# hy-vision-learning/jck-generation

Measured on AMD Instinct MI355X. Metric: images/sec (G+D step) DCGAN 64x64 bs256, higher is better.
Workload: dtype bf16; 1 GPU; DCGAN 64x64x3 synthetic, batch 256 per GPU, full G+D step incl. GP pass, RNG and Adam (BASELINE.json configs[1]); per_gpu_batch=256, global_batch=256, parallelism=dp1, dead_D_wgrad_in_G_phase=skipped (never observable: zeroed at train/dcgan_trainer.py:155)

## Files before the change

### include/jckgan.h

```cpp
#ifndef JCKGAN_H
#define JCKGAN_H
#include <stddef.h>
#include <stdint.h>
#ifdef __cplusplus
extern "C" {
#endif

#define JCK_PREC_BF16 0
#define JCK_PREC_F32 1
#define JCK_PREC_BF16X3 2

#define JCK_OK 0
#define JCK_E_ARG (-1)
#define JCK_E_HIP (-2)
#define JCK_E_WS (-3)

const char* jck_last_error(void);
const char* jck_last_launch(void);
const char* jck_launch_name(int i);
int jck_version(void);
int jck_pad_rows(int c);
int jck_pad_chan(int c);

size_t jck_packed_bytes(int prec, long long elems);
// ... 1 lines not shown
int jck_pack_up(int prec, const float* w, int Cs, int Cb, void* wp, void* stream);
int jck_pack_g1(int prec, const float* w, int Ci, int Co, int CiPad, void* wp, void* stream);
int jck_pack_head(const float* w, int C, float* wp, void* stream);

size_t jck_stats_floats(long long pixels, int C, int nyrep);
int jck_conv_down(int prec, const void* big, const void* w, void* small_out, float* stats, int* stats_slots,
                  int N, int Hb, int Wb, int Cb, int Cs, void* stream);
int jck_conv_up(int prec, const void* small_in, const void* w, void* big_out, float* stats, int* stats_slots,
                int epi_tanh, int N, int Hs, int Ws, int Cs, int Cb, void* stream);
size_t jck_conv_wgrad_ws_bytes(int N, int Hb, int Wb, int Cb, int Cs);
int jck_conv_wgrad(int prec, const void* small_side, const void* big_side, float* ws, size_t ws_bytes, float* grad,
                   int accumulate, int N, int Hb, int Wb, int Cb, int Cs, void* stream);
int jck_g1_fwd(int prec, const void* z, const void* w, void* out, float* stats, int* stats_slots, int B, int CiPad,
               int Co, void* stream);
int jck_conv_up_affine(int prec, const void* small_in, const void* w, const float* scale, const float* shift, void* big_out,
                       int N, int Hs, int Ws, int Cs, int Cb, void* stream);
int jck_g1_fwd_affine(int prec, const void* z, const void* w, const float* scale, const float* shift, void* out, int B,
                      int CiPad, int Co, void* stream);
int jck_conv_down_mask(int prec, const void* big, const void* w, const void* a_small, const float* scale, void* small_out,
                       int N, int Hb, int Wb, int Cb, int Cs, void* stream);
int jck_conv_down_affine(int prec, const void* big, const void* w, const float* scale, const float* shift, float slope,
                         void* small_out, int N, int Hb, int Wb, int Cb, int Cs, void* stream);
int jck_latent_loss(int prec, const void* x_nhwc4, const float* target_nchw_f32, void* g_raw_out, float* loss_out, int N, int HW,
                    void* stream);
int jck_latent_adam(int prec, const float* slab, int Z, int ld, float* z, float* m, float* v, float lr, float prior, int t,
                    void* z_operand, int CiPad, int N, void* stream);
int jck_conv_up_mask(int prec, const void* small_in, const void* w, const void* a_big, const float* scale, float slope, void* big_out,
                     int N, int Hs, int Ws, int Cs, int Cb, void* stream);
int jck_leaky_affine_bwd(int prec, const void* g, const void* a, const float* scale, float slope, void* g_y, long long rows, int C,
                         void* stream);
int jck_critic_ds(const float* logit, int mode, float weight, int B, float* ds, float* term, void* stream);
int jck_latent_loss_ex(int prec, const void* x_nhwc4, const float* target_nchw_f32, const float* weight, const void* g_x, void* g_raw_out,
                       float* loss_out, int N, int HW, void* stream);
int jck_feat_match(int prec, const void* a, const void* f, const float* scale, float slope, float weight, void* g_y, int accumulate,
                   float* fterm, int N, long long M, int C, void* stream);
size_t jck_g1_wgrad_ws_bytes(int B, int CiPad, int Co);
int jck_g1_wgrad(int prec, const void* z, const void* dy, float* ws, size_t ws_bytes, float* grad, int accumulate, int B,
                 int Ci, int CiPad, int Co, void* stream);

int jck_bn_finalize(const float* stats, int slots, float count, const float* gamma, const float* beta,
                    float* running_mean, float* running_var, int64_t* num_batches_tracked, float momentum, float eps,
                    float* aux, int C, void* stream);
int jck_bn_act_fwd(int prec, const void* y, const float* aux, float slope, void* a, long long rows, int C, void* stream);
int jck_bn_eval_aux(int nlayers, const float* const* gamma, const float* const* beta, const float* const* running_mean,
                    const float* const* running_var, float* const* aux, const int* C, float eps, void* stream);
size_t jck_bn_bwd_ws_floats(int C);
int jck_bn_act_bwd(int prec, const void* g_a, const void* y, const float* aux, float slope, float* sums, void* g_y,
                   float* dgamma, float* dbeta, long long rows, int C, void* stream);
int jck_bn_finalize_grouped(const float* stats, int slots_per_group, float count, const float* gamma, const float* beta, float eps,
                            float* aux, float* stat_out, int C, int groups, void* stream);
int jck_bn_fwd(int prec, const void* y, const float* stats, int slots_per_group, float count, const float* gamma, const float* beta,
               float eps, float slope, void* a, float* aux, float* stat_out, float* running_mean, float* running_var, int64_t* nbt,
               float momentum, long long rows_per_group, int C, int groups, void* stream);
int jck_bn_act_fwd_grouped(int prec, const void* y, const float* aux, float slope, void* a, long long rows_per_group, int C,
                           int groups, void* stream);
int jck_bn_act_bwd_grouped(int prec, const void* g_a, const void* y, const float* aux, float slope, float* sums, void* g_y,
                           float* dgamma, float* dbeta, long long rows_per_group, int C, int groups, int grad_groups, void* stream);
size_t jck_grid_sync_bytes(void);
int jck_grid_sync_error(const void* sync_ws);
int jck_bn_act_bwd_res(int prec, const void* g_a, const void* y, const float* aux, float slope, float* sums, void* g_y,
                       float* dgamma, float* dbeta, long long rows_per_group, int C, int groups, int grad_groups, void* sync_ws,
                       void* stream);
int jck_conv_down_grouped(int prec, const void* big, const void* w, void* small_out, float* stats, int* stats_slots, int N, int Hb,
                          int Wb, int Cb, int Cs, int group_images, void* stream);
int jck_conv_up_grouped(int prec, const void* small_in, const void* w, void* big_out, float* stats, int* stats_slots, int N, int Hs,
                        int Ws, int Cs, int Cb, int group_images, void* stream);
int jck_img_prep(int prec, const float* img_nchw, const float* noise_nchw, float keep, float mix, void* out, int N, int HW,
                 void* stream);
int jck_img_prep_u8(int prec, const unsigned char* data, const int64_t* idx, const float* noise, float keep, float mix,
                    void* out_nhwc4, float* out_nchw, int B, int Hs, int Ws, void* stream);
#define JCK_RESIZE_MAX_SRC 1024
#define JCK_RESIZE_TAPS_MAGIC 0x7a736572
long long jck_resize_taps_bytes(int Hs, int Ws, int S);
int jck_resize_taps_build(int Hs, int Ws, int S, void* host_buf);
int jck_img_prep_u8_any(int prec, const unsigned char* data, const int64_t* idx, const unsigned char* flip, const float* noise,
                        const unsigned* rng, int tensor_id, float keep, float mix, void* out_nhwc4, float* out_nchw, int B, int Hs,
                        int Ws, int S, const void* taps_dev, void* stream);
long long jck_resize_lds_bytes(int Hs, int S, int* band, int* rows);
int jck_img_prep_u8_box(int prec, const unsigned char* data, const int64_t* idx, const unsigned char* flip,
                        const int* origin , const float* noise,
                        const unsigned* rng, int tensor_id, float keep, float mix, void* out_nhwc4, float* out_nchw,
                        int B, int Hs, int Ws, int Hc, int Wc, int y0, int x0 , int S,
                        const void* taps_dev , void* stream);
int jck_resize_norm(const float* in, float* out, int N, int C, int H, int W, int OH, int OW, float pre_scale, float pre_shift,
                    const float* mean, const float* stdv, void* stream);
int jck_nhwc4_to_nchw(int prec, const void* in, float* out_nchw, int N, int HW, void* stream);
int jck_img_to_u8(int prec, const void* in, unsigned char* out_u8_nhwc, int N, int HW, void* stream);
int jck_axpy_noise(int prec, const void* x, const float* noise_nchw, float keep, float mix, void* out, int N, int HW,
                   void* stream);
int jck_interp(int prec, const void* a, const void* b, const float* alpha, void* out, int N, int HW, void* stream);
int jck_mix_interp(int prec, const void* x, const float* noise_nchw, const unsigned* rng, int tensor_id, float keep, float mix, void* out,
                   const void* real, const float* alpha, void* xhat, int N, int HW, void* stream);
int jck_gp_norm(int prec, const void* g, int N, int HW, float* scal, int slot, int scal_ld, float* norms, void* stream);
int jck_tanh_bwd(int prec, const void* g, const void* y, float scale, void* out, long long numel, void* stream);
int jck_head_fwd(int prec, const void* a4, const float* wp, const float* bias , int B, int K,
                 float target, int mode, float* prob, float* ds, float* scal, int slot_loss, int slot_p, int scal_ld, void* stream);
int jck_score_head(int prec, const void* x, const float* w, const float* bias , int B, int K,
                   float* logit, float* prob , void* stream);
int jck_grid_pool(int prec, const void* a, int N, int H, int C, int grid, int mode, float* out, long long ld, long long col0,
                  void* stream);
int jck_head_fwd_grouped(int prec, const void* a4, const float* wp, const float* bias, int B, int K, int G, const float* targets,
                         const int* modes, float* prob, float* ds, float* scal, const int* slot_loss, const int* slot_p,
                         int scal_ld, void* stream);
size_t jck_head_bwd_ws_floats(int K);
int jck_head_bwd(int prec, const float* ds, const float* wp, const void* a4, int B, int K, void* g_a4, float* dwp,
                 int accumulate, float* ws, void* stream);
int jck_head_unpack_grad(const float* dwp, int C, float* grad, int accumulate, void* stream);
int jck_head_bwd_conv(int prec, const float* ds, const float* wp, const void* a4, int B, int C, void* g_a4, float* grad,
                      float* ws, void* stream);
int jck_head_bwd_conv2(int prec, const float* ds, const float* wp, const void* a4, int B, int B_more, int C, void* g_a4, float* grad,
                       float* ws, void* stream);

int jck_pack_linear(int prec, const float* w, int N, int K, int rows, int cols, int transpose, int permC, int permHW, void* wp,
                    void* stream);
int jck_linear_fwd(int prec, const void* x, const void* wp, const float* bias, void* out, int B, int Kpad, int N, int NStore,
                   int ksplit, void* stream);
int jck_linear_finish(int prec, const float* slab, int Z, const float* bias, const float* mask, float scale, void* h, void* hd,
                      int B, int N, void* stream);
size_t jck_linear_wgrad_ws_bytes(int B, int Kpad, int N);
int jck_linear_wgrad(int prec, const void* gy, int ldgy, const void* x, int Kpad, float* ws, size_t ws_bytes, float* gradp,
                     int accumulate, int B, int N, void* stream);
int jck_unperm_linear_grad(const float* gp, int N, int K, int ldp, int permC, int permHW, float* grad, int accumulate, void* stream);
int jck_label_embed_fwd(int prec, const int64_t* labels, const float* W, const float* b, float slope, int B, int NI, int NO,
                        void* cbuf, int ld, int col0, float* pre, void* stream);
int jck_label_embed_bwd(int prec, const void* gc, int ld, int col0, const float* pre, const int64_t* labels, float slope, int B,
                        int NI, int NO, float* dW, float* db, void* stream);
int jck_label_embed_fwd_tiled(int prec, const int64_t* labels, const float* W, const float* b, float slope, int B, int NI, int NO,
                              void* cbuf, int ld, int col0, float* pre, int label_period, void* stream);
int jck_label_embed_bwd_tiled(int prec, const void* gc, int ld, int col0, const float* pre, const int64_t* labels, float slope,
                              int B, int NI, int NO, float* dW, float* db, int label_period, void* stream);
int jck_concat_rows(int prec, const void* a4, int K0, void* cbuf, int ld, int B, void* stream);
int jck_split_rows(int prec, const void* gc, int ld, int K0, void* ga4, int B, void* stream);
int jck_dropout(int prec, const void* x, const float* mask, float scale, void* y, long long n, void* stream);
int jck_colsum(int prec, const void* g, int B, int N, int ld, float* db, void* stream);
int jck_sum_vec(const float* x, int n, float* out, void* stream);
int jck_cgan_z(int prec, const float* z, const int64_t* labels, int B, int NZ, int NL, int CiPad, void* out, void* stream);
int jck_gp_grad(int prec, const void* g, const float* norms, float coef, int N, int HW, void* u, void* stream);
int jck_gp_head2(int prec, const void* ughd, const float* w2, const float* prob, int B, int K, float* rs, float* dw2, float* ws,
                 void* stream);
size_t jck_gp_head2_conv_ws_floats(int B);
int jck_gp_head2_conv(int prec, const void* v4, const void* a4, const float* wp, const float* prob, int B, int C, float* rs,
                      void* g_a4, float* grad, float* ws, void* stream);
size_t jck_bn2_ws_floats(int C);
int jck_bn2_vchain(int prec, const void* v, const void* y, const void* gy, const float* aux, const float* s1, const float* gamma,
                   float slope, float* ws, void* u, void* xdir, float* dgamma, long long rows, int C, void* stream);
int jck_bn2_reverse(int prec, const void* ua, const void* y, const void* xdir, const float* aux, const float* gamma,
                    const float* vsums, float slope, float* ws, void* uy, float* dgamma, float* dbeta, long long rows, int C,
                    void* stream);

int jck_adam(float* p, const float* g, float* m, float* v, long long n, double lr, double beta1, double beta2, double eps,
             int step, float grad_scale, void* stream);
int jck_adam_ema(float* p, const float* g, float* m, float* v, float* ema, long long n, double lr, double beta1, double beta2,
                 double eps, int step, float grad_scale, float ema_weight, const unsigned* skip_if, void* stream);

typedef struct jck_engine jck_engine;
int jck_engine_create(jck_engine** out, int family, int prec, int batch);
int jck_engine_create_sized(jck_engine** out, int family, int prec, int batch, int image_size);
#define JCK_ENGINE_GP_BACKWARD 1u
int jck_engine_create_ex(jck_engine** out, int family, int prec, int batch, int image_size, unsigned flags);
int jck_engine_image_size(const jck_engine*);
int jck_engine_num_tensors_of(const jck_engine*, int net);
int jck_engine_tensor_info_of(const jck_engine*, int net, int idx, char* name, int name_cap, int* kind, long long* offset,
                              long long* numel, int* shape4);
long long jck_engine_arena_numel_of(const jck_engine*, int net, int which);
void jck_engine_destroy(jck_engine*);
int jck_engine_num_tensors(int family, int net );
int jck_engine_tensor_info(int family, int net, int idx, char* name, int name_cap, int* kind, long long* offset,
                           long long* numel, int* shape4);
size_t jck_engine_workspace_bytes(const jck_engine*);
long long jck_engine_arena_numel(int family, int net, int which );
int jck_engine_bind(jck_engine*, void* workspace, size_t ws_bytes, float* g_params, float* g_grads, float* g_m, float* g_v,
                    float* g_bn, int64_t* g_nbt, float* d_params, float* d_grads, float* d_m, float* d_v, float* d_bn,
                    int64_t* d_nbt);
int jck_engine_repack(jck_engine*, int net, void* stream);
#define JCK_PHASE_D_LOSS 0
#define JCK_PHASE_D_GP 1
#define JCK_PHASE_D_STEP 2
#define JCK_PHASE_G_LOSS 3
#define JCK_PHASE_G_STEP 4
#define JCK_PHASE_D_REAL 5
#define JCK_PHASE_D_FAKE 6
#define JCK_PHASE_D_REAL_FWD 7
#define JCK_PHASE_D_LOSS_A 8
#define JCK_PHASE_D_LOSS_B 9
#define JCK_PHASE_GP_ONLY 10
#define JCK_PHASE_LAZY_JOIN 0x100
#define JCK_PHASE_NO_RESIDENT 0x200
typedef struct jck_step_inputs {
  const float* real_nchw;
  const float* noise_real;
  const float* z;
  const float* noise_fake;
  const float* alpha;
  float lr;
  float grad_scale;
  int step;
  const int64_t* labels;
  const float* drop_mask[4];
  const unsigned char* real_u8;
  const int64_t* real_idx;
  int real_h, real_w;
  const unsigned char* real_flip;
  const void* real_taps;
  int real_box_h, real_box_w, real_y0, real_x0;
  const int* real_origin;
} jck_step_inputs;
int jck_engine_phase(jck_engine*, int phase, const jck_step_inputs* in, void* stream);
long long jck_engine_grad_tail(const jck_engine*, int net);
int jck_engine_order_after_tail(jck_engine*, void* stream);
int jck_engine_drop_prefetch(jck_engine*, void* stream);
int jck_engine_check(jck_engine*);
const float* jck_engine_scalars(const jck_engine*);
const float* jck_engine_scalars_at(const jck_engine*, int step);
int jck_engine_sample(jck_engine*, const float* z, const int64_t* labels , int n, float* out_nchw, void* stream);
#define JCK_SAMPLE_EVAL 1u
int jck_engine_sample_ex(jck_engine*, const float* z, const int64_t* labels, int n, unsigned flags, float* out_nchw ,
                         unsigned char* out_u8_nhwc , void* stream);
int jck_engine_latent_grad(jck_engine*, const float* z, const int64_t* labels, const float* target_nchw, int n,
                           float* loss , float* dz , void* stream);
int jck_engine_project(jck_engine*, float* z , const int64_t* labels, const float* target_nchw, int n,
                       int steps, float lr, float prior, float* m, float* v , int t0,
                       float* loss_hist , void* stream);
int jck_engine_latent_grad_ex(jck_engine*, const float* z, const int64_t* labels, const float* target_nchw ,
                              const float* weight , int critic_mode, float critic_weight, int n, float* loss ,
                              float* term , float* logit , float* dz , void* stream);
int jck_engine_project_ex(jck_engine*, float* z , const int64_t* labels, const float* target_nchw , int n,
                          int steps, float lr, float prior, const float* weight , int critic_mode, float critic_weight,
                          float* m, float* v, int t0, float* loss_hist , float* term_hist ,
                          void* stream);
int jck_engine_latent_grad_fm(jck_engine*, const float* z, const int64_t* labels, const float* target_nchw ,
                              const float* weight , int critic_mode, float critic_weight, int n, float* loss ,
                              float* term , float* logit , float* dz , void* stream,
                              const float* feat_target_nchw , int feat_stage, float feat_weight, float* fterm );
int jck_engine_project_fm(jck_engine*, float* z , const int64_t* labels, const float* target_nchw , int n,
                          int steps, float lr, float prior, const float* weight , int critic_mode, float critic_weight,
                          float* m, float* v, int t0, float* loss_hist , float* term_hist ,
                          void* stream, const float* feat_target_nchw , int feat_stage, float feat_weight,
                          float* fterm_hist );
int jck_engine_score(jck_engine*, const float* images_nchw , const float* noise_nchw ,
                     const int64_t* labels , int n, float* logit , float* prob , void* stream);
long long jck_engine_feature_dim(const jck_engine*, int grid);
int jck_engine_features(jck_engine*, const float* images_nchw ,
                        int n, int grid, int mode, float* out , long long ld, void* stream);
const void* jck_engine_tensor(const jck_engine*, const char* name, long long* numel);

int jck_conv2d_nhwc_f32(const float* x, const float* w_kc, const float* scale, const float* shift, float* out, int N, int H, int W,
                        int Cin, int KH, int KW, int SH, int SW, int PH, int PW, int Cout, int out_cstride, int out_coff, int relu,
                        void* stream);
int jck_pool2d_nhwc_f32(const float* x, float* out, int N, int H, int W, int C, int k, int stride, int pad, int mode, int out_cstride,
                        int out_coff, void* stream);
int jck_global_avgpool_nhwc_f32(const float* x, float* out, int N, int HW, int C, void* stream);
int jck_nchw_to_nhwc_f32(const float* x, float* out, int N, int C, int H, int W, void* stream);
int jck_mean_cov_f64(const float* x, double* mean, double* cov, int N, int D, void* stream);

size_t jck_pairstat_ws_bytes(int M, int N);
int jck_poly3_sum_f64(const float* x, int M, const float* y, int N, int D, double gamma, double coef0, int skip_diag, double* out,
                      double* ws, void* stream);
int jck_knn_radius2_f32(const float* x, int N, int D, int k, float* r2, void* stream);
int jck_manifold_hit_u8(const float* q, int M, const float* ref, const float* r2, int N, int D, unsigned char* hit, void* stream);

size_t jck_knn_index_ws_bytes(int M, int N);
int jck_knn_index_f32(const float* q, int M, const float* ref, int N, int D, int k, long long q_base, long long ref_base,
                      int exclude_self, int merge, long long* idx, float* d2, void* ws, void* stream);

int jck_engine_set_step(jck_engine*, int step, float lr, void* stream);
int jck_engine_bind_ema(jck_engine*, float* g_ema);
int jck_engine_set_ema(jck_engine*, double decay, int start_step);
int jck_engine_set_noise_seed(jck_engine*, unsigned long long seed);
int jck_step_rng(float* hp, int step, unsigned long long seed, float* z, long long nz, float* alpha, long long nalpha,
                 float* masks, long long nmask, float keep_p, void* stream);
int jck_img_prep_rng(int prec, const float* img_nchw, const unsigned* rng, int tensor_id, float keep, float mix, void* out, int N, int HW,
                     void* stream);
int jck_img_prep_u8_rng(int prec, const unsigned char* data, const int64_t* idx, const unsigned* rng, int tensor_id, float keep,
                        float mix, void* out_nhwc4, int B, int Hs, int Ws, void* stream);
int jck_axpy_noise_rng(int prec, const void* x, const unsigned* rng, int tensor_id, float keep, float mix, void* out, int N, int HW,
                       void* stream);
int jck_engine_capture_begin(jck_engine*, void* stream);
int jck_engine_capture_end(jck_engine*, void* stream, void** graph_exec);
int jck_engine_capture_abort(jck_engine*, void* stream);
int jck_engine_graph_nodes(const jck_engine*);
int jck_graph_launch(void* graph_exec, void* stream);
void jck_graph_destroy(void* graph_exec);

int jck_tune(const char* key, int value);
int jck_prof_enable(int on);
int jck_prof_collect(int cap, const char** name_out, int* count_out, double* ms_out, double* flops_out, double* bytes_out,
                     void** stream_out);

int jck_debug_tr_read(const void* in, int ld, void* out, void* stream);

typedef struct jck_comm jck_comm;
#define JCK_COMM_ID_BYTES 128
int jck_comm_unique_id(unsigned char* id128);
int jck_comm_create(jck_comm** out, const unsigned char* id128, int world, int rank);
int jck_comm_world(const jck_comm*);
int jck_comm_allreduce_enqueue(jck_comm*, float* buf, size_t count, void* producer_stream, int* ticket);
int jck_comm_wait(jck_comm*, int ticket, void* consumer_stream);
int jck_comm_destroy(jck_comm*);

#ifdef __cplusplus
}
#endif
#endif
```

### jck-generation_amd/csrc/engine.hip

```cpp
#include <cstdlib>

#include "engine_internal.hpp"
#define JCK_BATCHED_DEFAULT 3

namespace {

constexpr long long ALIGN_F = 64;

void add_param(NetLayout& L, const char* name, int a, int b, int c, int d) {
  TensorInfo ti{name, 0, L.n_params, (long long)a * b * c * d, {a, b, c, d}};
  L.t.push_back(ti);
  L.n_params = (L.n_params + ti.numel + ALIGN_F - 1) / ALIGN_F * ALIGN_F;
}
void add_bn(NetLayout& L, const char* wn, const char* bn, const char* rm, const char* rv, int c) {
  add_param(L, wn, c, 1, 1, 1);
  add_param(L, bn, c, 1, 1, 1);
  TensorInfo m{rm, 1, L.n_bn, c, {c, 1, 1, 1}};
  L.t.push_back(m);
  L.n_bn += (c + ALIGN_F - 1) / ALIGN_F * ALIGN_F;
  TensorInfo v{rv, 2, L.n_bn, c, {c, 1, 1, 1}};
  L.t.push_back(v);
  L.n_bn += (c + ALIGN_F - 1) / ALIGN_F * ALIGN_F;
}

Topo make_topo(int S) {
  Topo T = {};
  T.S = S; T.NS = S == 128 ? 5 : 4; T.HW = S * S;
  T.G_C1 = 64 << (T.NS - 1);
  T.FEAT = 16 * T.G_C1;
  for (int i = 0; i < T.NS; ++i) {
    T.D_CS[i] = 64 << i; T.D_CB[i] = i == 0 ? 3 : 32 << i; T.D_HB[i] = S >> i;
    T.G_CS[i] = T.G_C1 >> i; T.G_CB[i] = i == T.NS - 1 ? 3 : T.G_C1 >> (i + 1); T.G_HS[i] = 4 << i;
  }
  return T;
}
NetLayout make_layout(int family, int net, int S = 64) {
  NetLayout L;
  const Topo T = make_topo(S);
  const char* const* CW = CWN; const char* const* NW = NWN; const char* const* NB = NBN; const char* const* RM = RMN; const char* const* RV = RVN;
  if (net == 0) {
    add_param(L, CW[0], z_dim(family), T.G_C1, 4, 4);
    add_bn(L, NW[0], NB[0], RM[0], RV[0], T.G_C1);
    for (int i = 0; i < T.NS; ++i) {
      add_param(L, CW[i + 1], T.G_CS[i], T.G_CB[i], 4, 4);
      if (i < T.NS - 1) add_bn(L, NW[i + 1], NB[i + 1], RM[i + 1], RV[i + 1], T.G_CB[i]);
    }
  } else {
    if (family == 1) {
      add_param(L, "label_embedding.weight", EMB, N_CLASS, 1, 1);
      add_param(L, "label_embedding.bias", EMB, 1, 1, 1);
    }
    for (int i = 0; i < T.NS; ++i) {
      add_param(L, CW[i], T.D_CS[i], T.D_CB[i], 4, 4);
      add_bn(L, NW[i], NB[i], RM[i], RV[i], T.D_CS[i]);
    }
    if (family == 0) {
      add_param(L, CW[T.NS], 1, T.G_C1, 4, 4);
    } else {
      add_param(L, "linear1.weight", L1_OUT, L1_K, 1, 1);
      add_param(L, "linear1.bias", L1_OUT, 1, 1, 1);
      add_param(L, "linear2.weight", 1, L1_OUT, 1, 1);
      add_param(L, "linear2.bias", 1, 1, 1, 1);
    }
  }
  return L;
}

}

static unsigned jck_event_flags() { return hipEventDisableTiming | hipEventDisableSystemFence; }

DActs DActs::group(const jck_engine* e, int first, int n) const {
  DActs v = *this;
  v.g0 = g0 + first; v.groups = n;
  const size_t B = (size_t)e->B;
  auto at = [&](void* p, size_t elems) { return (void*)((unsigned char*)p + elems * e->esz); };
  for (int i = 0; i < TT.NS; ++i) {
    const int cs = TT.D_CS[i];
    const size_t px = (size_t)(TT.D_HB[i] / 2) * (TT.D_HB[i] / 2), off = first * B * px * cs;
    v.y[i] = at(y[i], off); v.a[i] = at(a[i], off); v.g[i] = at(g[i], off);
    v.aux[i] = aux[i] + (size_t)first * 4 * cs;
    v.sums[i] = sums[i] + (size_t)first * jck_bn_bwd_ws_floats(cs);
    v.stats[i] = stats[i] + (size_t)first * (jck_stats_floats((long long)(cap * B * px), cs, 1) / cap / (2 * cs)) * (2 * cs);
  }
  v.prob = prob + first * B; v.ds = ds + first * B;
  return v;
}

static bool env_on(const char* name) {
  const char* v = getenv(name);
  return !(v && atoi(v) == 0);
}
static int create_side_streams(jck_engine* e) {
  hipError_t rc = hipSuccess;
  e->for_each_side_stream([&](hipStream_t& s) { if (rc == hipSuccess) rc = hipStreamCreateWithFlags(&s, hipStreamNonBlocking); });
  e->for_each_event([&](hipEvent_t& ev) { if (rc == hipSuccess) rc = hipEventCreateWithFlags(&ev, jck_event_flags()); });
  HIPCHK(rc);
  return JCK_OK;
}
static void destroy_side_streams(jck_engine* e, bool sync) {
  e->for_each_side_stream([&](hipStream_t& s) {
    if (s) { if (sync) (void)hipStreamSynchronize(s); (void)hipStreamDestroy(s); }
    s = nullptr;
  });
  e->for_each_event([](hipEvent_t& ev) { if (ev) (void)hipEventDestroy(ev); ev = nullptr; });
}

extern "C" int jck_engine_create(jck_engine** out, int family, int prec, int batch) {
  return jck_engine_create_sized(out, family, prec, batch, 64);
}
extern "C" int jck_engine_create_sized(jck_engine** out, int family, int prec, int batch, int image_size) {
  return jck_engine_create_ex(out, family, prec, batch, image_size, 0);
}
extern "C" int jck_engine_create_ex(jck_engine** out, int family, int prec, int batch, int image_size, unsigned flags) {
  if (!out) JCK_FAIL(JCK_E_ARG, "null out");
  if (flags & ~JCK_ENGINE_GP_BACKWARD) JCK_FAIL(JCK_E_ARG, "unknown engine flags");
  if (image_size != 64 && image_size != 128) JCK_FAIL(JCK_E_ARG, "image_size must be 64 or 128");
  if (image_size != 64 && family != 0) JCK_FAIL(JCK_E_ARG, "the 128x128 topology exists for DCGAN only (CGAN's Linear(8392,256) fixes 64x64)");
  if (family != 0 && family != 1) JCK_FAIL(JCK_E_ARG, "family must be 0 (DCGAN) or 1 (CGAN)");
  if (prec != JCK_PREC_BF16 && !prec_f32_storage(prec)) JCK_FAIL(JCK_E_ARG, "bad prec");
  if (batch < 1 || batch > 8192) JCK_FAIL(JCK_E_ARG, "batch must be in [1, 8192]");
  jck_engine* e = new jck_engine();
  e->family = family; e->prec = prec; e->B = batch; e->esz = prec_f32_storage(prec) ? 4 : 2;
  e->T = make_topo(image_size);
  e->LG = make_layout(family, 0, image_size); e->LD = make_layout(family, 1, image_size);
  e->overlap = env_on("JCK_OVERLAP");
  e->batched = getenv("JCK_BATCHED") ? atoi(getenv("JCK_BATCHED")) : JCK_BATCHED_DEFAULT;
  if (!e->overlap || batch % 8 != 0 || e->batched != 3) e->batched = 0;
  e->gp_bwd = family == 0 && (flags & JCK_ENGINE_GP_BACKWARD);
  e->carve(nullptr);
  e->wgrad_side = env_on("JCK_WGRAD_SIDE");
  e->head_side = env_on("JCK_HEAD_SIDE");
  e->ext_events = env_on("JCK_EXT_EVENTS");
  e->bn_res = env_on("JCK_BN_RES");
  e->cbuf_direct = family == 1 && env_on("JCK_CBUF_DIRECT");
  e->head_fuse = env_on("JCK_HEAD_FUSE");
  e->real_side = env_on("JCK_REAL_SIDE");
  e->fold_zero = env_on("JCK_FOLD_ZERO");
  e->fuse_tanh = env_on("JCK_FUSE_TANH");
  if (e->overlap) JCK_TRY(create_side_streams(e));
  *out = e;
  return JCK_OK;
}
extern "C" void jck_engine_destroy(jck_engine* e) {
  if (!e) return;
  if (e->overlap) destroy_side_streams(e, true);
  infer_free(e);
  delete e;
}
extern "C" int jck_engine_num_tensors(int family, int net) { return (int)make_layout(family, net).t.size(); }
static int tensor_info(const NetLayout& L, int idx, char* name, int name_cap, int* kind, long long* offset, long long* numel, int* shape4) {
  if (idx < 0 || idx >= (int)L.t.size()) JCK_FAIL(JCK_E_ARG, "index out of range");
  const TensorInfo& t = L.t[idx];
  if (name && name_cap > 0) { strncpy(name, t.name, name_cap - 1); name[name_cap - 1] = 0; }
  if (kind) *kind = t.kind;
  if (offset) *offset = t.offset;
  if (numel) *numel = t.numel;
  if (shape4) for (int q_ = 0; q_ < 4; ++q_) shape4[q_] = t.shape[q_];
  return JCK_OK;
}
static long long arena_numel(const NetLayout& L, int which) { return which == 0 ? L.n_params : L.n_bn; }
extern "C" int jck_engine_tensor_info(int family, int net, int idx, char* name, int name_cap, int* kind, long long* offset,
                                      long long* numel, int* shape4) {
  return tensor_info(make_layout(family, net), idx, name, name_cap, kind, offset, numel, shape4);
}
extern "C" long long jck_engine_arena_numel(int family, int net, int which) { return arena_numel(make_layout(family, net), which); }
extern "C" int jck_engine_num_tensors_of(const jck_engine* e, int net) { return e ? (int)(net == 0 ? e->LG : e->LD).t.size() : 0; }
extern "C" int jck_engine_tensor_info_of(const jck_engine* e, int net, int idx, char* name, int name_cap, int* kind, long long* offset,
                                         long long* numel, int* shape4) {
  if (!e) JCK_FAIL(JCK_E_ARG, "null engine");
  return tensor_info(net == 0 ? e->LG : e->LD, idx, name, name_cap, kind, offset, numel, shape4);
}
extern "C" long long jck_engine_arena_numel_of(const jck_engine* e, int net, int which) {
  return e ? arena_numel(net == 0 ? e->LG : e->LD, which) : 0;
}
extern "C" int jck_engine_image_size(const jck_engine* e) { return e ? e->T.S : 0; }
extern "C" size_t jck_engine_workspace_bytes(const jck_engine* e) { return e ? e->ws_bytes : 0; }

extern "C" int jck_engine_bind(jck_engine* e, void* workspace, size_t ws_bytes, float* g_params, float* g_grads, float* g_m,
                               float* g_v, float* g_bn, int64_t* g_nbt, float* d_params, float* d_grads, float* d_m,
                               float* d_v, float* d_bn, int64_t* d_nbt) {
  if (!e || !workspace) JCK_FAIL(JCK_E_ARG, "null engine / workspace");
  if (ws_bytes < e->ws_bytes) JCK_FAIL(JCK_E_WS, "workspace too small: need " + std::to_string(e->ws_bytes));
  if (((uintptr_t)workspace) % 256) JCK_FAIL(JCK_E_ARG, "workspace must be 256-byte aligned");
  e->carve(reinterpret_cast<unsigned char*>(workspace));
  {
    unsigned char* p0 = reinterpret_cast<unsigned char*>(e->d_down[0]);
    unsigned char* p1 = reinterpret_cast<unsigned char*>(e->dset[0].y[0]);
    HIPCHK(hipMemset(p0, 0, (size_t)(p1 - p0)));
  }
  HIPCHK(hipMemset(e->gsync, 0, jck_grid_sync_bytes()));
  e->gp = g_params; e->gg = g_grads; e->gm = g_m; e->gv = g_v; e->gbn = g_bn; e->gnbt = g_nbt;
  e->dp = d_params; e->dg = d_grads; e->dm = d_m; e->dv = d_v; e->dbn = d_bn; e->dnbt = d_nbt;
  e->bound = true;
  return JCK_OK;
}

static int repack_convs(jck_engine* e, int net, void* stream, const TailJobs* tail = nullptr, int tail_x = 0) {
  PackJobs jobs = {};
  int n = 0, chunk = 0;
  auto add = [&](int kind, const float* w, void* wp, long long total, int a, int b, int c) {
    PackJob& J = jobs.j[n];
    J.w = w; J.wp = wp; J.total = total; J.kind = kind; J.a = a; J.b = b; J.c = c;
    jobs.first_chunk[n] = chunk;
    chunk += (int)((total + PACK_CHUNK - 1) / PACK_CHUNK);
    ++n;
  };
  auto add_down = [&](const float* w, int Cs, int Cb, void* wp) { add(0, w, wp, (long long)Cs * Cb, Cs, Cb, ilog2(jck_pad_chan(Cb))); };
  auto add_up = [&](const float* w, int Cs, int Cb, void* wp) {
    if (Cb <= 4) add(2, w, wp, (long long)Cs * Cb, Cs, Cb, 0);
    else add(1, w, wp, (long long)Cs * Cb, Cs, Cb, jck_pad_rows(Cb));
  };
  if (net == 1) {
    for (int i = 0; i < TT.NS; ++i) {
      const float* w = e->P(e->LD, e->dp, CWN[i]);
      add_down(w, TT.D_CS[i], TT.D_CB[i], e->d_down[i]);
      add_up(w, TT.D_CS[i], TT.D_CB[i], e->d_up[i]);
    }
    if (e->family == 0) add(4, e->P(e->LD, e->dp, CWN[TT.NS]), e->d_head_wp, TT.G_C1, TT.G_C1, 0, 0);
  } else {
    add(3, e->P(e->LG, e->gp, CWN[0]), e->g1_w, (long long)z_dim(e->family) * TT.G_C1, z_dim(e->family), TT.G_C1, z_pad(e->family));
    for (int i = 0; i < TT.NS; ++i) {
      const float* w = e->P(e->LG, e->gp, CWN[i + 1]);
      add_up(w, TT.G_CS[i], TT.G_CB[i], e->g_up[i]);
      add_down(w, TT.G_CS[i], TT.G_CB[i], e->g_down[i]);
    }
  }
  jobs.first_chunk[n] = chunk;
  jobs.n = n;
  if (net == 1) e->d_packed = true;
  if (tail) {
    const int nblk = chunk + tail_x * (tail->nl + 1);
    if (e->prec == JCK_PREC_BF16) hipLaunchKernelGGL(pack_tail_kernel<bf16_t>, dim3(nblk), dim3(256), 0, (hipStream_t)stream, jobs, chunk, *tail, tail_x);
    else hipLaunchKernelGGL(pack_tail_kernel<float>, dim3(nblk), dim3(256), 0, (hipStream_t)stream, jobs, chunk, *tail, tail_x);
  } else if (e->prec == JCK_PREC_BF16) hipLaunchKernelGGL(pack_multi_kernel<bf16_t>, dim3(chunk), dim3(256), 0, (hipStream_t)stream, jobs);
  else hipLaunchKernelGGL(pack_multi_kernel<float>, dim3(chunk), dim3(256), 0, (hipStream_t)stream, jobs);
  HIPCHK(hipGetLastError());
  return JCK_OK;
}
static int repack_linear(jck_engine* e, void* stream) {
  const float* w1 = e->P(e->LD, e->dp, "linear1.weight");
  return pack_linear_pair(e->prec, w1, L1_OUT, L1_K, L1_OUT, L1_KPAD, e->l1_w, L1_KPAD, L1_OUT, e->l1_wT, 512, 16, (hipStream_t)stream);
}
extern "C" int jck_engine_repack(jck_engine* e, int net, void* stream) {
  if (!e || !e->bound) JCK_FAIL(JCK_E_ARG, "engine not bound");
  JCK_TRY(repack_convs(e, net, stream));
  if (net == 1 && e->family == 1) JCK_TRY(repack_linear(e, stream));
  return JCK_OK;
}

static const double ADAM_B1 = 0.5, ADAM_B2 = 0.999, ADAM_EPS = 1e-8;


static int fork_side(jck_engine* e, int k, hipStream_t st, hipStream_t side, hipStream_t* ws, bool record = true) {
  *ws = st;
  if (!side) return JCK_OK;
  if (record) HIPCHK(hipEventRecord(e->evW[k], st));
  HIPCHK(hipStreamWaitEvent(side, e->evW[k], 0));
  *ws = side;
  return JCK_OK;
}

static int d_convs_forward(jck_engine* e, const DActs& S, const void* x_in, int B, int pass0, hipStream_t st, bool to_cbuf = false) {
  const int n = S.groups;
  const void* in = x_in;
  for (int i = 0; i < TT.NS; ++i) {
    const int hb = TT.D_HB[i], cs = TT.D_CS[i];
    const long long rows = (long long)B * (hb / 2) * (hb / 2);
    float* rec = e->d_rs[i] + ((size_t)e->parity * 4 + pass0 + S.g0) * 2 * cs;
    int slots = 0;
    JCK_TRY(jck_conv_down_grouped(e->prec, in, e->d_down[i], S.y[i], S.stats[i], &slots, n * B, hb, hb, TT.D_CB[i], cs, B, st));
    if (slots % n) JCK_FAIL(JCK_E_ARG, "batched D pass: statistic slots do not split by group");
    const bool cb = to_cbuf && i == TT.NS - 1;
    void* out = cb ? (unsigned char*)e->cbuf + (size_t)S.g0 * B * L1_KPAD * e->esz : S.a[i];
    bool fused = false;
    JCK_TRY(bn_fwd_fused(e->prec, S.y[i], S.stats[i], slots / n, (float)rows, e->P(e->LD, e->dp, NWN[i]), e->P(e->LD, e->dp, NBN[i]), BN_EPS, LRELU, out,
                         S.aux[i], rec, nullptr, nullptr, nullptr, BN_MOM, rows, cs, n, cb ? TT.FEAT : 0, cb ? L1_KPAD : 0, st, &fused));
    if (!fused) {
      JCK_TRY(jck_bn_finalize_grouped(S.stats[i], slots / n, (float)rows, e->P(e->LD, e->dp, NWN[i]), e->P(e->LD, e->dp, NBN[i]), BN_EPS, S.aux[i], rec,
                                      cs, n, st));
      JCK_TRY(bn_act_fwd_pitched(e->prec, S.y[i], S.aux[i], LRELU, out, rows, cs, n, cb ? TT.FEAT : 0, cb ? L1_KPAD : 0, st));
    }
    in = S.a[i];
  }
  return JCK_OK;
}

static int cg_head_forward(jck_engine* e, const void* a4, int rows, const float* drop_mask, hipStream_t st, int label_period = 0, bool finish = true) {
  if (!e->cur_labels || !drop_mask) JCK_FAIL(JCK_E_ARG, "CGAN pass needs labels and a dropout mask");
  if (a4) JCK_TRY(jck_concat_rows(e->prec, a4, TT.FEAT, e->cbuf, L1_KPAD, rows, st));
  JCK_TRY(jck_label_embed_fwd_tiled(e->prec, e->cur_labels, e->P(e->LD, e->dp, "label_embedding.weight"),
                                    e->P(e->LD, e->dp, "label_embedding.bias"), LRELU, rows, N_CLASS, EMB, e->cbuf, L1_KPAD, TT.FEAT,
                                    e->pre_e, label_period, st));
  JCK_TRY(jck_linear_fwd(e->prec, e->cbuf, e->l1_w, nullptr, e->l1_slab, rows, L1_KPAD, L1_OUT, L1_OUT, L1_KSPLIT, st));
  if (!finish) return JCK_OK;
  return jck_linear_finish(e->prec, e->l1_slab, L1_KSPLIT, e->P(e->LD, e->dp, "linear1.bias"), drop_mask, 1.0f / 0.75f, e->h_pre,
                           e->h_drop, rows, L1_OUT, st);
}
static int cg_head_middle(jck_engine* e, int B, int G, const float* targets, const int* modes, const int* slot_loss, const int* slot_p,
                          float* prob, float* ds, const float* drop_mask, hipStream_t st) {
  return cg_head_mid(e->prec, e->l1_slab, L1_KSPLIT, e->P(e->LD, e->dp, "linear1.bias"), drop_mask, 1.0f / 0.75f, e->h_pre, e->h_drop,
                     e->P(e->LD, e->dp, "linear2.weight"), e->P(e->LD, e->dp, "linear2.bias"), B, G, targets, modes, prob, ds, e->acc, slot_loss,
                     slot_p, e->acc_ld, e->g_hd, e->g_h, st);
}

static int d_forward(jck_engine* e, DActs& D, const void* x_in, int B, int pass, const float* drop_mask, hipStream_t st, bool head_finish = true) {
  const bool direct = e->family == 1 && e->cbuf_direct;
  JCK_TRY(d_convs_forward(e, D, x_in, B, pass, st, direct));
  if (e->family == 1) return cg_head_forward(e, direct ? nullptr : D.a[TT.NS - 1], B, drop_mask, st, 0, head_finish);
  return JCK_OK;
}

static int d_head(jck_engine* e, DActs& D, int B, float target, int mode, int slot_loss, int slot_p, hipStream_t st, void* g_out = nullptr) {
  if (e->family == 0)
    return head_fwd_grouped_ev(e->prec, D.a[TT.NS - 1], e->d_head_wp, nullptr, B, TT.FEAT, 1, &target, &mode, D.prob, D.ds, e->acc, &slot_loss,
                               &slot_p, e->acc_ld, g_out, st, nullptr);
  return jck_head_fwd(e->prec, e->h_drop, e->P(e->LD, e->dp, "linear2.weight"), e->P(e->LD, e->dp, "linear2.bias"), B, L1_OUT, target,
                      mode, D.prob, D.ds, e->acc, slot_loss, slot_p, e->acc_ld, st);
}

static int d_head_backward(jck_engine* e, DActs& D, const float* ds, int B, bool want_wgrad, const float* drop_mask, void* ga4_out, hipStream_t st,
                           hipStream_t side = nullptr, bool mid_done = false) {
  if (e->family == 0)
    return jck_head_bwd_conv(e->prec, ds, e->d_head_wp, D.a[TT.NS - 1], B, TT.G_C1, mid_done ? nullptr : ga4_out,
                             want_wgrad ? e->P(e->LD, e->dg, CWN[TT.NS]) : nullptr, e->head_ws, st);
  const size_t r0 = (size_t)e->ss.head_row0, w0 = (size_t)e->ss.head_wrow0;
  auto hb = [&](void* p, size_t row, size_t per_row) { return (void*)((unsigned char*)p + row * per_row * e->esz); };
  void *h_drop = hb(e->h_drop, r0, L1_OUT), *cbuf = hb(e->cbuf, r0, L1_KPAD);
  void *g_hd = hb(e->g_hd, w0, L1_OUT), *g_h = hb(e->g_h, w0, L1_OUT), *gc = hb(e->gc, w0, L1_KPAD);
  const float* pre_e = e->pre_e + r0 * EMB;
  hipStream_t ws = st;
  auto fork = [&](int k) { return fork_side(e, k, st, side, &ws); };
  const float* w2 = e->P(e->LD, e->dp, "linear2.weight");
  if (!mid_done) JCK_TRY(jck_head_bwd(e->prec, ds, w2, h_drop, B, L1_OUT, g_hd, nullptr, 1, e->head_ws, st));
  if (want_wgrad) {
    JCK_TRY(fork(0));
    JCK_TRY(jck_head_bwd(e->prec, ds, w2, h_drop, B, L1_OUT, nullptr, e->P(e->LD, e->dg, "linear2.weight"), 1, e->head_ws, ws));
    JCK_TRY(jck_sum_vec(ds, B, e->P(e->LD, e->dg, "linear2.bias"), ws));
  }
  if (!mid_done) JCK_TRY(jck_dropout(e->prec, g_hd, drop_mask, 1.0f / 0.75f, g_h, (long long)B * L1_OUT, st));
  if (want_wgrad) {
    JCK_TRY(fork(1));
    JCK_TRY(jck_linear_wgrad(e->prec, g_h, L1_OUT, cbuf, L1_KPAD, e->wg_ws, e->wg_ws_bytes, e->gw1p, 1, B, L1_OUT, ws));
    JCK_TRY(jck_colsum(e->prec, g_h, B, L1_OUT, L1_OUT, e->P(e->LD, e->dg, "linear1.bias"), ws));
  }
  JCK_TRY(jck_linear_fwd(e->prec, g_h, e->l1_wT, nullptr, gc, B, L1_OUT, L1_KPAD, L1_KPAD, 1, st));
  if (want_wgrad) {
    JCK_TRY(fork(2));
    JCK_TRY(jck_label_embed_bwd(e->prec, gc, L1_KPAD, TT.FEAT, pre_e, e->cur_labels, LRELU, B, N_CLASS, EMB,
                                e->P(e->LD, e->dg, "label_embedding.weight"), e->P(e->LD, e->dg, "label_embedding.bias"), ws));
  }
  return jck_split_rows(e->prec, gc, L1_KPAD, TT.FEAT, ga4_out, B, st);
}

static int cg_head_backward_batched(jck_engine* e, const float* ds, int B, const float* drop_mask, void* ga4_out, hipStream_t st,
                                    hipStream_t side = nullptr, bool mid_done = false) {
  const int R3 = 3 * B, R2 = 2 * B;
  const float* w2 = e->P(e->LD, e->dp, "linear2.weight");
  hipStream_t ws = st;
  auto fork = [&](int k) { return fork_side(e, k, st, side, &ws); };
  if (!mid_done) JCK_TRY(jck_head_bwd(e->prec, ds, w2, e->h_drop, R3, L1_OUT, e->g_hd, nullptr, 1, e->head_ws, st));
  if (!mid_done) {
    JCK_TRY(fork(0));
    JCK_TRY(jck_head_bwd(e->prec, ds, w2, e->h_drop, R2, L1_OUT, nullptr, e->P(e->LD, e->dg, "linear2.weight"), 1, e->head_ws, ws));
    JCK_TRY(jck_sum_vec(ds, R2, e->P(e->LD, e->dg, "linear2.bias"), ws));
    JCK_TRY(jck_dropout(e->prec, e->g_hd, drop_mask, 1.0f / 0.75f, e->g_h, (long long)R3 * L1_OUT, st));
  }
  JCK_TRY(fork(1));
  if (mid_done) {
    JCK_TRY(jck_head_bwd(e->prec, ds, w2, e->h_drop, R2, L1_OUT, nullptr, e->P(e->LD, e->dg, "linear2.weight"), 1, e->head_ws, ws));
    JCK_TRY(jck_sum_vec(ds, R2, e->P(e->LD, e->dg, "linear2.bias"), ws));
  }
  JCK_TRY(jck_linear_wgrad(e->prec, e->g_h, L1_OUT, e->cbuf, L1_KPAD, e->wg_ws, e->wg_ws_bytes, e->gw1p, 1, R2, L1_OUT, ws));
  JCK_TRY(jck_colsum(e->prec, e->g_h, R2, L1_OUT, L1_OUT, e->P(e->LD, e->dg, "linear1.bias"), ws));
  JCK_TRY(jck_linear_fwd(e->prec, e->g_h, e->l1_wT, nullptr, e->gc, R3, L1_OUT, L1_KPAD, L1_KPAD, 1, st));
  JCK_TRY(fork(2));
  JCK_TRY(jck_label_embed_bwd_tiled(e->prec, e->gc, L1_KPAD, TT.FEAT, e->pre_e, e->cur_labels, LRELU, R2, N_CLASS, EMB,
                                    e->P(e->LD, e->dg, "label_embedding.weight"), e->P(e->LD, e->dg, "label_embedding.bias"), B, ws));
  if (side) HIPCHK(hipEventRecord(e->evHead, side));
  return jck_split_rows(e->prec, e->gc, L1_KPAD, TT.FEAT, ga4_out, R3, st);
}

// ... 133 lines not shown
    JCK_TRY(jck_linear_wgrad(e->prec, gh1, L1_OUT, e->cbuf2, L1_KPAD, e->wg_ws, e->wg_ws_bytes, e->gw1p, 1, B, L1_OUT, ws));
    if (side) (void)hipEventRecord(e->evGP, side);
    JCK_TRY(jck_linear_fwd(e->prec, e->cbuf2, e->l1_w, nullptr, e->l1_slab, B, L1_KPAD, L1_OUT, L1_OUT, L1_KSPLIT, st));
    const bool fuse = e->head_fuse && L1_OUT == 256;
    if (!fuse) JCK_TRY(jck_linear_finish(e->prec, e->l1_slab, L1_KSPLIT, nullptr, drop_mask, 1.0f / 0.75f, nullptr, e->ughd, B, L1_OUT, st));
    hipStream_t hs = e->head_side && e->ext_events ? side : nullptr;
    if (fuse) {
      const size_t w0 = (size_t)e->ss.head_wrow0 * L1_OUT * esz;
      JCK_TRY(gp_head_mid_ev(e->prec, e->l1_slab, L1_KSPLIT, drop_mask, 1.0f / 0.75f, e->ughd, e->P(e->LD, e->dp, "linear2.weight"), prob1, B, e->rs,
                             e->P(e->LD, e->dg, "linear2.weight"), e->gp2_ws, (unsigned char*)e->g_hd + w0, (unsigned char*)e->g_h + w0, st, hs,
                             hs ? e->evHead : nullptr));
    } else
      JCK_TRY(gp_head2_ev(e->prec, e->ughd, e->P(e->LD, e->dp, "linear2.weight"), prob1, B, L1_OUT, e->rs,
                          e->P(e->LD, e->dg, "linear2.weight"), e->gp2_ws, st, hs, hs ? e->evHead : nullptr));
    if (side) (void)hipStreamWaitEvent(st, e->evGP, 0); else join();
    JCK_TRY(d_head_backward(e, e->dset[0], e->rs, B, true, drop_mask, e->d_v[TT.NS - 1], st, hs, fuse));
    JCK_TRY(jck_unperm_linear_grad(e->gw1p, L1_OUT, L1_K, L1_KPAD, 512, 16, e->P(e->LD, e->dg, "linear1.weight"), 1, hs ? hs : st));
  }
  for (int i = TT.NS - 1; i >= 0; --i) {
    const int hb = TT.D_HB[i], cs = TT.D_CS[i], cb = TT.D_CB[i];
    const long long rows = (long long)B * (hb / 2) * (hb / 2);
    JCK_TRY(jck_bn2_reverse(e->prec, e->d_v[i], P.y[i], e->d_xdir[i], P.aux[i], e->P(e->LD, e->dp, NWN[i]), e->bn2_ws[i],
                            LRELU, e->bn2_ws_rev, e->d_v[i], e->P(e->LD, e->dg, NWN[i]), e->P(e->LD, e->dg, NBN[i]), rows, cs, st));
    const void* big = i == 0 ? xhat : P.a[i - 1];
    JCK_TRY(fork(i));
    JCK_TRY(jck_conv_wgrad(e->prec, e->d_v[i], big, e->wg_ws, e->wg_ws_bytes, e->P(e->LD, e->dg, CWN[i]), 1, B, hb, hb, cb, cs, ws));
    if (side && lazy_join && i == 1) { (void)hipEventRecord(e->evWmid, side); e->ss.mid_recorded = true; }
    if (i > 0)
      JCK_TRY(jck_conv_up(e->prec, e->d_v[i], e->d_up[i], e->d_v[i - 1], nullptr, nullptr, 0, B, hb / 2, hb / 2, cs, cb, st));
  }
  if (side && lazy_join) { (void)hipEventRecord(e->evWdone, side); e->ss.join_pending = true; }
  else join();
  return JCK_OK;
}

int g_eval_fold(jck_engine* e, hipStream_t st) {
  const float *gamma[JCK_MAX_STAGES], *beta[JCK_MAX_STAGES], *rm[JCK_MAX_STAGES], *rv[JCK_MAX_STAGES];
  float* aux[JCK_MAX_STAGES];
  int Cs[JCK_MAX_STAGES];
  for (int i = 0; i < TT.NS; ++i) {
    gamma[i] = e->P(e->LG, e->gp, NWN[i]); beta[i] = e->P(e->LG, e->gp, NBN[i]);
    rm[i] = e->gbn + find(e->LG, RMN[i])->offset; rv[i] = e->gbn + find(e->LG, RVN[i])->offset;
    aux[i] = e->g_bn[i].aux; Cs[i] = TT.G_C1 >> i;
  }
  return jck_bn_eval_aux(TT.NS, gamma, beta, rm, rv, aux, Cs, BN_EPS, st);
}
int g_eval_products(jck_engine* e, int B, hipStream_t st) {
  const int zp = z_pad(e->family);
  auto scale = [&](int i) { return e->g_bn[i].aux; };
  auto shift = [&](int i) { return e->g_bn[i].aux + (TT.G_C1 >> i); };
  JCK_TRY(jck_g1_fwd_affine(e->prec, e->g_z, e->g1_w, scale(0), shift(0), e->g_a[0], B, zp, TT.G_C1, st));
  for (int i = 0; i < TT.NS; ++i) {
    const int h = 4 << i;
    if (i < TT.NS - 1)
      JCK_TRY(jck_conv_up_affine(e->prec, e->g_a[i], e->g_up[i], scale(i + 1), shift(i + 1), e->g_a[i + 1], B, h, h, TT.G_CS[i], TT.G_CB[i], st));
    else
      JCK_TRY(jck_conv_up(e->prec, e->g_a[i], e->g_up[i], e->fake_raw, nullptr, nullptr, 1, B, h, h, TT.G_CS[i], TT.G_CB[i], st));
  }
  return JCK_OK;
}

int g_forward(jck_engine* e, const float* z, const int64_t* labels, int B, hipStream_t st, bool z_in_place, bool eval) {
  const int zp = z_pad(e->family);
  if (e->family == 1) {
    if (!labels) JCK_FAIL(JCK_E_ARG, "CGAN generator needs labels");
    JCK_TRY(jck_cgan_z(e->prec, z, labels, B, 100, N_CLASS, zp, e->g_z, st));
  } else if (!z_in_place) {
    e->ss.gz_step = -1;
    if (e->prec == JCK_PREC_BF16) launch_pad_rows<bf16_t>(z, B, 100, zp, e->g_z, st); else launch_pad_rows<float>(z, B, 100, zp, e->g_z, st);
    HIPCHK(hipGetLastError());
  }
  if (eval) {
    JCK_TRY(g_eval_fold(e, st));
    return g_eval_products(e, B, st);
  }
  JCK_TRY(jck_g1_fwd(e->prec, e->g_z, e->g1_w, e->g_y[0], e->g_bn[0].stats, &e->g_bn[0].slots, B, zp, TT.G_C1, st));
  for (int i = 0; i < TT.NS; ++i) {
    const int h = 4 << i, C = TT.G_C1 >> i;
    const long long rows = (long long)B * h * h;
    bool fused = false;
    JCK_TRY(bn_fwd_fused(e->prec, e->g_y[i], e->g_bn[i].stats, e->g_bn[i].slots, (float)rows, e->P(e->LG, e->gp, NWN[i]), e->P(e->LG, e->gp, NBN[i]), BN_EPS,
                         0.f, e->g_a[i], e->g_bn[i].aux, nullptr, e->gbn + find(e->LG, RMN[i])->offset, e->gbn + find(e->LG, RVN[i])->offset,
                         (int64_t*)(e->gnbt + i), BN_MOM, rows, C, 1, 0, 0, st, &fused));
    if (!fused) {
    JCK_TRY(jck_bn_finalize(e->g_bn[i].stats, e->g_bn[i].slots, (float)rows, e->P(e->LG, e->gp, NWN[i]), e->P(e->LG, e->gp, NBN[i]),
                            e->gbn + find(e->LG, RMN[i])->offset, e->gbn + find(e->LG, RVN[i])->offset,
                            e->gnbt + i, BN_MOM, BN_EPS, e->g_bn[i].aux, C, st));
    JCK_TRY(jck_bn_act_fwd(e->prec, e->g_y[i], e->g_bn[i].aux, 0.f, e->g_a[i], rows, C, st));
    }
    if (i < TT.NS - 1)
      JCK_TRY(jck_conv_up_grouped(e->prec, e->g_a[i], e->g_up[i], e->g_y[i + 1], e->g_bn[i + 1].stats, &e->g_bn[i + 1].slots, B, h, h, TT.G_CS[i], TT.G_CB[i], B, st));
    else
      JCK_TRY(jck_conv_up(e->prec, e->g_a[i], e->g_up[i], e->fake_raw, nullptr, nullptr, 1, B, h, h, TT.G_CS[i], TT.G_CB[i], st));
  }
  return JCK_OK;
}

static int g_backward(jck_engine* e, const void* g_fake, int B, hipStream_t st, hipStream_t side, bool raw_ready = false) {
  const bool ext = side && e->ext_events;
  if (!raw_ready)
    JCK_TRY(tanh_bwd_ev(e->prec, g_fake, e->fake_raw, 0.9f, e->g_raw, (long long)B * TT.HW * 4, st, ext ? e->evW[TT.NS - 1] : nullptr));
  const void* gbig = e->g_raw;
  for (int i = TT.NS - 1; i >= 0; --i) {
    const int hs = TT.G_HS[i], cs = TT.G_CS[i], cb = TT.G_CB[i];
    hipStream_t ws = st;
    if (side) { if (!ext) HIPCHK(hipEventRecord(e->evW[i], st)); HIPCHK(hipStreamWaitEvent(side, e->evW[i], 0)); ws = side; }
    JCK_TRY(jck_conv_wgrad(e->prec, e->g_a[i], gbig, e->wg_ws, e->wg_ws_bytes, e->P(e->LG, e->gg, CWN[i + 1]), 1, B,
                           2 * hs, 2 * hs, cb, cs, ws));
    const long long rows = (long long)B * hs * hs;
    JCK_TRY(jck_conv_down(e->prec, gbig, e->g_down[i], e->g_gr[i], nullptr, nullptr, B, 2 * hs, 2 * hs, cb, cs, st));
    JCK_TRY(bn_act_bwd_res_ev(e->prec, e->g_gr[i], e->g_y[i], e->g_bn[i].aux, 0.f, e->g_bn[i].sums, e->g_gr[i],
                              e->P(e->LG, e->gg, NWN[i]), e->P(e->LG, e->gg, NBN[i]), rows, cs, 1, 1, e->bn_res ? e->gsync : nullptr, st,
                              ext && i > 0 ? e->evW[i - 1] : nullptr));
    gbig = e->g_gr[i];
  }
  JCK_TRY(jck_g1_wgrad(e->prec, e->g_z, e->g_gr[0], e->g1_ws, e->g1_ws_bytes, e->P(e->LG, e->gg, CWN[0]), 1, B, z_dim(e->family),
                       z_pad(e->family), TT.G_C1, st));
  if (side) { HIPCHK(hipEventRecord(e->evWdone, side)); HIPCHK(hipStreamWaitEvent(st, e->evWdone, 0)); }
  return JCK_OK;
}

static int prep_real(jck_engine* e, const jck_step_inputs* in, int B, hipStream_t st) {
  if (in->real_u8 && in->real_box_h)
    return jck_img_prep_u8_box(e->prec, in->real_u8, in->real_idx, in->real_flip, in->real_origin, in->noise_real, in->noise_real ? nullptr : e->rng(),
                               0, 0.9f, 0.1f, e->real_noisy, nullptr, B, in->real_h, in->real_w, in->real_box_h, in->real_box_w, in->real_y0,
                               in->real_x0, TT.S, in->real_taps, st);
  if (in->real_u8 && in->real_taps)
    return jck_img_prep_u8_any(e->prec, in->real_u8, in->real_idx, in->real_flip, in->noise_real, in->noise_real ? nullptr : e->rng(), 0,
                               0.9f, 0.1f, e->real_noisy, nullptr, B, in->real_h, in->real_w, TT.S, in->real_taps, st);
  if (in->real_u8) {
    if (TT.S != 64) JCK_FAIL(JCK_E_ARG, "the device-resident uint8 pipeline is the reference's Resize(64) of 32x32 images: 64x64 engines only");
    if (!in->noise_real)
      return jck_img_prep_u8_rng(e->prec, in->real_u8, in->real_idx, e->rng(), 0, 0.9f, 0.1f, e->real_noisy, B, 32, 32, st);
    return jck_img_prep_u8(e->prec, in->real_u8, in->real_idx, in->noise_real, 0.9f, 0.1f, e->real_noisy, nullptr, B, 32, 32, st);
  }
  if (!in->noise_real) return jck_img_prep_rng(e->prec, in->real_nchw, e->rng(), 0, 0.9f, 0.1f, e->real_noisy, B, TT.HW, st);
  return jck_img_prep(e->prec, in->real_nchw, in->noise_real, 0.9f, 0.1f, e->real_noisy, B, TT.HW, st);
}

static int refresh_adam_scalars(jck_engine* e, int step, float lr, hipStream_t st) {
  const int q = step & 1;
  JCK_TRY(jck_adam_set_step(e->hp2 + 8 * q, (double)lr, ADAM_B1, ADAM_B2, step, e->noise_seed, e->ema_w(step), st));
  e->hp_step[q] = step;
  e->hp_lr[q] = lr;
  return JCK_OK;
}
static int set_step_impl(jck_engine* e, int step, float lr, void* stream, bool zero_d);
static int adam_net(jck_engine* e, int net, long long first, long long count, float grad_scale, const float* hp, hipStream_t st,
                    float* zero_other = nullptr, float* ema = nullptr) {
  float *p = net ? e->dp : e->gp, *g = net ? e->dg : e->gg, *m = net ? e->dm : e->gm, *v = net ? e->dv : e->gv;
  return jck_adam_hp(p + first, g + first, m + first, v + first, count, ADAM_B1, ADAM_B2, ADAM_EPS, grad_scale, hp, st, zero_other,
                     zero_other ? (net ? e->LG : e->LD).n_params : 0, jck_grid_sync_error_word(e->gsync), ema);
}
static int clear_or_memset(jck_engine* e, int& clean_step, int step, hipStream_t st, void* p, size_t bytes, void* p2 = nullptr, size_t bytes2 = 0) {
  const bool clean = clean_step == step && !e->capturing;
  clean_step = -1;
  if (!clean) HIPCHK(hipMemsetAsync(p, 0, bytes, st));
  if (!clean && p2) HIPCHK(hipMemsetAsync(p2, 0, bytes2, st));
  return JCK_OK;
}
static int zero_d_grads(jck_engine* e, int step, hipStream_t st) {
  return clear_or_memset(e, e->ss.dg_clean_step, step, st, e->dg, e->LD.n_params * sizeof(float), e->family == 1 ? e->gw1p : nullptr,
                         (size_t)L1_OUT * L1_KPAD * sizeof(float));
}
static int clear_acc(jck_engine* e, int step, hipStream_t st) {
  return clear_or_memset(e, e->ss.acc_clean_step, step, st, e->acc, (size_t)8 * e->acc_ld * sizeof(float));
}

struct PhaseCtx {
  hipStream_t st, sA;
  const jck_step_inputs* in;
  const jck_step_inputs* given;
  int B, HW;
  bool cg, lazy, lazy_tail;
  bool par, ov_g, ov_gp;
  DActs &DR, &D0, &D1;
};

static int penalty_pass(jck_engine* e, const PhaseCtx& c, DActs& D, hipStream_t s) {
  JCK_TRY(jck_interp(e->prec, e->real_noisy, e->fake, c.in->alpha, e->xhat, c.B, c.HW, s));
  JCK_TRY(d_forward(e, D, e->xhat, c.B, 2, c.in->drop_mask[2], s));
  JCK_TRY(d_head(e, D, c.B, 0.f, 1, -1, -1, s));
  DBackward bw;
  bw.gw = 0; bw.resident = c.cg; bw.xgrad = bw.gp_norm = true;
  return d_backward(e, D, e->xhat, c.B, c.in->drop_mask[2], s, bw);
}
static int g_forward_step(jck_engine* e, const PhaseCtx& c, hipStream_t s) {
  return g_forward(e, c.in->z, c.in->labels, c.B, s, c.in->z == e->rz[c.in->step & 1] && e->ss.gz_step == (long long)c.in->step);
}

static int d_batched_forward(jck_engine* e, const PhaseCtx& c, bool pre, bool split, bool direct) {
  const DActs& S = e->bset;
  const bool beside = !pre && e->real_side && c.sA;
  const bool pre_side = pre && e->ss.pre_on_side;
  e->ss.pre_on_side = false;
  hipStream_t sr = beside ? c.sA : c.st;
  if (beside) { HIPCHK(hipEventRecord(e->ev0, c.st)); HIPCHK(hipStreamWaitEvent(c.sA, e->ev0, 0)); }
  if (!pre) JCK_TRY(prep_real(e, c.in, c.B, sr));
  if (!pre && split) JCK_TRY(d_convs_forward(e, S.group(e, 0, 1), e->real_noisy, c.B, 0, sr, direct));
  if (beside) HIPCHK(hipEventRecord(e->evReal, c.sA));
  JCK_TRY(g_forward_step(e, c, c.st));
  if (beside || pre_side) HIPCHK(hipStreamWaitEvent(c.st, e->evReal, 0));
  JCK_TRY(e->mix_fake_noise_interp(c.in, c.B, c.st));
  if (split) return d_convs_forward(e, S.group(e, 1, 2), e->fake, c.B, 0, c.st, direct);
  return d_convs_forward(e, S, e->real_noisy, c.B, 0, c.st, direct);
}

static int cg_batched_heads_backward(jck_engine* e, const PhaseCtx& c, bool head3, bool direct) {
  const DActs& S = e->bset;
  const float tg[2] = {0.9f, 0.1f};
  const float *w2 = e->P(e->LD, e->dp, "linear2.weight"), *b2 = e->P(e->LD, e->dp, "linear2.bias");
  e->ss.head_row0 = 0;
  if (head3) {
    const bool fuse = e->head_fuse;
    const float tg3[3] = {tg[0], tg[1], 0.f};
    const int md3[3] = {0, 0, 1}, sl3[3] = {0, 1, -1}, sp3[3] = {3, 4, -1};
    JCK_TRY(cg_head_forward(e, direct ? nullptr : S.a[TT.NS - 1], 3 * c.B, c.in->drop_mask[0], c.st, c.B, !fuse));
    if (fuse) JCK_TRY(cg_head_middle(e, c.B, 3, tg3, md3, sl3, sp3, S.prob, S.ds, c.in->drop_mask[0], c.st));
    else JCK_TRY(jck_head_fwd_grouped(e->prec, e->h_drop, w2, b2, c.B, L1_OUT, 3, tg3, md3, S.prob, S.ds, e->acc, sl3, sp3, e->acc_ld, c.st));
    JCK_TRY(cg_head_backward_batched(e, S.ds, c.B, c.in->drop_mask[0], S.g[TT.NS - 1], c.st, e->head_side ? c.sA : nullptr, fuse));
    e->ss.head_row0 = 2 * c.B;
    e->ss.head_wrow0 = 0;
  } else
    for (int g = 0; g < 3; ++g) {
      const bool pen = g == 2;
      const DActs Sg = S.group(e, g, 1);
      JCK_TRY(cg_head_forward(e, Sg.a[TT.NS - 1], c.B, c.in->drop_mask[g], c.st));
      JCK_TRY(jck_head_fwd(e->prec, e->h_drop, w2, b2, c.B, L1_OUT, pen ? 0.f : tg[g], pen ? 1 : 0, Sg.prob, Sg.ds, e->acc, pen ? -1 : g,
                           pen ? -1 : 3 + g, e->acc_ld, c.st));
      JCK_TRY(d_head_backward(e, e->dset[0], Sg.ds, c.B, !pen, c.in->drop_mask[g], Sg.g[TT.NS - 1], c.st));
    }
  DBackward bw;
  bw.gw = 2; bw.side = c.sA; bw.xgrad = bw.gp_norm = true; bw.lazy_join = c.lazy;
  JCK_TRY(d_convs_backward(e, S, e->real_noisy, c.B, c.st, bw));
  e->ss.gp_done = true;
  return JCK_OK;
}

static int phase_d_loss_batched(jck_engine* e, const PhaseCtx& c, int phase) {
  if (phase != JCK_PHASE_D_LOSS && (c.cg || e->batched != 3 || e->capturing || e->gp_bwd))
    JCK_FAIL(JCK_E_ARG, "PHASE_D_LOSS_A / _B: only with the batched DCGAN schedule, outside a capture, without JCK_ENGINE_GP_BACKWARD "
                        "(D's gradients are final only after PHASE_D_GP then)");
  const float tg[2] = {0.9f, 0.1f};
  const int sl[2] = {0, 1}, sp[2] = {3, 4};
  if (phase == JCK_PHASE_D_LOSS_B) {
    JCK_TRY(d_batched_pass(e, e->real_noisy, c.B, 3, tg, sl, sp, c.st, c.sA, 2));
    e->ss.gp_done = true;
    return JCK_OK;
  }
  if ((!c.in->real_nchw && !c.in->real_u8) || !c.in->z || !c.in->alpha) JCK_FAIL(JCK_E_ARG, "PHASE_D_LOSS needs real_nchw (or real_u8), z and alpha");
  const bool pre = !c.cg && e->ss.real_fwd_step == (long long)c.in->step;
  if (!c.cg) e->ss.real_fwd_step = -1;
  JCK_TRY(clear_acc(e, c.in->step, c.st));
  JCK_TRY(zero_d_grads(e, c.in->step, c.st));
  const bool head3 = c.cg && c.in->drop_mask[0] && c.in->drop_mask[1] == c.in->drop_mask[0] + (size_t)c.B * L1_OUT &&
                     c.in->drop_mask[2] == c.in->drop_mask[0] + (size_t)2 * c.B * L1_OUT;
  const bool direct = head3 && e->cbuf_direct;
  JCK_TRY(d_batched_forward(e, c, pre, pre || e->real_side, direct));
  if (c.cg) return cg_batched_heads_backward(e, c, head3, direct);
  const int part = phase == JCK_PHASE_D_LOSS_A ? 1 : 0;
  JCK_TRY(d_batched_pass(e, e->real_noisy, c.B, 3, tg, sl, sp, c.st, c.sA, part, c.lazy_tail));
  if (part == 0) e->ss.gp_done = true;
  return JCK_OK;
}

static int phase_d_per_pass(jck_engine* e, const PhaseCtx& c, int phase) {
  if (phase != JCK_PHASE_D_FAKE) {
    if (!c.in->real_nchw && !c.in->real_u8) JCK_FAIL(JCK_E_ARG, "PHASE_D_REAL needs real_nchw (or real_u8)");
    JCK_TRY(clear_acc(e, c.in->step, c.st));
    JCK_TRY(zero_d_grads(e, c.in->step, c.st));
  }
  hipStream_t sG = c.st;
  if (phase == JCK_PHASE_D_LOSS || phase == JCK_PHASE_D_FAKE) {
    if (!c.in->z) JCK_FAIL(JCK_E_ARG, "G forward needs z");
    if (c.ov_gp && !c.in->alpha) JCK_FAIL(JCK_E_ARG, "alpha is needed here (the penalty pass starts inside this phase)");
    if (c.ov_g) { HIPCHK(hipEventRecord(e->ev0, c.st)); HIPCHK(hipStreamWaitEvent(e->sB, e->ev0, 0)); sG = e->sB; }
    JCK_TRY(g_forward_step(e, c, sG));
    JCK_TRY(e->mix_fake_noise(c.in, c.B, sG));
    if (c.ov_g) HIPCHK(hipEventRecord(e->evF, sG));
  }
  if (phase != JCK_PHASE_D_FAKE) {
    JCK_TRY(prep_real(e, c.in, c.B, c.st));
    if (c.ov_gp && phase == JCK_PHASE_D_LOSS) HIPCHK(hipEventRecord(e->evReal, c.st));
    JCK_TRY(d_forward(e, c.DR, e->real_noisy, c.B, 0, c.in->drop_mask[0], c.st));
    JCK_TRY(d_head(e, c.DR, c.B, 0.9f, 0, 0, 3, c.st));
    DBackward bw;
    bw.side = c.sA; bw.join = phase == JCK_PHASE_D_REAL || c.cg || !e->defer_join;
    JCK_TRY(d_backward(e, c.DR, e->real_noisy, c.B, c.in->drop_mask[0], c.st, bw));
    if (phase == JCK_PHASE_D_REAL) return JCK_OK;
  }
  if (c.ov_g) HIPCHK(hipStreamWaitEvent(c.st, e->evF, 0));
  if (c.ov_gp) {
    if (phase == JCK_PHASE_D_FAKE) HIPCHK(hipEventRecord(e->evReal, c.st));
    HIPCHK(hipStreamWaitEvent(e->sC, e->evF, 0));
    HIPCHK(hipStreamWaitEvent(e->sC, e->evReal, 0));
    JCK_TRY(penalty_pass(e, c, c.D1, e->sC));
    HIPCHK(hipEventRecord(e->evGP, e->sC));
    e->ss.gp_inflight = true;
  }
  JCK_TRY(d_forward(e, c.D0, e->fake, c.B, 1, c.in->drop_mask[1], c.st));
  JCK_TRY(d_head(e, c.D0, c.B, 0.1f, 0, 1, 4, c.st));
  DBackward bw;
  bw.side = c.sA;
  return d_backward(e, c.D0, e->fake, c.B, c.in->drop_mask[1], c.st, bw);
}

static int phase_d_real_fwd(jck_engine* e, const PhaseCtx& c) {
  if (c.cg || e->batched != 3 || e->capturing) JCK_FAIL(JCK_E_ARG, "PHASE_D_REAL_FWD: only with the batched DCGAN schedule, outside a capture");
  if (!c.in->real_nchw && !c.in->real_u8) JCK_FAIL(JCK_E_ARG, "PHASE_D_REAL_FWD needs real_nchw (or real_u8)");
  hipStream_t sr = (e->real_side && c.sA) ? c.sA : c.st;
  if (sr != c.st) { HIPCHK(hipEventRecord(e->ev0, c.st)); HIPCHK(hipStreamWaitEvent(sr, e->ev0, 0)); }
  JCK_TRY(prep_real(e, c.in, c.B, sr));
  JCK_TRY(d_convs_forward(e, e->bset.group(e, 0, 1), e->real_noisy, c.B, 0, sr));
  if (sr != c.st) HIPCHK(hipEventRecord(e->evReal, sr));
  e->ss.pre_on_side = sr != c.st;
  e->ss.real_fwd_step = c.in->step;
  return JCK_OK;
}

static int phase_gp_only(jck_engine* e, const PhaseCtx& c) {
  if (!c.in->real_nchw || !c.in->noise_real || !c.given->alpha) JCK_FAIL(JCK_E_ARG, "PHASE_GP_ONLY needs real_nchw (real), noise_real (fake) and alpha");
  if (e->capturing) JCK_FAIL(JCK_E_ARG, "PHASE_GP_ONLY: not inside a capture");
  if (c.cg && !c.given->drop_mask[2]) JCK_FAIL(JCK_E_ARG, "PHASE_GP_ONLY (CGAN) needs drop_mask[2]");
  HIPCHK(hipMemsetAsync(e->acc, 0, (size_t)8 * e->acc_ld * sizeof(float), c.st));
  HIPCHK(hipMemsetAsync(e->dg, 0, e->LD.n_params * sizeof(float), c.st));
  if (c.cg) HIPCHK(hipMemsetAsync(e->gw1p, 0, (size_t)L1_OUT * L1_KPAD * sizeof(float), c.st));
  e->ss.begin_gp_only();
  JCK_TRY(jck_img_prep(e->prec, c.in->real_nchw, nullptr, 1.0f, 0.0f, e->real_noisy, c.B, c.HW, c.st));
  JCK_TRY(jck_img_prep(e->prec, c.in->noise_real, nullptr, 1.0f, 0.0f, e->fake, c.B, c.HW, c.st));
  JCK_TRY(penalty_pass(e, c, c.D0, c.st));
  if (c.cg || e->gp_bwd) JCK_TRY(gp_double_backward(e, c.D0, e->xhat, c.B, 1.0f, c.in->drop_mask[2], c.st, nullptr));
  return JCK_OK;
}

static int phase_d_gp(jck_engine* e, const PhaseCtx& c) {
  if (!c.in->alpha) JCK_FAIL(JCK_E_ARG, "PHASE_D_GP needs alpha");
  if (e->ss.gp_done && (c.cg || e->gp_bwd)) {
    e->ss.gp_done = false;
    JCK_TRY(gp_double_backward(e, e->bset.group(e, 2, 1), e->xhat, c.B, 10.0f, c.in->drop_mask[2], c.st, c.sA, c.lazy));
    if (!(c.lazy && c.sA)) e->ss.join_pending = e->ss.mid_recorded = false;
    e->ss.head_row0 = 0;
    return JCK_OK;
  }
  if (e->ss.gp_done) { e->ss.gp_done = false; return JCK_OK; }
  if (e->ss.gp_inflight) {
    HIPCHK(hipStreamWaitEvent(c.st, e->evGP, 0));
    e->ss.gp_inflight = false;
    if (e->gp_bwd) JCK_TRY(gp_double_backward(e, c.D1, e->xhat, c.B, 10.0f, nullptr, c.st, c.sA));
    return JCK_OK;
  }
  JCK_TRY(penalty_pass(e, c, c.D0, c.st));
  if (c.cg || e->gp_bwd) JCK_TRY(gp_double_backward(e, c.D0, e->xhat, c.B, 10.0f, c.in->drop_mask[2], c.st, c.sA));
  return JCK_OK;
}

static int phase_d_step(jck_engine* e, const PhaseCtx& c) {
  if (e->ss.gp_inflight || (e->gp_bwd && e->ss.gp_done)) JCK_FAIL(JCK_E_ARG, "PHASE_D_GP must be called before PHASE_D_STEP");
  if (!e->hp_holds(c.in->step, c.in->lr) && !e->capturing) JCK_TRY(refresh_adam_scalars(e, c.in->step, c.in->lr, c.st));
  const float* hp = e->hp2 + 8 * e->parity;
  float* zg = (e->fold_zero && !e->capturing && e->LG.n_params % 4 == 0) ? e->gg : nullptr;
  if (zg) e->ss.gg_clean_step = c.in->step;
  if (e->ss.join_pending) {
    const TensorInfo* c1 = find(e->LD, CWN[0]);
    const long long cut = c1->offset + c1->numel;
    HIPCHK(hipStreamWaitEvent(c.st, e->ss.mid_recorded ? e->evWmid : e->evWdone, 0));
    JCK_TRY(adam_net(e, 1, cut, e->LD.n_params - cut, c.in->grad_scale, hp, c.st, zg));
    JCK_TRY(repack_linear(e, c.st));
    if (e->ss.mid_recorded) HIPCHK(hipStreamWaitEvent(c.st, e->evWdone, 0));
    e->ss.join_pending = e->ss.mid_recorded = false;
    JCK_TRY(adam_net(e, 1, 0, cut, c.in->grad_scale, hp, c.st));
    return repack_convs(e, 1, c.st);
  }
  JCK_TRY(adam_net(e, 1, 0, e->LD.n_params, c.in->grad_scale, hp, c.st, zg));
  return jck_engine_repack(e, 1, c.st);
}

static int phase_g_loss(jck_engine* e, const PhaseCtx& c) {
  JCK_TRY(clear_or_memset(e, e->ss.gg_clean_step, c.in->step, c.st, e->gg, e->LG.n_params * sizeof(float)));
  const bool fuse = e->head_fuse;
  JCK_TRY(d_forward(e, c.D0, e->fake, c.B, 3, c.in->drop_mask[3], c.st, !fuse));
  if (fuse && !c.cg) JCK_TRY(d_head(e, c.D0, c.B, 0.9f, 0, 2, 5, c.st, c.D0.g[TT.NS - 1]));
  else if (fuse) {
    const float tg1 = 0.9f;
    const int md1 = 0, sl1 = 2, sp1 = 5;
    JCK_TRY(cg_head_middle(e, c.B, 1, &tg1, &md1, &sl1, &sp1, c.D0.prob, c.D0.ds, c.in->drop_mask[3], c.st));
  } else JCK_TRY(d_head(e, c.D0, c.B, 0.9f, 0, 2, 5, c.st));
  XgradEpi xe = {e->fake_raw, 0.9f, e->g_raw, (c.sA && e->ext_events) ? e->evW[TT.NS - 1] : nullptr, false};
  DBackward bw;
  bw.gw = 0; bw.xgrad = true; bw.xe = e->fuse_tanh ? &xe : nullptr;
  JCK_TRY(d_backward(e, c.D0, e->fake, c.B, c.in->drop_mask[3], c.st, bw, fuse));
  return g_backward(e, c.D0.gx, c.B, c.st, c.sA, xe.fused);
}

static int phase_g_step(jck_engine* e, const PhaseCtx& c) {
  if (!e->hp_holds(c.in->step, c.in->lr) && !e->capturing) JCK_TRY(refresh_adam_scalars(e, c.in->step, c.in->lr, c.st));
  JCK_TRY(adam_net(e, 0, 0, e->LG.n_params, c.in->grad_scale, e->hp2 + 8 * e->parity, c.st, nullptr, e->gema));
  TailJobs t = {};
  for (int i = 0; i < TT.NS; ++i) {
    const int cs = TT.D_CS[i];
    t.l[i].rec = e->d_rs[i] + (size_t)e->parity * 4 * 2 * cs;
    t.l[i].rm = e->dbn + find(e->LD, RMN[i])->offset;
    t.l[i].rv = e->dbn + find(e->LD, RVN[i])->offset;
    t.l[i].nbt = (long long*)(e->dnbt + i);
    t.l[i].C = cs;
  }
  t.nl = TT.NS; t.npass = 4; t.momentum = BN_MOM; t.acc = e->acc; t.acc_ld = e->acc_ld; t.B = c.B; t.invB = 1.0f / (float)c.B; t.lambda_gp = 10.0f; t.out = e->scal_out;
  return repack_convs(e, 0, c.st, &t, cdiv(TT.G_C1, 256));
}

static int phase_begin(jck_engine* e, int phase, jck_step_inputs& loc, hipStream_t st) {
  const bool cg = e->family == 1;
  const int q = loc.step & 1;
  if (!loc.z) loc.z = e->rz[q];
  if (!loc.alpha) loc.alpha = e->ralpha[q];
  if (cg && !loc.drop_mask[0] && !loc.drop_mask[1] && !loc.drop_mask[2] && !loc.drop_mask[3])
    for (int i = 0; i < 4; ++i) loc.drop_mask[i] = e->rmask[q] + (size_t)i * e->B * L1_OUT;
  if (e->ss.join_pending && !(phase == JCK_PHASE_D_STEP || (phase == JCK_PHASE_D_GP && cg && e->ss.gp_done))) {
    HIPCHK(hipStreamWaitEvent(st, e->evWdone, 0));
    e->ss.join_pending = e->ss.mid_recorded = false;
  }
  if (cg) {
    if (!loc.labels) JCK_FAIL(JCK_E_ARG, "CGAN phases need labels");
    e->cur_labels = loc.labels;
  }
  e->parity = q;
  if (!e->capturing) {
    const int ph = phase & 0xff;
    const bool zero_d = ph == JCK_PHASE_D_LOSS || ph == JCK_PHASE_D_LOSS_A || ph == JCK_PHASE_D_REAL || ph == JCK_PHASE_D_REAL_FWD;
    if (e->hp_step[q] != loc.step) JCK_TRY(set_step_impl(e, loc.step, loc.lr, st, zero_d));
    else if (e->hp_lr[q] != loc.lr) JCK_TRY(refresh_adam_scalars(e, loc.step, loc.lr, st));
  }
  e->acc = e->acc2 + (size_t)8 * e->acc_ld * e->parity;
  e->scal_out = e->scal2 + 8 * e->parity;
  return JCK_OK;
}
static int phase_impl(jck_engine* e, int phase, const jck_step_inputs* in_, void* stream) {
  if (!e || !e->bound || !in_) JCK_FAIL(JCK_E_ARG, "engine not bound / null inputs");
  hipStream_t st = (hipStream_t)stream;
  const bool cg = e->family == 1;
  const bool lazy = (phase & JCK_PHASE_LAZY_JOIN) && cg && !e->capturing;
  const bool lazy_tail = (phase & JCK_PHASE_LAZY_JOIN) && !cg && (phase & 0xff) == JCK_PHASE_D_LOSS_A;
  phase &= ~JCK_PHASE_LAZY_JOIN;
  jck_step_inputs loc = *in_;
  JCK_TRY(phase_begin(e, phase, loc, st));
  const bool par = e->overlap && !e->capturing;
  const PhaseCtx c = {st, (par && e->wgrad_side) ? e->sA : nullptr, &loc, in_, e->B, TT.HW, cg, lazy, lazy_tail, par, par, par && !cg,
                      cg ? e->dset[0] : e->dset[2], e->dset[0], e->dset[1]};
  switch (phase) {
    case JCK_PHASE_D_LOSS_A: case JCK_PHASE_D_LOSS_B: return phase_d_loss_batched(e, c, phase);
    case JCK_PHASE_D_LOSS: return e->batched ? phase_d_loss_batched(e, c, phase) : phase_d_per_pass(e, c, phase);
    case JCK_PHASE_D_REAL: case JCK_PHASE_D_FAKE: return phase_d_per_pass(e, c, phase);
    case JCK_PHASE_D_REAL_FWD: return phase_d_real_fwd(e, c);
    case JCK_PHASE_GP_ONLY: return phase_gp_only(e, c);
    case JCK_PHASE_D_GP: return phase_d_gp(e, c);
    case JCK_PHASE_D_STEP: return phase_d_step(e, c);
    case JCK_PHASE_G_LOSS: return phase_g_loss(e, c);
    case JCK_PHASE_G_STEP: return phase_g_step(e, c);
  }
  JCK_FAIL(JCK_E_ARG, "unknown phase");
}
extern "C" int jck_engine_phase(jck_engine* e, int phase, const jck_step_inputs* in_, void* stream) {
  const bool keep_res = e ? e->bn_res : false;
  if (e && (phase & JCK_PHASE_NO_RESIDENT)) e->bn_res = false;
  const int rc = phase_impl(e, phase & ~JCK_PHASE_NO_RESIDENT, in_, stream);
  if (e) e->bn_res = keep_res;
  if (rc != JCK_OK && e) {
    if (e->ss.join_pending && e->sA && stream && !e->capturing) (void)hipStreamWaitEvent((hipStream_t)stream, e->evWdone, 0);
    e->ss.drop_promises();
  }
  return rc;
}

static int set_step_impl(jck_engine* e, int step, float lr, void* stream, bool zero_d) {
  if (!e || !e->bound) JCK_FAIL(JCK_E_ARG, "engine not bound");
  if (e->capturing) JCK_FAIL(JCK_E_ARG, "set_step inside a graph capture would bake one step's scalars into the graph");
  const int q = step & 1;
  zero_d = zero_d && e->fold_zero && e->LD.n_params % 4 == 0;
  JCK_TRY(jck_adam_set_step(e->hp2 + 8 * q, (double)lr, ADAM_B1, ADAM_B2, step, e->noise_seed, e->ema_w(step), (hipStream_t)stream, e->rz[q], (long long)e->B * 100,
                            e->ralpha[q], e->B, e->rmask[q], e->rmask[q] ? (long long)4 * e->B * L1_OUT : 0, 0.75f,
                            e->acc2 + (size_t)8 * e->acc_ld * q, (long long)8 * e->acc_ld,
                            zero_d ? e->dg : nullptr, e->LD.n_params, zero_d && e->family == 1 ? e->gw1p : nullptr, (long long)L1_OUT * L1_KPAD,
                            e->family == 0 && e->fold_zero ? e->g_z : nullptr, 100, z_pad(e->family), prec_f32_storage(e->prec) ? 1 : 0));
  e->ss.gz_step = (e->family == 0 && e->fold_zero) ? step : -1;
  if (zero_d) e->ss.dg_clean_step = step;
  e->ss.acc_clean_step = step;
  e->hp_step[step & 1] = step;
  e->hp_lr[step & 1] = lr;
  return JCK_OK;
}
extern "C" int jck_engine_set_step(jck_engine* e, int step, float lr, void* stream) { return set_step_impl(e, step, lr, stream, false); }
extern "C" int jck_engine_bind_ema(jck_engine* e, float* g_ema) {
  if (!e || !e->bound) JCK_FAIL(JCK_E_ARG, "engine not bound");
  if (e->capturing) JCK_FAIL(JCK_E_ARG, "bind_ema inside a graph capture");
  if ((uintptr_t)g_ema & 15) JCK_FAIL(JCK_E_ARG, "bind_ema: the EMA arena must be 16-byte aligned");
  e->gema = g_ema;
  e->hp_step[0] = e->hp_step[1] = 0;
  e->hp_lr[0] = e->hp_lr[1] = -1.f;
  return JCK_OK;
}
extern "C" int jck_engine_set_ema(jck_engine* e, double decay, int start_step) {
  if (!e) JCK_FAIL(JCK_E_ARG, "null engine");
  if (!(decay >= 0.0 && decay <= 1.0)) JCK_FAIL(JCK_E_ARG, "set_ema: decay must lie in [0, 1]");
  e->ema_decay = decay; e->ema_start = start_step;
  e->hp_step[0] = e->hp_step[1] = 0;
  e->hp_lr[0] = e->hp_lr[1] = -1.f;
  return JCK_OK;
}
extern "C" int jck_engine_set_noise_seed(jck_engine* e, unsigned long long seed) {
  if (!e) JCK_FAIL(JCK_E_ARG, "null engine");
  e->noise_seed = seed;
  e->hp_step[0] = e->hp_step[1] = 0;
  e->hp_lr[0] = e->hp_lr[1] = -1.f;
  return JCK_OK;
}

extern "C" int jck_engine_capture_begin(jck_engine* e, void* stream) {
  if (!e || !e->bound) JCK_FAIL(JCK_E_ARG, "engine not bound");
  if (!stream) JCK_FAIL(JCK_E_ARG, "cannot capture on the default stream");
  if (jck_prof_is_on()) JCK_FAIL(JCK_E_ARG, "per-launch profiling (jck_prof_enable) records timing events: not capturable");
  HIPCHK(hipStreamBeginCapture((hipStream_t)stream, hipStreamCaptureModeRelaxed));
  e->capturing = true;
  return JCK_OK;
}
extern "C" int jck_engine_capture_end(jck_engine* e, void* stream, void** graph_exec) {
  if (!e || !graph_exec) JCK_FAIL(JCK_E_ARG, "null argument");
  e->capturing = false;
  hipGraph_t g = nullptr;
  HIPCHK(hipStreamEndCapture((hipStream_t)stream, &g));
  {
    size_t nn = 0, ne = 0;
    hipError_t q = hipGraphGetNodes(g, nullptr, &nn);
    if (q == hipSuccess) q = hipGraphGetEdges(g, nullptr, nullptr, &ne);
    bool linear = q == hipSuccess && nn > 0 && ne == nn - 1;
    e->graph_nodes = (int)nn;
    if (linear && ne > 0) {
      std::vector<hipGraphNode_t> from(ne), to(ne);
      q = hipGraphGetEdges(g, from.data(), to.data(), &ne);
      linear = q == hipSuccess;
      for (size_t i = 0; linear && i < ne; ++i)
        for (size_t k = i + 1; k < ne; ++k)
          if (from[i] == from[k] || to[i] == to[k]) { linear = false; break; }
    }
    if (!linear) {
      (void)hipGraphDestroy(g);
      JCK_FAIL(JCK_E_ARG, "captured graph has parallel branches (" + std::to_string(nn) + " nodes, " + std::to_string(ne) +
                              " edges): not instantiated on this runtime - see DESIGN.md section 5.6");
    }
  }
  hipGraphExec_t ge = nullptr;
  hipError_t rc = hipGraphInstantiate(&ge, g, nullptr, nullptr, 0);
  (void)hipGraphDestroy(g);
  if (rc != hipSuccess) JCK_FAIL(JCK_E_HIP, std::string("hipGraphInstantiate: ") + hipGetErrorString(rc));
  *graph_exec = ge;
  return JCK_OK;
}
extern "C" int jck_engine_capture_abort(jck_engine* e, void* stream) {
  if (e) e->capturing = false;
  hipGraph_t g = nullptr;
  (void)hipStreamEndCapture((hipStream_t)stream, &g);
  if (g) (void)hipGraphDestroy(g);
// ... 78 lines not shown
```

### jck-generation_amd/csrc/engine_internal.hpp

```cpp
#pragma once
#include <cstring>
#include <vector>

#include "ops_internal.hpp"
#include "ew_optim.hpp"
#define JCK_INTERNAL __attribute__((visibility("hidden")))
struct jck_engine;
#define TT (e->T)

namespace jck_eng JCK_INTERNAL {

struct TensorInfo { const char* name; int kind; long long offset, numel; int shape[4]; };

struct NetLayout {
  std::vector<TensorInfo> t;
  long long n_params = 0, n_bn = 0;
};

#define JCK_MAX_STAGES 5
struct Topo {
  int S, NS, HW;
  int D_CS[JCK_MAX_STAGES], D_CB[JCK_MAX_STAGES], D_HB[JCK_MAX_STAGES];
  int G_CS[JCK_MAX_STAGES], G_CB[JCK_MAX_STAGES], G_HS[JCK_MAX_STAGES];
  int G_C1, FEAT;
};
const int N_CLASS = 100, EMB = 200, L1_OUT = 256, L1_FEAT = 8192, L1_K = L1_FEAT + EMB, L1_KPAD = 8448;
constexpr int L1_KSPLIT = 12;
inline int z_dim(int family) { return family == 1 ? 200 : 100; }
inline int z_pad(int family) { return family == 1 ? 256 : 128; }

static const char* const CWN[6] = {"conv1.weight", "conv2.weight", "conv3.weight", "conv4.weight", "conv5.weight", "conv6.weight"};
static const char* const NWN[5] = {"norm1.weight", "norm2.weight", "norm3.weight", "norm4.weight", "norm5.weight"};
static const char* const NBN[5] = {"norm1.bias", "norm2.bias", "norm3.bias", "norm4.bias", "norm5.bias"};
static const char* const RMN[5] = {"norm1.running_mean", "norm2.running_mean", "norm3.running_mean", "norm4.running_mean", "norm5.running_mean"};
static const char* const RVN[5] = {"norm1.running_var", "norm2.running_var", "norm3.running_var", "norm4.running_var", "norm5.running_var"};

inline const TensorInfo* find(const NetLayout& L, const char* name) {
  for (auto& t : L.t) if (!strcmp(t.name, name)) return &t;
  return nullptr;
}

struct Carver {
  size_t off = 0;
  unsigned char* base = nullptr;
  template <typename T> T* take(size_t count) {
    T* p = base ? reinterpret_cast<T*>(base + off) : nullptr;
    off = (off + count * sizeof(T) + 255) / 256 * 256;
    return p;
  }
};

struct BnBuf { float *stats, *sums, *aux; int slots; };

struct DActs {
  void *y[JCK_MAX_STAGES], *a[JCK_MAX_STAGES], *g[JCK_MAX_STAGES], *gx;
  float *stats[JCK_MAX_STAGES], *aux[JCK_MAX_STAGES], *sums[JCK_MAX_STAGES], *prob, *ds, *norms;
  int cap, g0, groups;
  DActs group(const jck_engine* e, int first, int n) const;
};

}
using namespace jck_eng;

static const float BN_MOM = 0.1f, BN_EPS = 1e-5f, LRELU = 0.2f;

struct StepState {
  bool gp_done = false;
  bool gp_inflight = false;
  bool join_pending = false, mid_recorded = false;
  long long real_fwd_step = -1;
  bool tail_on_side = false, pre_on_side = false;
  int head_row0 = 0;
  int head_wrow0 = 0;
  int acc_clean_step = -1;
  int dg_clean_step = -1, gg_clean_step = -1;
  long long gz_step = -1;
  void drop_promises() { acc_clean_step = dg_clean_step = gg_clean_step = -1; join_pending = mid_recorded = false; }
  void begin_gp_only() { acc_clean_step = dg_clean_step = -1; gp_done = gp_inflight = false; head_row0 = head_wrow0 = 0; }
};
struct jck_engine {
  int family, prec, B;
  Topo T;
  size_t esz;
  NetLayout LG, LD;
  size_t ws_bytes = 0;
  bool bound = false;
  float *gp = nullptr, *gg = nullptr, *gm = nullptr, *gv = nullptr, *gbn = nullptr;
  float *dp = nullptr, *dg = nullptr, *dm = nullptr, *dv = nullptr, *dbn = nullptr;
  int64_t *gnbt = nullptr, *dnbt = nullptr;
  float* gema = nullptr;
  double ema_decay = 0.0; int ema_start = 0;
  float ema_w(int step) const { return !gema ? 0.f : (step < ema_start ? 1.f : (float)(1.0 - ema_decay)); }
  int graph_nodes = 0;
  void *d_down[JCK_MAX_STAGES], *d_up[JCK_MAX_STAGES];
  float *d_head_wp, *d_head_dwp;
  void *g1_w, *g_up[JCK_MAX_STAGES], *g_down[JCK_MAX_STAGES];
  DActs dset[3] = {};
  DActs bset = {};
  int batched = 0;
  StepState ss;
  float* d_rs[JCK_MAX_STAGES];
  int parity = 0;
  hipStream_t sA = nullptr, sB = nullptr, sC = nullptr;
  hipEvent_t evW[JCK_MAX_STAGES] = {}, evWdone = nullptr, evWmid = nullptr, evHead = nullptr, evTail = nullptr, ev0 = nullptr, evF = nullptr, evReal = nullptr, evGP = nullptr;
  template <typename F> void for_each_side_stream(F f) { for (hipStream_t* p : {&sA, &sB, &sC}) f(*p); }
  template <typename F> void for_each_event(F f) {
    for (hipEvent_t* p : {&evWdone, &evWmid, &evHead, &evTail, &ev0, &evF, &evReal, &evGP}) f(*p);
    for (hipEvent_t& p : evW) f(p);
  }
  bool overlap = true, defer_join = true;
  bool wgrad_side = true;
  bool head_side = true;
  bool ext_events = true;
  unsigned* gsync = nullptr; bool bn_res = true;
  bool cbuf_direct = true;
  bool head_fuse = true;
  bool real_side = true;
  bool fold_zero = true;
  bool fuse_tanh = true;
  void *g_z, *g_y[JCK_MAX_STAGES], *g_a[JCK_MAX_STAGES], *g_gr[JCK_MAX_STAGES], *fake_raw, *fake, *g_raw;
  void *real_noisy, *xhat;
  BnBuf g_bn[JCK_MAX_STAGES];
  float *acc, *scal_out;
  float *acc2, *scal2;
  int acc_ld = 0;
  float *head_ws, *gp2_ws;
  float* hp2;
  unsigned long long noise_seed = 0x6a636b67616e0001ull;
  float *rz[2] = {nullptr, nullptr}, *ralpha[2] = {nullptr, nullptr}, *rmask[2] = {nullptr, nullptr};
  int hp_step[2] = {0, 0};
  float hp_lr[2] = {-1.f, -1.f};
  bool hp_holds(int step, float lr) const { return hp_step[step & 1] == step && hp_lr[step & 1] == lr; }
  bool capturing = false;
  bool gp_bwd = false;
  float* g1_ws = nullptr; size_t g1_ws_bytes = 0;
  float* wg_ws; size_t wg_ws_bytes;
  void *l1_w, *l1_wT;
  void *cbuf, *cbuf2;
  void *h_pre, *h_drop, *g_h, *g_hd, *gh_b1, *ughd, *gc;
  float *pre_e, *l1_slab, *gw1p, *rs, *prob_gp;
  void *d_v[JCK_MAX_STAGES], *d_xdir[JCK_MAX_STAGES], *d_u0;
  float* bn2_ws[JCK_MAX_STAGES]; float* bn2_ws_rev;
  const int64_t* cur_labels = nullptr;
  struct LatentBufs {
    void* base = nullptr;
    void* w = nullptr; float *slab = nullptr, *loss = nullptr;
  } lat;
  struct ScoreBufs {
    void* base = nullptr;
    void *x = nullptr, *y = nullptr, *a[JCK_MAX_STAGES] = {}, *cbuf = nullptr, *h = nullptr;
    float *aux[JCK_MAX_STAGES] = {}, *slab = nullptr;
  } sc;
  struct CriticBufs {
    void* base = nullptr;
    void *g[JCK_MAX_STAGES] = {}, *gx = nullptr, *g_h = nullptr, *gc = nullptr;
    float *ds = nullptr, *term = nullptr, *logit = nullptr;
  } cr;
  struct FeatBufs {
    void* base = nullptr;
    void* fa = nullptr; float* term = nullptr;
  } fm;
  bool d_packed = false;

  void carve(unsigned char* base) {
    jck_engine* e = this;
    Carver c; c.base = base;
    auto bytes = [&](size_t n) { return n * esz; };
    for (int i = 0; i < TT.NS; ++i) {
      d_down[i] = c.take<unsigned char>(bytes((size_t)jck_pad_rows(TT.D_CS[i]) * 16 * jck_pad_chan(TT.D_CB[i])));
      d_up[i] = c.take<unsigned char>(bytes((size_t)4 * jck_pad_rows(TT.D_CB[i]) * 4 * TT.D_CS[i]));
    }
    d_head_wp = c.take<float>(TT.FEAT); d_head_dwp = c.take<float>(TT.FEAT);
    g1_w = c.take<unsigned char>(bytes((size_t)16 * TT.G_C1 * z_pad(family)));
    for (int i = 0; i < TT.NS; ++i) {
      g_up[i] = c.take<unsigned char>(bytes((size_t)4 * jck_pad_rows(TT.G_CB[i]) * 4 * TT.G_CS[i]));
      g_down[i] = c.take<unsigned char>(bytes((size_t)jck_pad_rows(TT.G_CS[i]) * 16 * jck_pad_chan(TT.G_CB[i])));
    }
    const size_t img = (size_t)B * TT.HW * 4;
    auto take_set = [&](DActs& D, int cap, bool penalty_out) {
      D.cap = D.groups = cap; D.g0 = 0;
      for (int i = 0; i < TT.NS; ++i) {
        const size_t n = (size_t)cap * B * (TT.D_HB[i] / 2) * (TT.D_HB[i] / 2) * TT.D_CS[i];
        D.y[i] = c.take<unsigned char>(bytes(n)); D.a[i] = c.take<unsigned char>(bytes(n)); D.g[i] = c.take<unsigned char>(bytes(n));
        D.sums[i] = c.take<float>(cap * jck_bn_bwd_ws_floats(TT.D_CS[i]));
        D.aux[i] = c.take<float>(cap * 4 * TT.D_CS[i]);
        D.stats[i] = c.take<float>(jck_stats_floats((long long)cap * B * (TT.D_HB[i] / 2) * (TT.D_HB[i] / 2), TT.D_CS[i], 1));
      }
      if (penalty_out) D.gx = c.take<unsigned char>(bytes(img));
      D.prob = c.take<float>((size_t)cap * B); D.ds = c.take<float>((size_t)cap * B);
      if (penalty_out) D.norms = c.take<float>(B);
    };
    for (DActs& D : dset) take_set(D, 1, true);
    for (int i = 0; i < TT.NS; ++i) d_rs[i] = c.take<float>(2 * 4 * 2 * TT.D_CS[i]);
    g_z = c.take<unsigned char>(bytes((size_t)B * z_pad(family)));
    for (int i = 0; i < TT.NS; ++i) {
      const int h = 4 << i, C = TT.G_C1 >> i;
      const size_t n = (size_t)B * h * h * C;
      g_y[i] = c.take<unsigned char>(bytes(n)); g_a[i] = c.take<unsigned char>(bytes(n)); g_gr[i] = c.take<unsigned char>(bytes(n));
    }
    fake_raw = c.take<unsigned char>(bytes(img)); g_raw = c.take<unsigned char>(bytes(img));
    real_noisy = c.take<unsigned char>(bytes(img)); fake = c.take<unsigned char>(bytes(img)); xhat = c.take<unsigned char>(bytes(img));
    if (batched) {
      take_set(bset, 3, false);
      bset.gx = dset[0].gx; bset.norms = dset[0].norms;
    }
    for (int i = 0; i < TT.NS; ++i) g_bn[i].sums = c.take<float>(jck_bn_bwd_ws_floats(TT.G_C1 >> i));
    for (int i = 0; i < TT.NS; ++i) {
      const int C = TT.G_C1 >> i, h = 4 << i;
      g_bn[i].aux = c.take<float>(4 * C);
      g_bn[i].stats = c.take<float>(jck_stats_floats((long long)B * h * h, C, i == 0 ? 16 : 1));
    }
    acc_ld = (B + 63) / 64 * 64;
    acc2 = c.take<float>((size_t)2 * 8 * acc_ld); scal2 = c.take<float>(16);
    acc = acc2; scal_out = scal2;
    hp2 = c.take<float>(16);
    for (int q = 0; q < 2; ++q) {
      rz[q] = c.take<float>((size_t)B * 100); ralpha[q] = c.take<float>((size_t)(B + 3) / 4 * 4);
      rmask[q] = family == 1 ? c.take<float>((size_t)4 * B * L1_OUT) : nullptr;
    }
    head_ws = c.take<float>(jck_head_bwd_ws_floats(TT.FEAT));
    gp2_ws = c.take<float>((size_t)acc_ld + jck_head_bwd_ws_floats(L1_OUT));
    gsync = c.take<unsigned>(jck_grid_sync_bytes() / sizeof(unsigned));
    size_t w = 0;
    for (int i = 0; i < TT.NS; ++i) {
      w = std::max(w, jck_conv_wgrad_ws_bytes(B, TT.D_HB[i], TT.D_HB[i], TT.D_CB[i], TT.D_CS[i]));
      w = std::max(w, jck_conv_wgrad_ws_bytes(2 * B, TT.D_HB[i], TT.D_HB[i], TT.D_CB[i], TT.D_CS[i]));
      w = std::max(w, jck_conv_wgrad_ws_bytes(B, TT.G_HS[i] * 2, TT.G_HS[i] * 2, TT.G_CB[i], TT.G_CS[i]));
    }
    w = std::max(w, jck_g1_wgrad_ws_bytes(B, z_pad(family), TT.G_C1));
    if (family == 1) w = std::max(std::max(w, jck_linear_wgrad_ws_bytes(B, L1_KPAD, L1_OUT)), jck_linear_wgrad_ws_bytes(2 * B, L1_KPAD, L1_OUT));
    wg_ws_bytes = w;
    wg_ws = c.take<float>(w / 4);
    g1_ws_bytes = jck_g1_wgrad_ws_bytes(B, z_pad(family), TT.G_C1);
    g1_ws = c.take<float>(g1_ws_bytes / 4);
    if (family == 1) {
      l1_w = c.take<unsigned char>(bytes((size_t)L1_OUT * L1_KPAD)); l1_wT = c.take<unsigned char>(bytes((size_t)L1_KPAD * L1_OUT));
      const size_t HR = batched ? 3 : 1;
      cbuf = c.take<unsigned char>(bytes(HR * B * L1_KPAD)); cbuf2 = c.take<unsigned char>(bytes((size_t)B * L1_KPAD));
      h_pre = c.take<unsigned char>(bytes(HR * B * L1_OUT)); h_drop = c.take<unsigned char>(bytes(HR * B * L1_OUT));
      g_h = c.take<unsigned char>(bytes(HR * B * L1_OUT)); g_hd = c.take<unsigned char>(bytes(HR * B * L1_OUT));
      gh_b1 = c.take<unsigned char>(bytes((size_t)B * L1_OUT)); ughd = c.take<unsigned char>(bytes((size_t)B * L1_OUT));
      gc = c.take<unsigned char>(bytes(HR * B * L1_KPAD));
      pre_e = c.take<float>(HR * B * EMB); l1_slab = c.take<float>((size_t)L1_KSPLIT * HR * B * L1_OUT);
      gw1p = c.take<float>((size_t)L1_OUT * L1_KPAD);
    }
    if (family == 1 || gp_bwd) {
      rs = c.take<float>(B); prob_gp = c.take<float>(B);
      for (int i = 0; i < TT.NS; ++i) {
        const size_t n = (size_t)B * (TT.D_HB[i] / 2) * (TT.D_HB[i] / 2) * TT.D_CS[i];
        d_v[i] = c.take<unsigned char>(bytes(n)); d_xdir[i] = c.take<unsigned char>(bytes(n));
        bn2_ws[i] = c.take<float>(jck_bn2_ws_floats(TT.D_CS[i]));
      }
      bn2_ws_rev = c.take<float>(jck_bn2_ws_floats(TT.G_C1));
      d_u0 = c.take<unsigned char>(bytes(img));
    }
    ws_bytes = c.off;
  }

  float* P(const NetLayout& L, float* arena, const char* name) const { return arena + find(L, name)->offset; }
  const unsigned* rng() const { return reinterpret_cast<const unsigned*>(hp2 + 8 * parity + 4); }
  int mix_fake_noise(const jck_step_inputs* in, int B, hipStream_t st) {
    if (!in->noise_fake) return jck_axpy_noise_rng(prec, fake_raw, rng(), 1, 0.9f, 0.1f, fake, B, T.HW, st);
    return jck_axpy_noise(prec, fake_raw, in->noise_fake, 0.9f, 0.1f, fake, B, T.HW, st);
  }
  int mix_fake_noise_interp(const jck_step_inputs* in, int B, hipStream_t st) {
    return jck_mix_interp(prec, fake_raw, in->noise_fake, in->noise_fake ? nullptr : rng(), 1, 0.9f, 0.1f, fake, real_noisy, in->alpha, xhat,
                          B, T.HW, st);
  }
};

template <typename T>
static void launch_pad_rows(const float* z, int B, int zd, int zp, void* out, hipStream_t st) {
// ... 9 lines not shown
```

### jck-generation_amd/csrc/ew_optim.hpp

```cpp
#pragma once
#include "common.hpp"
#include "philox.hpp"

struct StepRng { float* z; long long nz; float* alpha; long long nalpha; float* masks; long long nmask; float keep_p; float* zero; long long nzero;
                 float* zbig[2]; long long nzbig[2];
                 void* zpad; int zd, zp, zpad_f32; };
__device__ __forceinline__ float u01(unsigned x) { return ((float)(x >> 8) + 0.5f) * (1.0f / 16777216.0f); }
static __global__ void adam_hp_kernel(float* __restrict__ hp, float step_size, float bc2_sqrt, unsigned seed_lo, unsigned seed_hi,
                                      unsigned step, const StepRng r, float ema_w) {
  if (threadIdx.x == 0 && blockIdx.x == 0) {
    hp[0] = step_size; hp[1] = bc2_sqrt; hp[2] = ema_w;
    unsigned* w = reinterpret_cast<unsigned*>(hp + 4);
    w[0] = seed_lo; w[1] = seed_hi; w[2] = step; w[3] = 0u;
  }
  const long long q0 = (r.nz + 3) / 4, q1 = (r.nalpha + 3) / 4, q2 = (r.nmask + 3) / 4;
  for (long long i = blockIdx.x * (long long)blockDim.x + threadIdx.x; i < r.nzero; i += (long long)gridDim.x * blockDim.x) r.zero[i] = 0.f;
#pragma unroll
  for (int b = 0; b < 2; ++b)
    for (long long i = blockIdx.x * (long long)blockDim.x + threadIdx.x; i < (r.nzbig[b] >> 2); i += (long long)gridDim.x * blockDim.x)
      reinterpret_cast<f32x4*>(r.zbig[b])[i] = f32x4{0.f, 0.f, 0.f, 0.f};
  for (long long i = blockIdx.x * (long long)blockDim.x + threadIdx.x; i < q0 + q1 + q2; i += (long long)gridDim.x * blockDim.x) {
    unsigned o[4];
    if (i < q0) {
      philox4x32_10((unsigned)i, (unsigned)(i >> 32), 8u, step, seed_lo, seed_hi, o);
      const float r0 = sqrtf(-2.0f * logf(u01(o[0]))), r1 = sqrtf(-2.0f * logf(u01(o[2])));
      float s0, c0, s1, c1;
      sincosf(6.283185307179586f * u01(o[1]), &s0, &c0);
      sincosf(6.283185307179586f * u01(o[3]), &s1, &c1);
      const float v[4] = {r0 * c0, r0 * s0, r1 * c1, r1 * s1};
      for (int k = 0; k < 4; ++k)
        if (i * 4 + k < r.nz) {
          r.z[i * 4 + k] = v[k];
          if (r.zpad) {
            const long long e = i * 4 + k, b = e / r.zd;
            const int c = (int)(e - b * r.zd);
            if (r.zpad_f32) reinterpret_cast<float*>(r.zpad)[b * r.zp + c] = v[k];
            else stf(reinterpret_cast<bf16_t*>(r.zpad) + b * r.zp + c, v[k]);
          }
        }
    } else if (i < q0 + q1) {
      const long long j = i - q0;
      philox4x32_10((unsigned)j, (unsigned)(j >> 32), 9u, step, seed_lo, seed_hi, o);
      for (int k = 0; k < 4; ++k)
        if (j * 4 + k < r.nalpha) r.alpha[j * 4 + k] = (float)(o[k] >> 8) * (1.0f / 16777216.0f);
    } else {
      const long long j = i - q0 - q1;
      philox4x32_10((unsigned)j, (unsigned)(j >> 32), 10u, step, seed_lo, seed_hi, o);
      for (int k = 0; k < 4; ++k)
        if (j * 4 + k < r.nmask) r.masks[j * 4 + k] = (float)(o[k] >> 8) * (1.0f / 16777216.0f) < r.keep_p ? 1.f : 0.f;
    }
  }
}
__device__ __forceinline__ void adam_one(float& pi, float gi_raw, float& mi_io, float& vi_io, float w1, float beta2, float omb2,
                                         float eps, float step_size, float bc2_sqrt, float grad_scale) {
  const float gi = gi_raw * grad_scale;
  const float mi = (w1 < 0.5f) ? mi_io + w1 * (gi - mi_io) : gi - (gi - mi_io) * (1.f - w1);
  const float vi = vi_io * beta2 + (omb2 * gi) * gi;
  mi_io = mi;
  vi_io = vi;
  const float denom = sqrtf(vi) / bc2_sqrt + eps;
  pi = pi - step_size * (mi / denom);
}
__device__ __forceinline__ float ema_one(float e, float pn, float w) { return (w < 0.5f) ? e + w * (pn - e) : pn - (pn - e) * (1.f - w); }
template <bool EMA>
static __global__ void adam_kernel(float* __restrict__ p, const float* __restrict__ g, float* __restrict__ m,
                            float* __restrict__ v, long long n, float w1 , float beta2, float omb2 ,
                            float eps, float step_size, float bc2_sqrt, float grad_scale, const float* __restrict__ hp = nullptr,
                            int vec = 1, float* __restrict__ zero = nullptr, long long nzero4 = 0,
                            const unsigned* __restrict__ skip_if = nullptr, float* __restrict__ ema = nullptr, float ema_w = 1.f) {
  if (hp) { step_size = hp[0]; bc2_sqrt = hp[1]; }
  if (EMA && hp) ema_w = hp[2];
  const bool skip = skip_if && *skip_if != 0u;
  for (long long i = blockIdx.x * (long long)blockDim.x + threadIdx.x; i < nzero4; i += (long long)gridDim.x * blockDim.x)
    reinterpret_cast<f32x4*>(zero)[i] = f32x4{0.f, 0.f, 0.f, 0.f};
  if (skip) return;
  const long long n4 = vec ? (n >> 2) : 0;
  for (long long i = blockIdx.x * (long long)blockDim.x + threadIdx.x; i < n4; i += (long long)gridDim.x * blockDim.x) {
    f32x4 pv = reinterpret_cast<f32x4*>(p)[i], mv = reinterpret_cast<f32x4*>(m)[i], vv = reinterpret_cast<f32x4*>(v)[i];
    const f32x4 gv = reinterpret_cast<const f32x4*>(g)[i];
    f32x4 ev;
    if (EMA) ev = reinterpret_cast<f32x4*>(ema)[i];
#pragma unroll
    for (int k = 0; k < 4; ++k) {
      float pk = pv[k], mk = mv[k], vk = vv[k];
      adam_one(pk, gv[k], mk, vk, w1, beta2, omb2, eps, step_size, bc2_sqrt, grad_scale);
      pv[k] = pk; mv[k] = mk; vv[k] = vk;
      if (EMA) ev[k] = ema_one(ev[k], pk, ema_w);
    }
    reinterpret_cast<f32x4*>(p)[i] = pv; reinterpret_cast<f32x4*>(m)[i] = mv; reinterpret_cast<f32x4*>(v)[i] = vv;
    if (EMA) reinterpret_cast<f32x4*>(ema)[i] = ev;
  }
  for (long long i = (n4 << 2) + blockIdx.x * (long long)blockDim.x + threadIdx.x; i < n; i += (long long)gridDim.x * blockDim.x) {
    adam_one(p[i], g[i], m[i], v[i], w1, beta2, omb2, eps, step_size, bc2_sqrt, grad_scale);
    if (EMA) ema[i] = ema_one(ema[i], p[i], ema_w);
  }
}

__device__ __forceinline__ float pack_down_val(const float* __restrict__ w, int Cs, int Cb, int logCbPad, long long i) {
  const long long K = 16ll << logCbPad;
  const int cs = (int)(i / K);
  const int k = (int)(i % K);
  const int t = k >> logCbPad, cb = k & ((1 << logCbPad) - 1);
  return (cs < Cs && cb < Cb) ? w[((long long)cs * Cb + cb) * 16 + t] : 0.f;
}
template <typename W>
__global__ void pack_down_kernel(const float* __restrict__ w, int Cs, int Cb, int CsPad, int logCbPad, W* __restrict__ wp) {
  const long long K = 16ll << logCbPad, total = (long long)CsPad * K;
  for (long long i = blockIdx.x * (long long)blockDim.x + threadIdx.x; i < total; i += (long long)gridDim.x * blockDim.x)
    stf(wp + i, pack_down_val(w, Cs, Cb, logCbPad, i));
}

static __device__ __constant__ int c_up_k[2][2] = {{1, 3}, {0, 2}};
__device__ __forceinline__ float pack_up_val(const float* __restrict__ w, int Cs, int Cb, int CbPad, long long i) {
  const long long K = 4ll * Cs, per = (long long)CbPad * K;
  const int phase = (int)(i / per);
  const long long r = i % per;
  const int cb = (int)(r / K);
  const int k = (int)(r % K);
  const int t = k / Cs, cs = k % Cs;
  const int kh = c_up_k[phase >> 1][t >> 1], kw = c_up_k[phase & 1][t & 1];
  return cb < Cb ? w[((long long)cs * Cb + cb) * 16 + kh * 4 + kw] : 0.f;
}
template <typename W>
__global__ void pack_up_kernel(const float* __restrict__ w, int Cs, int Cb, int CbPad, W* __restrict__ wp) {
  const long long total = 4ll * CbPad * 4 * Cs;
  for (long long i = blockIdx.x * (long long)blockDim.x + threadIdx.x; i < total; i += (long long)gridDim.x * blockDim.x)
    stf(wp + i, pack_up_val(w, Cs, Cb, CbPad, i));
}

__device__ __forceinline__ float pack_up16_val(const float* __restrict__ w, int Cs, int Cb, long long i) {
  const long long K = 9ll * Cs;
  const int r = (int)(i / K), k = (int)(i % K);
  const int phase = r >> 2, c = r & 3, t9 = k / Cs, cs = k % Cs;
  const int dy = t9 / 3 - 1, dx = t9 % 3 - 1, ph = phase >> 1, pw = phase & 1;
  const int kh = ph == 0 ? (dy == 0 ? 1 : (dy == -1 ? 3 : -1)) : (dy == 1 ? 0 : (dy == 0 ? 2 : -1));
  const int kw = pw == 0 ? (dx == 0 ? 1 : (dx == -1 ? 3 : -1)) : (dx == 1 ? 0 : (dx == 0 ? 2 : -1));
  return (c < Cb && kh >= 0 && kw >= 0) ? w[((long long)cs * Cb + c) * 16 + kh * 4 + kw] : 0.f;
}
template <typename W>
__global__ void pack_up16_kernel(const float* __restrict__ w, int Cs, int Cb, W* __restrict__ wp) {
  const long long total = 16 * 9ll * Cs;
  for (long long i = blockIdx.x * (long long)blockDim.x + threadIdx.x; i < total; i += (long long)gridDim.x * blockDim.x)
    stf(wp + i, pack_up16_val(w, Cs, Cb, i));
}

__device__ __forceinline__ float pack_g1_val(const float* __restrict__ w, int Ci, int Co, int CiPad, long long i) {
  const int ci = (int)(i % CiPad);
  const long long r = i / CiPad;
  const int co = (int)(r % Co), t = (int)(r / Co);
  return ci < Ci ? w[((long long)ci * Co + co) * 16 + t] : 0.f;
}
template <typename W>
__global__ void pack_g1_kernel(const float* __restrict__ w, int Ci, int Co, int CiPad, W* __restrict__ wp) {
  const long long total = 16ll * Co * CiPad;
  for (long long i = blockIdx.x * (long long)blockDim.x + threadIdx.x; i < total; i += (long long)gridDim.x * blockDim.x)
    stf(wp + i, pack_g1_val(w, Ci, Co, CiPad, i));
}

static __global__ void pack_head_kernel(const float* __restrict__ w, int C, float* __restrict__ wp) {
  const int i = blockIdx.x * blockDim.x + threadIdx.x;
  if (i >= 16 * C) return;
  const int t = i / C, c = i % C;
  wp[i] = w[c * 16 + t];
}

#define PACK_MAX_JOBS 12
#define PACK_CHUNK 256
struct PackJob { const float* w; void* wp; long long total; int kind, a, b, c; };
struct PackJobs { PackJob j[PACK_MAX_JOBS]; int first_chunk[PACK_MAX_JOBS + 1]; int n; };
template <typename W>
__device__ __forceinline__ void pack_multi_block(const PackJobs& jobs, int bx) {
  int ji = 0;
  while (ji + 1 < jobs.n && bx >= jobs.first_chunk[ji + 1]) ++ji;
  const PackJob& J = jobs.j[ji];
  const long long u = (long long)(bx - jobs.first_chunk[ji]) * PACK_CHUNK + threadIdx.x;
  if (u >= J.total) return;
  W* wp = reinterpret_cast<W*>(J.wp);
  float v[16];
  auto load16 = [&](const float* src) {
#pragma unroll
    for (int q = 0; q < 4; ++q) {
      const f32x4 t = *reinterpret_cast<const f32x4*>(src + 4 * q);
      v[4 * q] = t[0]; v[4 * q + 1] = t[1]; v[4 * q + 2] = t[2]; v[4 * q + 3] = t[3];
    }
  };
  switch (J.kind) {
    case 0: {
      const int Cb = J.b, cs = (int)(u / Cb), cb = (int)(u % Cb);
      load16(J.w + ((long long)cs * Cb + cb) * 16);
      W* d = wp + (((long long)cs * 16) << J.c) + cb;
#pragma unroll
      for (int t = 0; t < 16; ++t) stf(d + ((long long)t << J.c), v[t]);
    } break;
    case 1: {
      const int Cs = J.a, Cb = J.b, cb = (int)(u / Cs), cs = (int)(u % Cs);
      load16(J.w + ((long long)cs * Cb + cb) * 16);
      const long long K = 4ll * Cs, per = (long long)J.c * K;
#pragma unroll
      for (int phase = 0; phase < 4; ++phase)
#pragma unroll
        for (int t = 0; t < 4; ++t) {
          const int kh = c_up_k[phase >> 1][t >> 1], kw = c_up_k[phase & 1][t & 1];
          stf(wp + phase * per + (long long)cb * K + (long long)t * Cs + cs, v[kh * 4 + kw]);
        }
    } break;
    case 2: {
      const int Cs = J.a, Cb = J.b, c = (int)(u / Cs), cs = (int)(u % Cs);
      load16(J.w + ((long long)cs * Cb + c) * 16);
      const long long K = 9ll * Cs;
#pragma unroll
      for (int phase = 0; phase < 4; ++phase)
#pragma unroll
        for (int t9 = 0; t9 < 9; ++t9) {
          const int dy = t9 / 3 - 1, dx = t9 % 3 - 1, ph = phase >> 1, pw = phase & 1;
          const int kh = ph == 0 ? (dy == 0 ? 1 : (dy == -1 ? 3 : -1)) : (dy == 1 ? 0 : (dy == 0 ? 2 : -1));
          const int kw = pw == 0 ? (dx == 0 ? 1 : (dx == -1 ? 3 : -1)) : (dx == 1 ? 0 : (dx == 0 ? 2 : -1));
          if (kh >= 0 && kw >= 0) stf(wp + (long long)(phase * 4 + c) * K + (long long)t9 * Cs + cs, v[kh * 4 + kw]);
        }
    } break;
    case 3: {
      const int Ci = J.a, Co = J.b, co = (int)(u / Ci), ci = (int)(u % Ci);
      load16(J.w + ((long long)ci * Co + co) * 16);
#pragma unroll
      for (int t = 0; t < 16; ++t) stf(wp + ((long long)t * Co + co) * J.c + ci, v[t]);
    } break;
    default: {
      const int c = (int)u;
      load16(J.w + (long long)c * 16);
#pragma unroll
      for (int t = 0; t < 16; ++t) reinterpret_cast<float*>(J.wp)[(long long)t * J.a + c] = v[t];
    } break;
  }
}
template <typename W>
__global__ __launch_bounds__(256) void pack_multi_kernel(const PackJobs jobs) { pack_multi_block<W>(jobs, (int)blockIdx.x); }

template <typename T>
__global__ void cast_f32_kernel(const float* __restrict__ in, T* __restrict__ out, long long n) {
  for (long long i = blockIdx.x * (long long)blockDim.x + threadIdx.x; i < n; i += (long long)gridDim.x * blockDim.x)
    stf(out + i, in[i]);
}
template <typename T>
__global__ void cast_to_f32_kernel(const T* __restrict__ in, float* __restrict__ out, long long n) {
  for (long long i = blockIdx.x * (long long)blockDim.x + threadIdx.x; i < n; i += (long long)gridDim.x * blockDim.x)
    out[i] = ldf(in + i);
}

template <typename T>
__global__ void pad_rows_kernel(const float* __restrict__ in, int B, int Ci, int CiPad, T* __restrict__ out) {
  const long long total = (long long)B * CiPad;
  for (long long i = blockIdx.x * (long long)blockDim.x + threadIdx.x; i < total; i += (long long)gridDim.x * blockDim.x) {
    const int c = (int)(i % CiPad);
    const long long b = i / CiPad;
    stf(out + i, c < Ci ? in[b * Ci + c] : 0.f);
  }
}

struct TailLayer { const float* rec; float* rm; float* rv; long long* nbt; int C; };
struct TailJobs { TailLayer l[5]; int nl; int npass; float momentum; const float* acc; int acc_ld, B; float invB, lambda_gp; float* out; };
__device__ __forceinline__ void step_tail_block(const TailJobs& t, int bx, int by) {
  if (by == t.nl) {
    if (bx != 0) return;
    __shared__ float sm[4];
    float tot[7];
#pragma unroll
    for (int q = 0; q < 7; ++q) {
      float s = 0.f;
      for (int n = threadIdx.x; n < t.B; n += 256) s += t.acc[(long long)q * t.acc_ld + n];
      tot[q] = block_sum256(s, sm);
    }
    if (threadIdx.x == 0) {
      const float lr = tot[0] * t.invB, lf = tot[1] * t.invB, gp = tot[6] * t.invB;
      t.out[0] = (lr + lf) + t.lambda_gp * gp;
      t.out[1] = tot[2] * t.invB;
      t.out[2] = tot[3] * t.invB;
      t.out[3] = tot[4] * t.invB;
      t.out[4] = tot[5] * t.invB;
      t.out[5] = gp;
      t.out[6] = lr;
      t.out[7] = lf;
    }
    return;
  }
  const TailLayer& L = t.l[by];
  const int c = bx * blockDim.x + threadIdx.x;
  if (c == 0 && L.nbt) *L.nbt += t.npass;
  if (c >= L.C) return;
  float rm = L.rm[c], rv = L.rv[c];
  for (int p = 0; p < t.npass; ++p) {
    rm = (1.f - t.momentum) * rm + t.momentum * L.rec[(long long)p * 2 * L.C + c];
    rv = (1.f - t.momentum) * rv + t.momentum * L.rec[(long long)p * 2 * L.C + L.C + c];
  }
  L.rm[c] = rm;
  L.rv[c] = rv;
}
template <typename W>
__global__ __launch_bounds__(256) void pack_tail_kernel(const PackJobs jobs, int pack_chunks, const TailJobs t, int tail_x) {
  if ((int)blockIdx.x < pack_chunks) { pack_multi_block<W>(jobs, (int)blockIdx.x); return; }
  const int q = (int)blockIdx.x - pack_chunks;
  step_tail_block(t, q % tail_x, q / tail_x);
}
```

### jck-generation_amd/csrc/ops.hip

```cpp
#include "ops_internal.hpp"
#include "ew.hpp"
#include "ew_optim.hpp"
#include "latent.hpp"
#include "resize.hpp"

#include <cstdlib>
#include <cstring>
#include <string>

static thread_local std::string g_err;
void jck_set_error(const std::string& s) { g_err = s; }
extern "C" const char* jck_last_error(void) { return g_err.c_str(); }
#ifndef JCK_BUILD_ID
#define JCK_BUILD_ID 100
#endif
extern "C" int jck_version(void) { return JCK_BUILD_ID; }

struct KernelInfo { const char* launch; const char* label; };
#define SAME(s) {s, s}
static constexpr KernelInfo KERNELS[] = {
    SAME("igemm<bf16,128,128>"),   SAME("igemm<bf16,128,64>"),   SAME("igemm<bf16,64,128,img>"),   {nullptr, "igemm<bf16,64,128>"}, SAME("igemm<bf16,16,256>"),
    SAME("igemm<f32,128,128>"),    SAME("igemm<f32,128,64>"),    SAME("igemm<f32,64,128,img>"),    SAME("igemm<f32,64,128>"),       SAME("igemm<f32,16,256>"),
    SAME("igemm<bf16x3,128,128>"), SAME("igemm<bf16x3,128,64>"), SAME("igemm<bf16x3,64,128,img>"), SAME("igemm<bf16x3,64,128>"),    SAME("igemm<bf16x3,16,256>"),
    {"igemm_dma_persist<128,256,8>", "igemm<bf16,128,256>"}, {"igemm_dma_persist<128,128,4>", "igemm<bf16,128,128>"},
// ... 397 lines not shown
  if (B < 1 || K < 8 || K % 8) JCK_FAIL(JCK_E_ARG, "score_head: B >= 1 and K a multiple of 8");
  if ((uintptr_t)x % 16 || (uintptr_t)w % 16) JCK_FAIL(JCK_E_ARG, "score_head: x and w must be 16-byte aligned");
  DISPATCH_T(prec, hipLaunchKernelGGL(score_head_kernel<T>, dim3(B), dim3(256), 0, (hipStream_t)stream, (const T*)x, w, K, bias, logit, prob));
  HIPCHK(hipGetLastError());
  return JCK_OK;
}
extern "C" int jck_grid_pool(int prec, const void* a, int N, int H, int C, int grid, int mode, float* out, long long ld, long long col0, void* stream) {
  if (!a || !out) JCK_FAIL(JCK_E_ARG, "grid_pool: null a / out");
  if (N < 1 || H < 1 || C < 8 || C % 8) JCK_FAIL(JCK_E_ARG, "grid_pool: N >= 1, H >= 1 and C a multiple of 8");
  if (grid != 1 && grid != 2 && grid != 4) JCK_FAIL(JCK_E_ARG, "grid_pool: grid must be 1, 2 or 4");
  if (H % grid) JCK_FAIL(JCK_E_ARG, "grid_pool: H must be a multiple of grid");
  if (mode != 0 && mode != 1) JCK_FAIL(JCK_E_ARG, "grid_pool: mode must be 0 (max) or 1 (mean)");
  if (col0 < 0 || ld < col0 + (long long)grid * grid * C) JCK_FAIL(JCK_E_ARG, "grid_pool: the column block [col0, col0 + grid * grid * C) must lie inside a row of ld");
  if ((uintptr_t)a % 16 || ((uintptr_t)out + 4 * (uintptr_t)col0) % 16 || (N > 1 && ld % 4))
    JCK_FAIL(JCK_E_ARG, "grid_pool: a and every row's column block must be 16-byte aligned");
  DISPATCH_T(prec, {
    const long long total = (long long)N * grid * grid * (C / (16 / (int)sizeof(T)));
    hipLaunchKernelGGL(grid_pool_kernel<T>, dim3(ew_grid(total, 64)), dim3(64), 0, (hipStream_t)stream, (const T*)a, H, C, grid, mode, out, ld, col0, total);
  });
  HIPCHK(hipGetLastError());
  return JCK_OK;
}
int cg_head_mid(int prec, const float* slab, int ksplit, const float* bias1, const float* mask, float scale, void* h, void* hd, const float* w2,
                const float* bias2, int B, int G, const float* targets, const int* modes, float* prob, float* ds, float* scal,
                const int* slot_loss, const int* slot_p, int scal_ld, void* g_hd, void* g_h, hipStream_t stream) {
  if (G < 1 || G > 4 || B < 1 || !mask || !slab || ksplit < 1) JCK_FAIL(JCK_E_ARG, "cg_head_mid: 1..4 groups of >= 1 rows, a dropout mask, split-K slabs");
  HeadGroups hg;
  if (!head_groups(hg, B, G, targets, modes, slot_loss, slot_p, scal, scal_ld)) JCK_FAIL(JCK_E_ARG, "cg_head_mid: scalar slots need scal with scal_ld >= B");
  const long long rows = (long long)G * B;
  DISPATCH_T(prec, hipLaunchKernelGGL(cg_head_mid_kernel<T>, dim3((unsigned)rows), dim3(256), 0, stream, slab, ksplit, rows * 256, bias1, mask, scale,
                                      (T*)h, (T*)hd, w2, bias2, hg, 1.0f / (float)B, prob, ds, scal, scal_ld, (T*)g_hd, (T*)g_h));
  HIPCHK(hipGetLastError());
  return JCK_OK;
}
#define HEAD_NS 8
#define HEAD_CONV_NS 16
extern "C" size_t jck_head_bwd_ws_floats(int K) { return (size_t)HEAD_CONV_NS * K; }
extern "C" int jck_head_bwd(int prec, const float* ds, const float* wp, const void* a4, int B, int K, void* g_a4, float* dwp,
                            int accumulate, float* ws, void* stream) {
  if (K % 8) JCK_FAIL(JCK_E_ARG, "head_bwd: K % 8 != 0");
  if (dwp && !ws) JCK_FAIL(JCK_E_ARG, "head_bwd: the weight gradient needs a workspace of jck_head_bwd_ws_floats(K) floats");
  if (g_a4) {
    const long long total8 = (long long)B * K / 8;
    DISPATCH_T(prec, hipLaunchKernelGGL(head_dgrad_kernel<T>, dim3(ew_grid(total8)), dim3(256), 0, (hipStream_t)stream, ds, wp,
                                        K, (T*)g_a4, total8));
    HIPCHK(hipGetLastError());
  }
  if (dwp) {
    DISPATCH_T(prec, hipLaunchKernelGGL(head_wgrad_kernel<T>, dim3(cdiv(K / 8, 64), HEAD_NS), dim3(256), 0, (hipStream_t)stream, ds,
                                        (const T*)a4, B, K, ws));
    HIPCHK(hipGetLastError());
    hipLaunchKernelGGL(head_part_reduce_kernel, dim3(cdiv(K, 256)), dim3(256), 0, (hipStream_t)stream, ws, HEAD_NS, K, 0, dwp, accumulate);
    HIPCHK(hipGetLastError());
  }
  return JCK_OK;
}
extern "C" int jck_head_bwd_conv(int prec, const float* ds, const float* wp, const void* a4, int B, int C, void* g_a4,
                                 float* grad, float* ws, void* stream) {
  return jck_head_bwd_conv2(prec, ds, wp, a4, B, 0, C, g_a4, grad, ws, stream);
}
extern "C" int jck_head_bwd_conv2(int prec, const float* ds, const float* wp, const void* a4, int B, int B_more, int C, void* g_a4,
                                  float* grad, float* ws, void* stream) {
  return head_bwd_conv2_ev(prec, ds, wp, a4, B, B_more, C, g_a4, grad, ws, (hipStream_t)stream, nullptr, nullptr);
}
int head_bwd_conv2_ev(int prec, const float* ds, const float* wp, const void* a4, int B, int B_more, int C, void* g_a4, float* grad, float* ws,
                      hipStream_t stream, hipStream_t side, hipEvent_t handover) {
  if (C % 8) JCK_FAIL(JCK_E_ARG, "head_bwd_conv: C % 8 != 0");
  if ((side != nullptr) != (handover != nullptr)) JCK_FAIL(JCK_E_ARG, "head_bwd_conv: side stream and hand-over event go together");
  if (B_more < 0 || (B_more > 0 && !g_a4)) JCK_FAIL(JCK_E_ARG, "head_bwd_conv2: the extra rows produce an input gradient only");
  if (!g_a4 && !grad) return JCK_OK;
  if (grad && !ws) JCK_FAIL(JCK_E_ARG, "head_bwd_conv: the weight gradient needs a workspace of jck_head_bwd_ws_floats(16*C) floats");
  const int K = 16 * C;
  if (!g_a4 && grad && side) {
    HIPCHK(hipStreamWaitEvent(side, handover, 0));
    DISPATCH_T(prec, hipLaunchKernelGGL(head_bwd_fused_kernel<T>, dim3(cdiv(K / 8, 64), HEAD_CONV_NS), dim3(256), 0, side, ds, wp,
                                        (const T*)a4, B, K, C, (T*)nullptr, ws, 0));
    HIPCHK(hipGetLastError());
    hipLaunchKernelGGL(head_part_reduce_kernel, dim3(cdiv(K, 256)), dim3(256), 0, side, ws, HEAD_CONV_NS, K, C, grad, 1);
    HIPCHK(hipGetLastError());
    return JCK_OK;
  }
  hipEvent_t ev = grad ? handover : nullptr;
  DISPATCH_T(prec, LAUNCH_EV(head_bwd_fused_kernel<T>, dim3(cdiv(K / 8, 64), HEAD_CONV_NS), dim3(256), 0, stream, ev, ds, wp,
                             (const T*)a4, B, K, C, (T*)g_a4, grad ? ws : nullptr, B_more));
  HIPCHK(hipGetLastError());
  if (grad) {
    hipStream_t rs = stream;
    if (ev) { HIPCHK(hipStreamWaitEvent(side, ev, 0)); rs = side; }
    hipLaunchKernelGGL(head_part_reduce_kernel, dim3(cdiv(K, 256)), dim3(256), 0, rs, ws, HEAD_CONV_NS, K, C, grad, 1);
    HIPCHK(hipGetLastError());
  }
  return JCK_OK;
}

extern "C" int jck_adam(float* p, const float* g, float* m, float* v, long long n, double lr, double beta1, double beta2,
                        double eps, int step, float grad_scale, void* stream) {
  if (step < 1) JCK_FAIL(JCK_E_ARG, "adam: step is 1-based");
  const double bc1 = 1.0 - std::pow(beta1, step), bc2 = 1.0 - std::pow(beta2, step);
  const float step_size = (float)(lr / bc1), bc2s = (float)std::sqrt(bc2);
  const int vec = (((uintptr_t)p | (uintptr_t)g | (uintptr_t)m | (uintptr_t)v) & 15) == 0;
  hipLaunchKernelGGL(adam_kernel<false>, dim3(ew_grid(vec ? (n + 3) / 4 : n)), dim3(256), 0, (hipStream_t)stream, p, g, m, v, n, (float)(1.0 - beta1),
                     (float)beta2, (float)(1.0 - beta2), (float)eps, step_size, bc2s, grad_scale, (const float*)nullptr, vec);
  HIPCHK(hipGetLastError());
  return JCK_OK;
}
extern "C" int jck_adam_ema(float* p, const float* g, float* m, float* v, float* ema, long long n, double lr, double beta1, double beta2,
                            double eps, int step, float grad_scale, float ema_weight, const unsigned* skip_if, void* stream) {
  if (step < 1) JCK_FAIL(JCK_E_ARG, "adam: step is 1-based");
  if (!ema) JCK_FAIL(JCK_E_ARG, "adam_ema: null EMA arena (jck_adam is the form without one)");
  if (!(ema_weight >= 0.f && ema_weight <= 1.f)) JCK_FAIL(JCK_E_ARG, "adam_ema: ema_weight = 1 - decay must lie in [0, 1]");
  const double bc1 = 1.0 - std::pow(beta1, step), bc2 = 1.0 - std::pow(beta2, step);
  const float step_size = (float)(lr / bc1), bc2s = (float)std::sqrt(bc2);
  const int vec = (((uintptr_t)p | (uintptr_t)g | (uintptr_t)m | (uintptr_t)v | (uintptr_t)ema) & 15) == 0;
  hipLaunchKernelGGL(adam_kernel<true>, dim3(ew_grid(vec ? (n + 3) / 4 : n)), dim3(256), 0, (hipStream_t)stream, p, g, m, v, n, (float)(1.0 - beta1),
                     (float)beta2, (float)(1.0 - beta2), (float)eps, step_size, bc2s, grad_scale, (const float*)nullptr, vec, (float*)nullptr,
                     0ll, skip_if, ema, ema_weight);
  HIPCHK(hipGetLastError());
  return JCK_OK;
}
int jck_adam_set_step(float* hp, double lr, double beta1, double beta2, int step, unsigned long long seed, float ema_w, hipStream_t st, float* rz,
                      long long nz, float* ralpha, long long nalpha, float* rmasks, long long nmask, float keep_p, float* zero,
                      long long nzero, float* zbig0, long long nzbig0, float* zbig1, long long nzbig1, void* zpad, int zd, int zp, int zpad_f32) {
  if (step < 1) JCK_FAIL(JCK_E_ARG, "adam: step is 1-based");
  if (((uintptr_t)zbig0 | (uintptr_t)zbig1) & 15 || (nzbig0 | nzbig1) & 3) JCK_FAIL(JCK_E_ARG, "set_step: large zero ranges must be 16-byte aligned, counts % 4 == 0");
  const double bc1 = 1.0 - std::pow(beta1, step), bc2 = 1.0 - std::pow(beta2, step);
  StepRng r = {rz, rz ? nz : 0, ralpha, ralpha ? nalpha : 0, rmasks, rmasks ? nmask : 0, keep_p, zero, zero ? nzero : 0,
               {zbig0, zbig1}, {zbig0 ? nzbig0 : 0, zbig1 ? nzbig1 : 0}, (rz && zd > 0 && zp >= zd) ? zpad : nullptr, zd, zp, zpad_f32};
  const long long quads = std::max((r.nz + 3) / 4 + (r.nalpha + 3) / 4 + (r.nmask + 3) / 4, std::max(r.nzbig[0], r.nzbig[1]) / 16);
  const unsigned blocks = (unsigned)std::max<long long>(1, std::min<long long>((quads + 255) / 256, 1024));
  hipLaunchKernelGGL(adam_hp_kernel, dim3(blocks), dim3(256), 0, st, hp, (float)(lr / bc1), (float)std::sqrt(bc2), (unsigned)seed,
                     (unsigned)(seed >> 32), (unsigned)step, r, ema_w);
  HIPCHK(hipGetLastError());
  return JCK_OK;
}
extern "C" int jck_step_rng(float* hp, int step, unsigned long long seed, float* z, long long nz, float* alpha, long long nalpha,
                            float* masks, long long nmask, float keep_p, void* stream) {
  if (!hp) JCK_FAIL(JCK_E_ARG, "step_rng: hp scratch (8 floats) is required");
  return jck_adam_set_step(hp, 2e-4, 0.5, 0.999, step, seed, 0.f, (hipStream_t)stream, z, nz, alpha, nalpha, masks, nmask, keep_p);
}
int jck_adam_hp(float* p, const float* g, float* m, float* v, long long n, double beta1, double beta2, double eps,
                float grad_scale, const float* hp, hipStream_t st, float* zero, long long nzero, const unsigned* skip_if, float* ema) {
  const int vec = (((uintptr_t)p | (uintptr_t)g | (uintptr_t)m | (uintptr_t)v | (uintptr_t)ema) & 15) == 0;
  if (zero && (((uintptr_t)zero & 15) || (nzero & 3))) JCK_FAIL(JCK_E_ARG, "adam: the zero range must be 16-byte aligned, count % 4 == 0");
  if (ema)
    hipLaunchKernelGGL(adam_kernel<true>, dim3(ew_grid(vec ? (n + 3) / 4 : n)), dim3(256), 0, st, p, g, m, v, n, (float)(1.0 - beta1), (float)beta2,
                       (float)(1.0 - beta2), (float)eps, 0.f, 1.f, grad_scale, hp, vec, zero, zero ? nzero / 4 : 0, skip_if, ema, 1.f);
  else
    hipLaunchKernelGGL(adam_kernel<false>, dim3(ew_grid(vec ? (n + 3) / 4 : n)), dim3(256), 0, st, p, g, m, v, n, (float)(1.0 - beta1), (float)beta2,
                     (float)(1.0 - beta2), (float)eps, 0.f, 1.f, grad_scale, hp, vec, zero, zero ? nzero / 4 : 0, skip_if);
  HIPCHK(hipGetLastError());
  return JCK_OK;
}

static int launch_latent_loss(KernelId id, double bytes, int prec, const void* x, const float* target, const float* weight, const void* g_x,
                              void* g_raw, float* loss, int N, int HW, hipStream_t st) {
  ProfScope prof(id, 0.0, st, bytes);
  if (target && !weight && !g_x) {
    DISPATCH_T(prec, hipLaunchKernelGGL((latent_loss_kernel<T, true>), dim3(N), dim3(256), 0, st, (const T*)x, target, nullptr, nullptr, (T*)g_raw,
                                        loss, HW));
  } else {
    DISPATCH_T(prec, hipLaunchKernelGGL((latent_loss_kernel<T, false>), dim3(N), dim3(256), 0, st, (const T*)x, target, weight, (const T*)g_x,
                                        (T*)g_raw, loss, HW));
  }
  HIPCHK(hipGetLastError());
  return JCK_OK;
}
extern "C" int jck_latent_loss(int prec, const void* x_nhwc4, const float* target_nchw_f32, void* g_raw_out, float* loss_out, int N,
                               int HW, void* stream) {
  if (!x_nhwc4 || !target_nchw_f32 || !g_raw_out || !loss_out || N < 1 || HW < 1) JCK_FAIL(JCK_E_ARG, "latent_loss: bad arguments");
  if ((((uintptr_t)x_nhwc4 | (uintptr_t)g_raw_out) & 15) != 0) JCK_FAIL(JCK_E_ARG, "latent_loss: the image tensors must be 16-byte aligned");
  return launch_latent_loss(K_LATENT_LOSS, (double)N * HW * (12.0 + 8.0 * (prec_f32_storage(prec) ? 4 : 2)), prec, x_nhwc4, target_nchw_f32,
                            nullptr, nullptr, g_raw_out, loss_out, N, HW, (hipStream_t)stream);
}
extern "C" int jck_latent_adam(int prec, const float* slab, int Z, int ld, float* z, float* m, float* v, float lr, float prior, int t,
                               void* z_operand, int CiPad, int N, void* stream) {
  const int zd = 100;
  if (!slab || !z || Z < 1 || ld < zd || N < 1 || t < 0) JCK_FAIL(JCK_E_ARG, "latent_adam: bad arguments");
  if (t > 0 && (!m || !v || !z_operand || CiPad < zd)) JCK_FAIL(JCK_E_ARG, "latent_adam: an update needs m, v and the operand rows");
  const double bc1 = 1.0 - std::pow(0.9, (double)t), bc2 = 1.0 - std::pow(0.999, (double)t);
  const double step_size = t > 0 ? (double)lr / bc1 : 0.0, bc2_sqrt = t > 0 ? std::sqrt(bc2) : 1.0;
  ProfScope prof(K_LATENT_ADAM, 0.0, (hipStream_t)stream, (double)N * zd * 4.0 * (Z + 6));
  DISPATCH_T(prec, hipLaunchKernelGGL(latent_adam_kernel<T>, dim3((unsigned)((N * zd + 255) / 256)), dim3(256), 0, (hipStream_t)stream, slab, Z,
                                      (long long)N * ld, ld, z, m, v, step_size, bc2_sqrt, 2.0 * (double)prior / zd, (T*)z_operand, CiPad, zd,
                                      N, t == 0 ? 1 : 0));
  HIPCHK(hipGetLastError());
  return JCK_OK;
}
extern "C" int jck_latent_loss_ex(int prec, const void* x_nhwc4, const float* target_nchw_f32, const float* weight, const void* g_x,
                                  void* g_raw_out, float* loss_out, int N, int HW, void* stream) {
  if (!x_nhwc4 || !g_raw_out || !loss_out || N < 1 || HW < 1) JCK_FAIL(JCK_E_ARG, "latent_loss_ex: bad arguments");
  if (!target_nchw_f32 && !g_x) JCK_FAIL(JCK_E_ARG, "latent_loss_ex: without a target the image gradient g_x is required");
  if ((((uintptr_t)x_nhwc4 | (uintptr_t)g_raw_out | (uintptr_t)g_x) & 15) != 0) JCK_FAIL(JCK_E_ARG, "latent_loss_ex: the image tensors must be 16-byte aligned");
  return launch_latent_loss(K_LATENT_LOSS_EX, (double)N * HW * (16.0 + 12.0 * (prec_f32_storage(prec) ? 4 : 2)), prec, x_nhwc4, target_nchw_f32,
                            weight, g_x, g_raw_out, loss_out, N, HW, (hipStream_t)stream);
}
extern "C" int jck_leaky_affine_bwd(int prec, const void* g, const void* a, const float* scale, float slope, void* g_y, long long rows, int C,
                                    void* stream) {
  if (!g || !a || !scale || !g_y || rows < 1) JCK_FAIL(JCK_E_ARG, "leaky_affine_bwd: null tensor or no rows");
  if (!is_pow2(C) || C < 8) JCK_FAIL(JCK_E_ARG, "leaky_affine_bwd: C must be a power of two >= 8");
  if ((((uintptr_t)g | (uintptr_t)a | (uintptr_t)g_y | (uintptr_t)scale) & 15) != 0) JCK_FAIL(JCK_E_ARG, "leaky_affine_bwd: tensors and scale must be 16-byte aligned");
  const long long total8 = rows * C / 8;
  ProfScope prof(K_LEAKY_AFFINE_BWD, 0.0, (hipStream_t)stream, (double)rows * C * 3.0 * (prec_f32_storage(prec) ? 4 : 2));
  DISPATCH_T(prec, hipLaunchKernelGGL(leaky_affine_bwd_kernel<T>, dim3(ew_grid(total8)), dim3(256), 0, (hipStream_t)stream, (const T*)g, (const T*)a,
                                      scale, slope, (T*)g_y, total8, C));
  HIPCHK(hipGetLastError());
  return JCK_OK;
}
extern "C" int jck_feat_match(int prec, const void* a, const void* f, const float* scale, float slope, float weight, void* g_y, int accumulate,
                              float* fterm, int N, long long M, int C, void* stream) {
  if (prec != JCK_PREC_BF16 && !prec_f32_storage(prec)) JCK_FAIL(JCK_E_ARG, "feat_match: bad prec");
  if (!a || !f || !scale || !g_y || !fterm || N < 1) JCK_FAIL(JCK_E_ARG, "feat_match: null tensor or no images");
  if (!is_pow2(C) || C < 8) JCK_FAIL(JCK_E_ARG, "feat_match: C must be a power of two >= 8");
  if (M < C || M % C) JCK_FAIL(JCK_E_ARG, "feat_match: M must be a positive multiple of C");
  if (!(weight >= 0.f) || !(weight <= 3.402823466e38f)) JCK_FAIL(JCK_E_ARG, "feat_match: weight must be finite and >= 0");
  if (accumulate != 0 && accumulate != 1) JCK_FAIL(JCK_E_ARG, "feat_match: accumulate must be 0 or 1");
  if ((((uintptr_t)a | (uintptr_t)f | (uintptr_t)g_y | (uintptr_t)scale) & 15) != 0) JCK_FAIL(JCK_E_ARG, "feat_match: tensors and scale must be 16-byte aligned");
  const hipStream_t st = (hipStream_t)stream;
  ProfScope prof(K_FEAT_MATCH, 0.0, st, (double)N * M * (accumulate ? 4.0 : 3.0) * (prec_f32_storage(prec) ? 4 : 2));
  if (accumulate) {
    DISPATCH_T(prec, hipLaunchKernelGGL((feat_match_kernel<T, true>), dim3(N), dim3(256), 0, st, (const T*)a, (const T*)f, scale, slope, weight,
                                        (T*)g_y, fterm, M, C));
  } else {
    DISPATCH_T(prec, hipLaunchKernelGGL((feat_match_kernel<T, false>), dim3(N), dim3(256), 0, st, (const T*)a, (const T*)f, scale, slope, weight,
                                        (T*)g_y, fterm, M, C));
  }
  HIPCHK(hipGetLastError());
  return JCK_OK;
}
extern "C" int jck_critic_ds(const float* logit, int mode, float weight, int B, float* ds, float* term, void* stream) {
  if (!logit || !ds || !term || B < 1) JCK_FAIL(JCK_E_ARG, "critic_ds: null logit / ds / term or no rows");
  if (mode != 1 && mode != 2) JCK_FAIL(JCK_E_ARG, "critic_ds: mode must be 1 (nsgan) or 2 (logit)");
  ProfScope prof(K_CRITIC_DS, 0.0, (hipStream_t)stream, (double)B * 12.0);
  hipLaunchKernelGGL(critic_ds_kernel, dim3(cdiv(B, 256)), dim3(256), 0, (hipStream_t)stream, logit, mode, weight, B, ds, term);
  HIPCHK(hipGetLastError());
  return JCK_OK;
}

extern "C" int jck_pack_linear(int prec, const float* w, int N, int K, int rows, int cols, int transpose, int permC, int permHW,
                               void* wp, void* stream) {
  const long long total = (long long)rows * cols;
  DISPATCH_T(prec, hipLaunchKernelGGL(pack_linear_kernel<T>, dim3(ew_grid(total)), dim3(256), 0, (hipStream_t)stream, w, N, K, rows,
                                      cols, transpose, permC, permHW, (T*)wp));
  HIPCHK(hipGetLastError());
  return JCK_OK;
}

int pack_linear_pair(int prec, const float* w, int N, int K, int rows0, int cols0, void* wp0, int rows1, int cols1, void* wp1, int permC,
                     int permHW, hipStream_t stream) {
  const long long total = std::max((long long)rows0 * cols0, (long long)rows1 * cols1);
  DISPATCH_T(prec, hipLaunchKernelGGL(pack_linear_pair_kernel<T>, dim3(ew_grid(total), 2), dim3(256), 0, stream, w, N, K, rows0, cols0,
                                      (T*)wp0, rows1, cols1, (T*)wp1, permC, permHW));
  HIPCHK(hipGetLastError());
  return JCK_OK;
}

extern "C" int jck_unperm_linear_grad(const float* gp, int N, int K, int ldp, int permC, int permHW, float* grad, int accumulate,
                                      void* stream) {
  const long long total = (long long)N * K;
  hipLaunchKernelGGL(unperm_linear_grad_kernel, dim3(ew_grid(total)), dim3(256), 0, (hipStream_t)stream, gp, N, K, ldp, permC,
                     permHW, grad, accumulate);
  HIPCHK(hipGetLastError());
  return JCK_OK;
}
extern "C" int jck_linear_finish(int prec, const float* slab, int Z, const float* bias, const float* mask, float scale, void* h,
                                 void* hd, int B, int N, void* stream) {
  DISPATCH_T(prec, hipLaunchKernelGGL(linear_finish_kernel<T>, dim3(cdiv(B * N, 256)), dim3(256), 0, (hipStream_t)stream, slab, Z,
                                      (long long)B * N, bias, mask, scale, (T*)h, (T*)hd, B, N));
  HIPCHK(hipGetLastError());
  return JCK_OK;
}
extern "C" int jck_label_embed_fwd_tiled(int prec, const int64_t* labels, const float* W, const float* b, float slope, int B, int NI,
                                         int NO, void* cbuf, int ld, int col0, float* pre, int label_period, void* stream) {
  if (label_period < 0 || (label_period > 0 && B % label_period)) JCK_FAIL(JCK_E_ARG, "label_embed: rows are not a multiple of the label period");
  DISPATCH_T(prec, hipLaunchKernelGGL(label_embed_fwd_kernel<T>, dim3(B), dim3(256), (size_t)NI * sizeof(float), (hipStream_t)stream,
                                      (const long long*)labels, W, b, slope, B, NI, NO, (T*)cbuf, ld, col0, pre, label_period));
  HIPCHK(hipGetLastError());
  return JCK_OK;
}
extern "C" int jck_label_embed_fwd(int prec, const int64_t* labels, const float* W, const float* b, float slope, int B, int NI,
                                   int NO, void* cbuf, int ld, int col0, float* pre, void* stream) {
  return jck_label_embed_fwd_tiled(prec, labels, W, b, slope, B, NI, NO, cbuf, ld, col0, pre, 0, stream);
}
extern "C" int jck_label_embed_bwd_tiled(int prec, const void* gc, int ld, int col0, const float* pre, const int64_t* labels, float slope,
                                         int B, int NI, int NO, float* dW, float* db, int label_period, void* stream) {
  if (label_period < 0 || (label_period > 0 && B % label_period)) JCK_FAIL(JCK_E_ARG, "label_embed: rows are not a multiple of the label period");
  DISPATCH_T(prec, hipLaunchKernelGGL(label_embed_bwd_kernel<T>, dim3(NI + cdiv(NO, 16)), dim3(256), (size_t)B * (sizeof(float) + sizeof(int)), (hipStream_t)stream,
                                      (const T*)gc, ld, col0, pre, (const long long*)labels, slope, B, NI, NO, dW, db, label_period));
  HIPCHK(hipGetLastError());
  return JCK_OK;
}
extern "C" int jck_label_embed_bwd(int prec, const void* gc, int ld, int col0, const float* pre, const int64_t* labels, float slope,
                                   int B, int NI, int NO, float* dW, float* db, void* stream) {
  return jck_label_embed_bwd_tiled(prec, gc, ld, col0, pre, labels, slope, B, NI, NO, dW, db, 0, stream);
}
extern "C" int jck_concat_rows(int prec, const void* a4, int K0, void* cbuf, int ld, int B, void* stream) {
  if (K0 % 8 || ld % 8) JCK_FAIL(JCK_E_ARG, "concat_rows: K0 % 8 or ld % 8");
  const long long total8 = (long long)B * K0 / 8;
  DISPATCH_T(prec, hipLaunchKernelGGL(concat_rows_kernel<T>, dim3(ew_grid(total8)), dim3(256), 0, (hipStream_t)stream, (const T*)a4,
                                      K0, (T*)cbuf, ld, total8));
  HIPCHK(hipGetLastError());
  return JCK_OK;
}
extern "C" int jck_split_rows(int prec, const void* gc, int ld, int K0, void* ga4, int B, void* stream) {
  if (K0 % 8 || ld % 8) JCK_FAIL(JCK_E_ARG, "split_rows: K0 % 8 or ld % 8");
  const long long total8 = (long long)B * K0 / 8;
  DISPATCH_T(prec, hipLaunchKernelGGL(split_rows_kernel<T>, dim3(ew_grid(total8)), dim3(256), 0, (hipStream_t)stream, (const T*)gc, ld,
// ... 90 lines not shown
```

### jck-generation_amd/csrc/ops_internal.hpp

```cpp
#pragma once
#include <hip/hip_ext.h>

#include <algorithm>
#include <cmath>
#include <string>

#include "../../include/jckgan.h"
#include "common.hpp"

void jck_set_error(const std::string& s);

static inline bool prec_f32_storage(int prec) { return prec == JCK_PREC_F32 || prec == JCK_PREC_BF16X3; }
static inline bool is_pow2(int v) { return v > 0 && (v & (v - 1)) == 0; }
static inline unsigned ew_grid(long long n, int per_block = 256) { return (unsigned)std::max<long long>(1, std::min<long long>((n + per_block - 1) / per_block, 8192)); }

#define JCK_FAIL(code, msg)                                   \
  do {                                                        \
    jck_set_error(std::string(__func__) + ": " + (msg));     \
    return (code);                                            \
  } while (0)

#define HIPCHK(expr)                                                                                     \
  do {                                                                                                   \
    hipError_t e_ = (expr);                                                                              \
    if (e_ != hipSuccess) {                                                                              \
      jck_set_error(std::string(__func__) + ": HIP error " + hipGetErrorString(e_) + " at " #expr);     \
      return JCK_E_HIP;                                                                                  \
    }                                                                                                    \
  } while (0)

#define JCK_TRY(expr)           \
  do {                          \
    int rc_ = (expr);           \
    if (rc_ != JCK_OK) return rc_; \
  } while (0)

#define LAUNCH_EV(kernel, grid, block, shmem, stream, ev, ...)                                                      \
  do {                                                                                                              \
    if (ev) hipExtLaunchKernelGGL(kernel, grid, block, shmem, stream, (hipEvent_t) nullptr, (hipEvent_t)(ev), 0u, __VA_ARGS__); \
    else hipLaunchKernelGGL(kernel, grid, block, shmem, stream, __VA_ARGS__);                                       \
  } while (0)
#define DISPATCH_T(prec, CALL)                                  \
  do {                                                          \
    if ((prec) == JCK_PREC_BF16) { typedef bf16_t T; CALL; }    \
    else if (prec_f32_storage(prec)) { typedef float T; CALL; } \
    else JCK_FAIL(JCK_E_ARG, "bad prec");                       \
  } while (0)

enum KernelId : int {
  K_PRECS = 3,
  K_IGEMM_TILES = 5,
  K_DMA_TILES = 4,
  K_WGRAD_TILES = 4,
  K_IGEMM = 0,
  K_IGEMM_PERSIST = K_IGEMM + K_PRECS * K_IGEMM_TILES,
  K_IGEMM_DMA = K_IGEMM_PERSIST + K_DMA_TILES,
  K_IMG_DOWN = K_IGEMM_DMA + K_DMA_TILES, K_IMG_UP,
  K_WGRAD_DMA_WS, K_WGRAD_DMA,
  K_WGRAD,
  K_BN_ACT_FWD = K_WGRAD + K_PRECS * K_WGRAD_TILES, K_BN_BWD_RES, K_BN_BWD_3L,
  K_LATENT_LOSS, K_LATENT_ADAM,
  K_CONV_UP_MASK, K_LEAKY_AFFINE_BWD, K_CRITIC_DS, K_LATENT_LOSS_EX,
  K_FEAT_MATCH,
  K_IMG_PREP_ANY,
  K_IMG_PREP_BOX,
  K_COUNT
};
template <class P> constexpr int kid_prec() { return P::SPLIT ? 2 : P::IS_F32 ? 1 : 0; }
template <class P, int BCH, int BPIX, int NSUB> constexpr KernelId kid_igemm() {
  static_assert(P::IS_F32 || !(BCH == 64 && NSUB == 1), "bf16 has no register-staged 64 x 128 tile (and no name for one)");
  return KernelId(K_IGEMM + K_IGEMM_TILES * kid_prec<P>() + (BCH == 128 ? (BPIX == 128 ? 0 : 1) : BCH == 64 ? (NSUB == 2 ? 2 : 3) : 4));
}
constexpr KernelId kid_igemm_dma(KernelId family, int BCH, int BPIX) { return KernelId(family + (BPIX == 256 ? 0 : BCH == 64 ? 3 : BPIX == 128 ? 1 : 2)); }
template <class P, int BG, int BS, int NSUB> constexpr KernelId kid_wgrad() {
  return KernelId(K_WGRAD + K_WGRAD_TILES * kid_prec<P>() + (BG == 128 ? (BS == 128 ? 0 : 1) : NSUB == 2 ? 2 : 3));
}
void note_launch(KernelId k);

extern bool g_prof_on;
struct ProfRec { KernelId kernel; double flops, bytes; hipStream_t st; hipEvent_t e0, e1; };
struct ProfScope {
  ProfScope(KernelId k, double flops, hipStream_t st, double bytes = 0.0) : on(g_prof_on) { if (on) begin(k, flops, st, bytes); }
  ~ProfScope() { if (on) end(); }
 private:
  void begin(KernelId k, double flops, hipStream_t st, double bytes);
  void end();
  bool on; ProfRec r;
};
bool jck_prof_is_on();

extern int g_igemm_dma_ksplit, g_bn_bwd_fuse, g_bn_res, g_wgrad_wgs, g_wgrad_ws, g_wgrad_dma;

int jck_adam_set_step(float* hp, double lr, double beta1, double beta2, int step, unsigned long long seed, float ema_w, hipStream_t st,
                      float* rz = nullptr, long long nz = 0, float* ralpha = nullptr, long long nalpha = 0, float* rmasks = nullptr,
                      long long nmask = 0, float keep_p = 0.75f, float* zero = nullptr, long long nzero = 0, float* zbig0 = nullptr,
                      long long nzbig0 = 0, float* zbig1 = nullptr, long long nzbig1 = 0, void* zpad = nullptr, int zd = 0, int zp = 0,
                      int zpad_f32 = 0);
int jck_adam_hp(float* p, const float* g, float* m, float* v, long long n, double beta1, double beta2, double eps,
                float grad_scale, const float* hp, hipStream_t st, float* zero = nullptr, long long nzero = 0,
                const unsigned* skip_if = nullptr,
                float* ema = nullptr);
const unsigned* jck_grid_sync_error_word(const void* sync_ws);
int bn_fwd_fused(int prec, const void* y, const float* stats, int slots_per_group, float count, const float* gamma, const float* beta,
                 float eps, float slope, void* a, float* aux, float* stat_out, float* running_mean, float* running_var, int64_t* nbt,
                 float momentum, long long rows_per_group, int C, int groups, long long out_row, long long out_pitch, hipStream_t stream,
                 bool* fused);
int bn_act_bwd_res_ev(int prec, const void* g_a, const void* y, const float* aux, float slope, float* sums, void* g_y, float* dgamma,
                      float* dbeta, long long rows_per_group, int C, int groups, int grad_groups, void* sync_ws, hipStream_t stream,
                      hipEvent_t done);
int conv_up_tanh_bwd_ev(int prec, const void* small_in, const void* w, const void* tanh_y, float scale, void* out, int N, int Hs, int Ws,
                        int Cs, int Cb, hipStream_t stream, hipEvent_t done, bool* fused);
int head_bwd_conv2_ev(int prec, const float* ds, const float* wp, const void* a4, int B, int B_more, int C, void* g_a4, float* grad, float* ws,
                      hipStream_t stream, hipStream_t side, hipEvent_t handover);
int gp_head2_ev(int prec, const void* ughd, const float* w2, const float* prob, int B, int K, float* rs, float* dw2, float* ws,
                hipStream_t stream, hipStream_t side, hipEvent_t handover);
int pack_linear_pair(int prec, const float* w, int N, int K, int rows0, int cols0, void* wp0, int rows1, int cols1, void* wp1, int permC,
                     int permHW, hipStream_t stream);
int bn_act_fwd_pitched(int prec, const void* y, const float* aux, float slope, void* a, long long rows_per_group, int C, int groups,
                       long long out_row, long long out_pitch, hipStream_t stream);
int cg_head_mid(int prec, const float* slab, int ksplit, const float* bias1, const float* mask, float scale, void* h, void* hd, const float* w2,
                const float* bias2, int B, int G, const float* targets, const int* modes, float* prob, float* ds, float* scal,
                const int* slot_loss, const int* slot_p, int scal_ld, void* g_hd, void* g_h, hipStream_t stream);
int gp_head_mid_ev(int prec, const float* slab, int ksplit, const float* mask, float scale, void* ughd, const float* w2, const float* prob, int B,
                   float* rs, float* dw2, float* ws, void* g_hd, void* g_h, hipStream_t stream, hipStream_t side, hipEvent_t handover);
int head_fwd_grouped_ev(int prec, const void* a4, const float* wp, const float* bias, int B, int K, int G, const float* targets,
                        const int* modes, float* prob, float* ds, float* scal, const int* slot_loss, const int* slot_p, int scal_ld,
                        void* g_out, hipStream_t stream, hipEvent_t done);
int tanh_bwd_ev(int prec, const void* g, const void* y, float scale, void* out, long long numel, hipStream_t stream, hipEvent_t done);
```

### jck-generation_amd/hipgan/_lib.py

```python
import ctypes as C
import os

import torch

HERE = os.path.dirname(os.path.abspath(__file__))
LIB_PATH = os.path.join(os.path.dirname(HERE), "lib", "libjckgan_hip.so")
PREC_BF16, PREC_F32, PREC_BF16X3 = 0, 1, 2

vp, i32, i64, f32, f64, sz = C.c_void_p, C.c_int, C.c_longlong, C.c_float, C.c_double, C.c_size_t


class StepInputs(C.Structure):
    _fields_ = [("real_nchw", vp), ("noise_real", vp), ("z", vp), ("noise_fake", vp), ("alpha", vp),
                ("lr", f32), ("grad_scale", f32), ("step", i32), ("labels", vp), ("drop_mask", vp * 4),
                ("real_u8", vp), ("real_idx", vp),
                ("real_h", i32), ("real_w", i32), ("real_flip", vp), ("real_taps", vp),
                ("real_box_h", i32), ("real_box_w", i32), ("real_y0", i32), ("real_x0", i32), ("real_origin", vp)]


PROTOS = {
    "jck_last_error": (C.c_char_p, []),
    "jck_last_launch": (C.c_char_p, []),
    "jck_launch_name": (C.c_char_p, [i32]),
    "jck_version": (i32, []),
    "jck_pad_rows": (i32, [i32]),
    "jck_pad_chan": (i32, [i32]),
    "jck_packed_bytes": (sz, [i32, i64]),
    "jck_stats_floats": (sz, [i64, i32, i32]),
    "jck_pack_down": (i32, [i32, vp, i32, i32, vp, vp]),
    "jck_pack_up": (i32, [i32, vp, i32, i32, vp, vp]),
    "jck_pack_g1": (i32, [i32, vp, i32, i32, i32, vp, vp]),
    "jck_pack_head": (i32, [vp, i32, vp, vp]),
    "jck_conv_down": (i32, [i32, vp, vp, vp, vp, C.POINTER(i32), i32, i32, i32, i32, i32, vp]),
    "jck_conv_up": (i32, [i32, vp, vp, vp, vp, C.POINTER(i32), i32, i32, i32, i32, i32, i32, vp]),
    "jck_conv_wgrad_ws_bytes": (sz, [i32, i32, i32, i32, i32]),
    "jck_conv_wgrad": (i32, [i32, vp, vp, vp, sz, vp, i32, i32, i32, i32, i32, i32, vp]),
    "jck_g1_fwd": (i32, [i32, vp, vp, vp, vp, C.POINTER(i32), i32, i32, i32, vp]),
    "jck_conv_up_affine": (i32, [i32, vp, vp, vp, vp, vp, i32, i32, i32, i32, i32, vp]),
    "jck_g1_fwd_affine": (i32, [i32, vp, vp, vp, vp, vp, i32, i32, i32, vp]),
    "jck_conv_down_mask": (i32, [i32, vp, vp, vp, vp, vp, i32, i32, i32, i32, i32, vp]),
    "jck_conv_down_affine": (i32, [i32, vp, vp, vp, vp, f32, vp, i32, i32, i32, i32, i32, vp]),
    "jck_conv_up_mask": (i32, [i32, vp, vp, vp, vp, f32, vp, i32, i32, i32, i32, i32, vp]),
    "jck_leaky_affine_bwd": (i32, [i32, vp, vp, vp, f32, vp, i64, i32, vp]),
    "jck_critic_ds": (i32, [vp, i32, f32, i32, vp, vp, vp]),
    "jck_latent_loss_ex": (i32, [i32, vp, vp, vp, vp, vp, vp, i32, i32, vp]),
    "jck_feat_match": (i32, [i32, vp, vp, vp, f32, f32, vp, i32, vp, i32, i64, i32, vp]),
    "jck_score_head": (i32, [i32, vp, vp, vp, i32, i32, vp, vp, vp]),
    "jck_grid_pool": (i32, [i32, vp, i32, i32, i32, i32, i32, vp, i64, i64, vp]),
    "jck_latent_loss": (i32, [i32, vp, vp, vp, vp, i32, i32, vp]),
    "jck_latent_adam": (i32, [i32, vp, i32, i32, vp, vp, vp, f32, f32, i32, vp, i32, i32, vp]),
    "jck_bn_eval_aux": (i32, [i32, C.POINTER(vp), C.POINTER(vp), C.POINTER(vp), C.POINTER(vp), C.POINTER(vp), C.POINTER(i32), f32, vp]),
    "jck_img_to_u8": (i32, [i32, vp, vp, i32, i32, vp]),
    "jck_g1_wgrad_ws_bytes": (sz, [i32, i32, i32]),
    "jck_g1_wgrad": (i32, [i32, vp, vp, vp, sz, vp, i32, i32, i32, i32, i32, vp]),
    "jck_bn_finalize": (i32, [vp, i32, f32, vp, vp, vp, vp, vp, f32, f32, vp, i32, vp]),
    "jck_bn_act_fwd": (i32, [i32, vp, vp, f32, vp, i64, i32, vp]),
    "jck_bn_bwd_ws_floats": (sz, [i32]),
    "jck_bn_act_bwd": (i32, [i32, vp, vp, vp, f32, vp, vp, vp, vp, i64, i32, vp]),
    "jck_bn_finalize_grouped": (i32, [vp, i32, f32, vp, vp, f32, vp, vp, i32, i32, vp]),
    "jck_bn_act_fwd_grouped": (i32, [i32, vp, vp, f32, vp, i64, i32, i32, vp]),
    "jck_bn_fwd": (i32, [i32, vp, vp, i32, f32, vp, vp, f32, f32, vp, vp, vp, vp, vp, vp, f32, i64, i32, i32, vp]),
    "jck_conv_down_grouped": (i32, [i32, vp, vp, vp, vp, vp, i32, i32, i32, i32, i32, i32, vp]),
    "jck_conv_up_grouped": (i32, [i32, vp, vp, vp, vp, vp, i32, i32, i32, i32, i32, i32, vp]),
    "jck_bn_act_bwd_grouped": (i32, [i32, vp, vp, vp, f32, vp, vp, vp, vp, i64, i32, i32, i32, vp]),
    "jck_grid_sync_bytes": (sz, []),
    "jck_grid_sync_error": (i32, [vp]),
    "jck_bn_act_bwd_res": (i32, [i32, vp, vp, vp, f32, vp, vp, vp, vp, i64, i32, i32, i32, vp, vp]),
    "jck_img_prep": (i32, [i32, vp, vp, f32, f32, vp, i32, i32, vp]),
    "jck_resize_norm": (i32, [vp, vp, i32, i32, i32, i32, i32, i32, f32, f32, vp, vp, vp]),
    "jck_img_prep_u8": (i32, [i32, vp, vp, vp, f32, f32, vp, vp, i32, i32, i32, vp]),
    "jck_resize_taps_bytes": (i64, [i32, i32, i32]),
    "jck_resize_taps_build": (i32, [i32, i32, i32, vp]),
    "jck_img_prep_u8_any": (i32, [i32, vp, vp, vp, vp, vp, i32, f32, f32, vp, vp, i32, i32, i32, i32, vp, vp]),
    "jck_resize_lds_bytes": (i64, [i32, i32, vp, vp]),
    "jck_img_prep_u8_box": (i32, [i32, vp, vp, vp, vp, vp, vp, i32, f32, f32, vp, vp, i32, i32, i32, i32, i32, i32, i32, i32, vp, vp]),
    "jck_nhwc4_to_nchw": (i32, [i32, vp, vp, i32, i32, vp]),
    "jck_axpy_noise": (i32, [i32, vp, vp, f32, f32, vp, i32, i32, vp]),
    "jck_interp": (i32, [i32, vp, vp, vp, vp, i32, i32, vp]),
    "jck_mix_interp": (i32, [i32, vp, vp, vp, i32, f32, f32, vp, vp, vp, vp, i32, i32, vp]),
    "jck_gp_norm": (i32, [i32, vp, i32, i32, vp, i32, i32, vp, vp]),
    "jck_tanh_bwd": (i32, [i32, vp, vp, f32, vp, i64, vp]),
    "jck_head_fwd": (i32, [i32, vp, vp, vp, i32, i32, f32, i32, vp, vp, vp, i32, i32, i32, vp]),
    "jck_head_fwd_grouped": (i32, [i32, vp, vp, vp, i32, i32, i32, vp, vp, vp, vp, vp, vp, vp, i32, vp]),
    "jck_head_bwd_ws_floats": (sz, [i32]),
    "jck_pack_linear": (i32, [i32, vp, i32, i32, i32, i32, i32, i32, i32, vp, vp]),
    "jck_linear_fwd": (i32, [i32, vp, vp, vp, vp, i32, i32, i32, i32, i32, vp]),
    "jck_linear_finish": (i32, [i32, vp, i32, vp, vp, f32, vp, vp, i32, i32, vp]),
    "jck_linear_wgrad_ws_bytes": (sz, [i32, i32, i32]),
    "jck_linear_wgrad": (i32, [i32, vp, i32, vp, i32, vp, sz, vp, i32, i32, i32, vp]),
    "jck_unperm_linear_grad": (i32, [vp, i32, i32, i32, i32, i32, vp, i32, vp]),
    "jck_label_embed_fwd": (i32, [i32, vp, vp, vp, f32, i32, i32, i32, vp, i32, i32, vp, vp]),
    "jck_label_embed_bwd": (i32, [i32, vp, i32, i32, vp, vp, f32, i32, i32, i32, vp, vp, vp]),
    "jck_label_embed_fwd_tiled": (i32, [i32, vp, vp, vp, f32, i32, i32, i32, vp, i32, i32, vp, i32, vp]),
    "jck_label_embed_bwd_tiled": (i32, [i32, vp, i32, i32, vp, vp, f32, i32, i32, i32, vp, vp, i32, vp]),
    "jck_concat_rows": (i32, [i32, vp, i32, vp, i32, i32, vp]),
    "jck_split_rows": (i32, [i32, vp, i32, i32, vp, i32, vp]),
    "jck_dropout": (i32, [i32, vp, vp, f32, vp, i64, vp]),
    "jck_colsum": (i32, [i32, vp, i32, i32, i32, vp, vp]),
    "jck_sum_vec": (i32, [vp, i32, vp, vp]),
    "jck_cgan_z": (i32, [i32, vp, vp, i32, i32, i32, i32, vp, vp]),
    "jck_gp_grad": (i32, [i32, vp, vp, f32, i32, i32, vp, vp]),
    "jck_gp_head2": (i32, [i32, vp, vp, vp, i32, i32, vp, vp, vp, vp]),
    "jck_gp_head2_conv_ws_floats": (sz, [i32]),
    "jck_gp_head2_conv": (i32, [i32, vp, vp, vp, vp, i32, i32, vp, vp, vp, vp, vp]),
    "jck_bn2_ws_floats": (sz, [i32]),
    "jck_bn2_vchain": (i32, [i32, vp, vp, vp, vp, vp, vp, f32, vp, vp, vp, vp, i64, i32, vp]),
    "jck_bn2_reverse": (i32, [i32, vp, vp, vp, vp, vp, vp, f32, vp, vp, vp, vp, i64, i32, vp]),
    "jck_head_bwd": (i32, [i32, vp, vp, vp, i32, i32, vp, vp, i32, vp, vp]),
    "jck_head_unpack_grad": (i32, [vp, i32, vp, i32, vp]),
    "jck_head_bwd_conv": (i32, [i32, vp, vp, vp, i32, i32, vp, vp, vp, vp]),
    "jck_head_bwd_conv2": (i32, [i32, vp, vp, vp, i32, i32, i32, vp, vp, vp, vp]),
    "jck_adam": (i32, [vp, vp, vp, vp, i64, f64, f64, f64, f64, i32, f32, vp]),
    "jck_adam_ema": (i32, [vp, vp, vp, vp, vp, i64, f64, f64, f64, f64, i32, f32, f32, vp, vp]),
    "jck_engine_create": (i32, [C.POINTER(vp), i32, i32, i32]),
    "jck_engine_create_sized": (i32, [C.POINTER(vp), i32, i32, i32, i32]),
    "jck_engine_create_ex": (i32, [C.POINTER(vp), i32, i32, i32, i32, C.c_uint]),
    "jck_engine_image_size": (i32, [vp]),
    "jck_engine_num_tensors_of": (i32, [vp, i32]),
    "jck_engine_tensor_info_of": (i32, [vp, i32, i32, C.c_char_p, i32, C.POINTER(i32), C.POINTER(i64), C.POINTER(i64),
                                        C.POINTER(i32)]),
    "jck_engine_arena_numel_of": (i64, [vp, i32, i32]),
    "jck_engine_destroy": (None, [vp]),
    "jck_engine_num_tensors": (i32, [i32, i32]),
    "jck_engine_tensor_info": (i32, [i32, i32, i32, C.c_char_p, i32, C.POINTER(i32), C.POINTER(i64), C.POINTER(i64),
                                     C.POINTER(i32)]),
    "jck_engine_workspace_bytes": (sz, [vp]),
    "jck_engine_arena_numel": (i64, [i32, i32, i32]),
    "jck_engine_bind": (i32, [vp, vp, sz] + [vp] * 12),
    "jck_engine_repack": (i32, [vp, i32, vp]),
    "jck_engine_phase": (i32, [vp, i32, C.POINTER(StepInputs), vp]),
    "jck_engine_order_after_tail": (i32, [vp, vp]),
    "jck_engine_drop_prefetch": (i32, [vp, vp]),
    "jck_engine_grad_tail": (i64, [vp, i32]),
    "jck_engine_check": (i32, [vp]),
    "jck_engine_scalars": (vp, [vp]),
    "jck_engine_scalars_at": (vp, [vp, i32]),
    "jck_engine_sample": (i32, [vp, vp, vp, i32, vp, vp]),
    "jck_engine_sample_ex": (i32, [vp, vp, vp, i32, C.c_uint, vp, vp, vp]),
    "jck_engine_latent_grad": (i32, [vp, vp, vp, vp, i32, vp, vp, vp]),
    "jck_engine_project": (i32, [vp, vp, vp, vp, i32, i32, f32, f32, vp, vp, i32, vp, vp]),
    "jck_engine_latent_grad_ex": (i32, [vp, vp, vp, vp, vp, i32, f32, i32, vp, vp, vp, vp, vp]),
    "jck_engine_project_ex": (i32, [vp, vp, vp, vp, i32, i32, f32, f32, vp, i32, f32, vp, vp, i32, vp, vp, vp]),
    "jck_engine_latent_grad_fm": (i32, [vp, vp, vp, vp, vp, i32, f32, i32, vp, vp, vp, vp, vp, vp, i32, f32, vp]),
    "jck_engine_project_fm": (i32, [vp, vp, vp, vp, i32, i32, f32, f32, vp, i32, f32, vp, vp, i32, vp, vp, vp, vp, i32, f32, vp]),
    "jck_engine_score": (i32, [vp, vp, vp, vp, i32, vp, vp, vp]),
    "jck_engine_feature_dim": (i64, [vp, i32]),
    "jck_engine_features": (i32, [vp, vp, i32, i32, i32, vp, i64, vp]),
    "jck_engine_tensor": (vp, [vp, C.c_char_p, C.POINTER(i64)]),
    "jck_debug_tr_read": (i32, [vp, i32, vp, vp]),
    "jck_tune": (i32, [C.c_char_p, i32]),
    "jck_conv2d_nhwc_f32": (i32, [vp, vp, vp, vp, vp] + [i32] * 14 + [vp]),
    "jck_pool2d_nhwc_f32": (i32, [vp, vp] + [i32] * 10 + [vp]),
    "jck_global_avgpool_nhwc_f32": (i32, [vp, vp, i32, i32, i32, vp]),
    "jck_nchw_to_nhwc_f32": (i32, [vp, vp, i32, i32, i32, i32, vp]),
    "jck_mean_cov_f64": (i32, [vp, vp, vp, i32, i32, vp]),
    "jck_pairstat_ws_bytes": (sz, [i32, i32]),
    "jck_poly3_sum_f64": (i32, [vp, i32, vp, i32, i32, f64, f64, i32, vp, vp, vp]),
    "jck_knn_radius2_f32": (i32, [vp, i32, i32, i32, vp, vp]),
    "jck_manifold_hit_u8": (i32, [vp, i32, vp, vp, i32, i32, vp, vp]),
    "jck_knn_index_ws_bytes": (sz, [i32, i32]),
    "jck_knn_index_f32": (i32, [vp, i32, vp, i32, i32, i32, i64, i64, i32, i32, vp, vp, vp, vp]),
    "jck_engine_set_step": (i32, [vp, i32, f32, vp]),
    "jck_engine_bind_ema": (i32, [vp, vp]),
    "jck_engine_set_ema": (i32, [vp, f64, i32]),
    "jck_engine_graph_nodes": (i32, [vp]),
    "jck_engine_set_noise_seed": (i32, [vp, C.c_ulonglong]),
    "jck_step_rng": (i32, [vp, i32, C.c_ulonglong, vp, C.c_longlong, vp, C.c_longlong, vp, C.c_longlong, f32, vp]),
    "jck_img_prep_rng": (i32, [i32, vp, vp, i32, f32, f32, vp, i32, i32, vp]),
    "jck_img_prep_u8_rng": (i32, [i32, vp, vp, vp, i32, f32, f32, vp, i32, i32, i32, vp]),
    "jck_axpy_noise_rng": (i32, [i32, vp, vp, i32, f32, f32, vp, i32, i32, vp]),
    "jck_engine_capture_begin": (i32, [vp, vp]),
    "jck_engine_capture_end": (i32, [vp, vp, C.POINTER(vp)]),
    "jck_engine_capture_abort": (i32, [vp, vp]),
    "jck_graph_launch": (i32, [vp, vp]),
    "jck_graph_destroy": (None, [vp]),
    "jck_comm_unique_id": (i32, [vp]),
    "jck_comm_create": (i32, [C.POINTER(vp), vp, i32, i32]),
    "jck_comm_world": (i32, [vp]),
    "jck_comm_allreduce_enqueue": (i32, [vp, vp, sz, vp, C.POINTER(i32)]),
    "jck_comm_wait": (i32, [vp, i32, vp]),
    "jck_comm_destroy": (i32, [vp]),
    "jck_prof_enable": (i32, [i32]),
    "jck_prof_collect": (i32, [i32, C.POINTER(C.c_char_p), C.POINTER(i32), C.POINTER(f64), C.POINTER(f64), C.POINTER(f64), C.POINTER(vp)]),
}


class JckError(RuntimeError):
    pass


_cdll = None


def load_library(path=None):
    global _cdll
    if _cdll is not None:
        return _cdll
    path = path or os.environ.get("JCKGAN_LIB", LIB_PATH)
    if not os.path.exists(path):
        raise JckError(f"{path} not found: build it with `python __graft_entry__.py build` "
                       f"(hipcc --offload-arch=gfx950); there is no CPU fallback")
    dll = C.CDLL(path)
    partial = os.environ.get("JCKGAN_ALLOW_PARTIAL") == "1"
    for name, (res, args) in PROTOS.items():
        if partial and not hasattr(dll, name):
            continue
        fn = getattr(dll, name)
        fn.restype, fn.argtypes = res, args
    if os.path.abspath(path) == os.path.abspath(LIB_PATH) and os.environ.get("JCKGAN_ALLOW_STALE") != "1":
        from . import build as _build
        want, got = _build.source_id(), dll.jck_version()
        if got != want:
            raise JckError(f"{path} was built from other sources than the ones beside it (jck_version {got}, sources {want}): "
                           f"rebuild with `python __graft_entry__.py build`")
    _cdll = dll
    return dll


def _arg(a):
    if a is None:
        return None
    if isinstance(a, torch.Tensor):
        return a.data_ptr()
    return a


class _Lib:

    def __getattr__(self, name):
        dll = load_library()
        fn = getattr(dll, name)

        def call(*args):
            for a in args:
                if isinstance(a, torch.Tensor):
                    if not a.is_cuda:
                        raise JckError(f"{name}: tensor argument is on {a.device}; the HIP path needs device memory")
                    if not a.is_contiguous():
                        raise JckError(f"{name}: non-contiguous tensor argument")
            r = fn(*[_arg(a) for a in args])
            if fn.restype is i32 and name not in ("jck_version", "jck_pad_rows", "jck_pad_chan", "jck_engine_num_tensors", "jck_prof_collect", "jck_grid_sync_error", "jck_comm_world", "jck_engine_graph_nodes") \
                    and r != 0:
                raise JckError(f"{name} failed ({r}): {dll.jck_last_error().decode()}")
            return r
        call.__name__ = name
        setattr(self, name, call)
        return call


lib = _Lib()


def cur_stream():
    return torch.cuda.current_stream().cuda_stream
```

Baseline: 164,300 images/sec.

## Fuse Adam update with conv weight repacking into one kernel

Adds a combined kernel that applies Adam to each conv weight tile, stages the updated values in shared memory, and writes the packed bf16/f32 conv layouts from there. Other parameter ranges get flat Adam blocks in the same launch, and the G-side BN tail jobs are folded in too. This removes separate Adam and repack launches and the re-read of the updated fp32 weights. The default flag is on, with a fallback to the old path when pointers are misaligned. Risks are the shared-memory footprint, lower occupancy, and sequential job-scan overhead.

```diff
diff --git a/include/jckgan.h b/include/jckgan.h
--- a/include/jckgan.h
+++ b/include/jckgan.h
@@ -177,6 +177,9 @@
              int step, float grad_scale, void* stream);
 int jck_adam_ema(float* p, const float* g, float* m, float* v, float* ema, long long n, double lr, double beta1, double beta2,
                  double eps, int step, float grad_scale, float ema_weight, const unsigned* skip_if, void* stream);
+int jck_adam_pack(int prec, float* p, const float* g, float* m, float* v, float* ema, long long n, int njobs, const int* kind,
+                  const long long* w_off, void* const* wp, const int* a, const int* b, double lr, double beta1, double beta2, double eps,
+                  int step, float grad_scale, float ema_weight, const unsigned* skip_if, void* stream);
 
 typedef struct jck_engine jck_engine;
 int jck_engine_create(jck_engine** out, int family, int prec, int batch);
diff --git a/jck-generation_amd/csrc/engine.hip b/jck-generation_amd/csrc/engine.hip
--- a/jck-generation_amd/csrc/engine.hip
+++ b/jck-generation_amd/csrc/engine.hip
@@ -138,6 +138,7 @@
   e->real_side = env_on("JCK_REAL_SIDE");
   e->fold_zero = env_on("JCK_FOLD_ZERO");
   e->fuse_tanh = env_on("JCK_FUSE_TANH");
+  e->adam_pack = env_on("JCK_ADAM_PACK");
   if (e->overlap) JCK_TRY(create_side_streams(e));
   *out = e;
   return JCK_OK;
@@ -196,8 +197,7 @@
   return JCK_OK;
 }
 
-static int repack_convs(jck_engine* e, int net, void* stream, const TailJobs* tail = nullptr, int tail_x = 0) {
-  PackJobs jobs = {};
+static int pack_jobs(const jck_engine* e, int net, PackJobs& jobs) {
   int n = 0, chunk = 0;
   auto add = [&](int kind, const float* w, void* wp, long long total, int a, int b, int c) {
     PackJob& J = jobs.j[n];
@@ -228,6 +228,11 @@
   }
   jobs.first_chunk[n] = chunk;
   jobs.n = n;
+  return chunk;
+}
+static int repack_convs(jck_engine* e, int net, void* stream, const TailJobs* tail = nullptr, int tail_x = 0) {
+  PackJobs jobs = {};
+  const int chunk = pack_jobs(e, net, jobs);
   if (net == 1) e->d_packed = true;
   if (tail) {
     const int nblk = chunk + tail_x * (tail->nl + 1);
@@ -667,6 +672,19 @@
   return jck_adam_hp(p + first, g + first, m + first, v + first, count, ADAM_B1, ADAM_B2, ADAM_EPS, grad_scale, hp, st, zero_other,
                      zero_other ? (net ? e->LG : e->LD).n_params : 0, jck_grid_sync_error_word(e->gsync), ema);
 }
+static int adam_repack_net(jck_engine* e, int net, long long first, long long count, float grad_scale, const float* hp, hipStream_t st,
+                           float* zero_other = nullptr, float* ema = nullptr, const TailJobs* tail = nullptr, int tail_x = 0) {
+  float *p = net ? e->dp : e->gp, *g = net ? e->dg : e->gg, *m = net ? e->dm : e->gm, *v = net ? e->dv : e->gv;
+  if (!e->adam_pack || (((uintptr_t)p | (uintptr_t)g | (uintptr_t)m | (uintptr_t)v | (uintptr_t)ema) & 15)) {
+    JCK_TRY(adam_net(e, net, first, count, grad_scale, hp, st, zero_other, ema));
+    return repack_convs(e, net, st, tail, tail_x);
+  }
+  PackJobs jobs = {};
+  pack_jobs(e, net, jobs);
+  if (net == 1) e->d_packed = true;
+  return jck_adam_pack_hp(e->prec, p, g, m, v, ema, first, count, jobs, ADAM_B1, ADAM_B2, ADAM_EPS, grad_scale, hp, 0.f, 1.f, 1.f, st, zero_other,
+                          zero_other ? (net ? e->LG : e->LD).n_params : 0, jck_grid_sync_error_word(e->gsync), tail, tail_x);
+}
 static int clear_or_memset(jck_engine* e, int& clean_step, int step, hipStream_t st, void* p, size_t bytes, void* p2 = nullptr, size_t bytes2 = 0) {
   const bool clean = clean_step == step && !e->capturing;
   clean_step = -1;
@@ -879,15 +897,15 @@
     const TensorInfo* c1 = find(e->LD, CWN[0]);
     const long long cut = c1->offset + c1->numel;
     HIPCHK(hipStreamWaitEvent(c.st, e->ss.mid_recorded ? e->evWmid : e->evWdone, 0));
-    JCK_TRY(adam_net(e, 1, cut, e->LD.n_params - cut, c.in->grad_scale, hp, c.st, zg));
+    if (e->adam_pack) JCK_TRY(adam_repack_net(e, 1, cut, e->LD.n_params - cut, c.in->grad_scale, hp, c.st, zg));
+    else JCK_TRY(adam_net(e, 1, cut, e->LD.n_params - cut, c.in->grad_scale, hp, c.st, zg));
     JCK_TRY(repack_linear(e, c.st));
     if (e->ss.mid_recorded) HIPCHK(hipStreamWaitEvent(c.st, e->evWdone, 0));
     e->ss.join_pending = e->ss.mid_recorded = false;
-    JCK_TRY(adam_net(e, 1, 0, cut, c.in->grad_scale, hp, c.st));
-    return repack_convs(e, 1, c.st);
-  }
-  JCK_TRY(adam_net(e, 1, 0, e->LD.n_params, c.in->grad_scale, hp, c.st, zg));
-  return jck_engine_repack(e, 1, c.st);
+    return adam_repack_net(e, 1, 0, cut, c.in->grad_scale, hp, c.st);
+  }
+  JCK_TRY(adam_repack_net(e, 1, 0, e->LD.n_params, c.in->grad_scale, hp, c.st, zg));
+  return e->family == 1 ? repack_linear(e, c.st) : JCK_OK;
 }
 
 static int phase_g_loss(jck_engine* e, const PhaseCtx& c) {
@@ -909,7 +927,6 @@
 
 static int phase_g_step(jck_engine* e, const PhaseCtx& c) {
   if (!e->hp_holds(c.in->step, c.in->lr) && !e->capturing) JCK_TRY(refresh_adam_scalars(e, c.in->step, c.in->lr, c.st));
-  JCK_TRY(adam_net(e, 0, 0, e->LG.n_params, c.in->grad_scale, e->hp2 + 8 * e->parity, c.st, nullptr, e->gema));
   TailJobs t = {};
   for (int i = 0; i < TT.NS; ++i) {
     const int cs = TT.D_CS[i];
@@ -920,7 +937,7 @@
     t.l[i].C = cs;
   }
   t.nl = TT.NS; t.npass = 4; t.momentum = BN_MOM; t.acc = e->acc; t.acc_ld = e->acc_ld; t.B = c.B; t.invB = 1.0f / (float)c.B; t.lambda_gp = 10.0f; t.out = e->scal_out;
-  return repack_convs(e, 0, c.st, &t, cdiv(TT.G_C1, 256));
+  return adam_repack_net(e, 0, 0, e->LG.n_params, c.in->grad_scale, e->hp2 + 8 * e->parity, c.st, nullptr, e->gema, &t, cdiv(TT.G_C1, 256));
 }
 
 static int phase_begin(jck_engine* e, int phase, jck_step_inputs& loc, hipStream_t st) {
diff --git a/jck-generation_amd/csrc/engine_internal.hpp b/jck-generation_amd/csrc/engine_internal.hpp
--- a/jck-generation_amd/csrc/engine_internal.hpp
+++ b/jck-generation_amd/csrc/engine_internal.hpp
@@ -118,6 +118,7 @@
   bool real_side = true;
   bool fold_zero = true;
   bool fuse_tanh = true;
+  bool adam_pack = true;
   void *g_z, *g_y[JCK_MAX_STAGES], *g_a[JCK_MAX_STAGES], *g_gr[JCK_MAX_STAGES], *fake_raw, *fake, *g_raw;
   void *real_noisy, *xhat;
   BnBuf g_bn[JCK_MAX_STAGES];
diff --git a/jck-generation_amd/csrc/ew_optim.hpp b/jck-generation_amd/csrc/ew_optim.hpp
--- a/jck-generation_amd/csrc/ew_optim.hpp
+++ b/jck-generation_amd/csrc/ew_optim.hpp
@@ -62,6 +62,31 @@
   pi = pi - step_size * (mi / denom);
 }
 __device__ __forceinline__ float ema_one(float e, float pn, float w) { return (w < 0.5f) ? e + w * (pn - e) : pn - (pn - e) * (1.f - w); }
+struct AdamScal { float w1 , beta2, omb2 , eps, step_size, bc2_sqrt, grad_scale, ema_w; };
+template <bool EMA>
+__device__ __forceinline__ void adam_quad(float* __restrict__ p, const float* __restrict__ g, float* __restrict__ m, float* __restrict__ v,
+                                          float* __restrict__ ema, long long i, const AdamScal& s, float* pn = nullptr) {
+  f32x4 pv = reinterpret_cast<f32x4*>(p)[i], mv = reinterpret_cast<f32x4*>(m)[i], vv = reinterpret_cast<f32x4*>(v)[i];
+  const f32x4 gv = reinterpret_cast<const f32x4*>(g)[i];
+  f32x4 ev;
+  if (EMA) ev = reinterpret_cast<f32x4*>(ema)[i];
+#pragma unroll
+  for (int k = 0; k < 4; ++k) {
+    float pk = pv[k], mk = mv[k], vk = vv[k];
+    adam_one(pk, gv[k], mk, vk, s.w1, s.beta2, s.omb2, s.eps, s.step_size, s.bc2_sqrt, s.grad_scale);
+    pv[k] = pk; mv[k] = mk; vv[k] = vk;
+    if (EMA) ev[k] = ema_one(ev[k], pk, s.ema_w);
+    if (pn) pn[k] = pk;
+  }
+  reinterpret_cast<f32x4*>(p)[i] = pv; reinterpret_cast<f32x4*>(m)[i] = mv; reinterpret_cast<f32x4*>(v)[i] = vv;
+  if (EMA) reinterpret_cast<f32x4*>(ema)[i] = ev;
+}
+template <bool EMA>
+__device__ __forceinline__ void adam_single(float* __restrict__ p, const float* __restrict__ g, float* __restrict__ m, float* __restrict__ v,
+                                            float* __restrict__ ema, long long i, const AdamScal& s) {
+  adam_one(p[i], g[i], m[i], v[i], s.w1, s.beta2, s.omb2, s.eps, s.step_size, s.bc2_sqrt, s.grad_scale);
+  if (EMA) ema[i] = ema_one(ema[i], p[i], s.ema_w);
+}
 template <bool EMA>
 static __global__ void adam_kernel(float* __restrict__ p, const float* __restrict__ g, float* __restrict__ m,
                             float* __restrict__ v, long long n, float w1 , float beta2, float omb2 ,
@@ -74,26 +99,12 @@
   for (long long i = blockIdx.x * (long long)blockDim.x + threadIdx.x; i < nzero4; i += (long long)gridDim.x * blockDim.x)
     reinterpret_cast<f32x4*>(zero)[i] = f32x4{0.f, 0.f, 0.f, 0.f};
   if (skip) return;
+  const AdamScal s = {w1, beta2, omb2, eps, step_size, bc2_sqrt, grad_scale, ema_w};
   const long long n4 = vec ? (n >> 2) : 0;
-  for (long long i = blockIdx.x * (long long)blockDim.x + threadIdx.x; i < n4; i += (long long)gridDim.x * blockDim.x) {
-    f32x4 pv = reinterpret_cast<f32x4*>(p)[i], mv = reinterpret_cast<f32x4*>(m)[i], vv = reinterpret_cast<f32x4*>(v)[i];
-    const f32x4 gv = reinterpret_cast<const f32x4*>(g)[i];
-    f32x4 ev;
-    if (EMA) ev = reinterpret_cast<f32x4*>(ema)[i];
-#pragma unroll
-    for (int k = 0; k < 4; ++k) {
-      float pk = pv[k], mk = mv[k], vk = vv[k];
-      adam_one(pk, gv[k], mk, vk, w1, beta2, omb2, eps, step_size, bc2_sqrt, grad_scale);
-      pv[k] = pk; mv[k] = mk; vv[k] = vk;
-      if (EMA) ev[k] = ema_one(ev[k], pk, ema_w);
-    }
-    reinterpret_cast<f32x4*>(p)[i] = pv; reinterpret_cast<f32x4*>(m)[i] = mv; reinterpret_cast<f32x4*>(v)[i] = vv;
-    if (EMA) reinterpret_cast<f32x4*>(ema)[i] = ev;
-  }
-  for (long long i = (n4 << 2) + blockIdx.x * (long long)blockDim.x + threadIdx.x; i < n; i += (long long)gridDim.x * blockDim.x) {
-    adam_one(p[i], g[i], m[i], v[i], w1, beta2, omb2, eps, step_size, bc2_sqrt, grad_scale);
-    if (EMA) ema[i] = ema_one(ema[i], p[i], ema_w);
-  }
+  for (long long i = blockIdx.x * (long long)blockDim.x + threadIdx.x; i < n4; i += (long long)gridDim.x * blockDim.x)
+    adam_quad<EMA>(p, g, m, v, ema, i, s);
+  for (long long i = (n4 << 2) + blockIdx.x * (long long)blockDim.x + threadIdx.x; i < n; i += (long long)gridDim.x * blockDim.x)
+    adam_single<EMA>(p, g, m, v, ema, i, s);
 }
 
 __device__ __forceinline__ float pack_down_val(const float* __restrict__ w, int Cs, int Cb, int logCbPad, long long i) {
@@ -169,68 +180,67 @@
 struct PackJob { const float* w; void* wp; long long total; int kind, a, b, c; };
 struct PackJobs { PackJob j[PACK_MAX_JOBS]; int first_chunk[PACK_MAX_JOBS + 1]; int n; };
 template <typename W>
+__device__ __forceinline__ void pack_store_pair(const PackJob& J, int x, int y, const float* v) {
+  W* wp = reinterpret_cast<W*>(J.wp);
+  switch (J.kind) {
+    case 0: {
+      W* d = wp + (((long long)x * 16) << J.c) + y;
+#pragma unroll
+      for (int t = 0; t < 16; ++t) stf(d + ((long long)t << J.c), v[t]);
+    } break;
+    case 1: {
+      const int Cs = J.a;
+      const long long K = 4ll * Cs, per = (long long)J.c * K;
+#pragma unroll
+      for (int phase = 0; phase < 4; ++phase)
+#pragma unroll
+        for (int t = 0; t < 4; ++t) {
+          const int kh = c_up_k[phase >> 1][t >> 1], kw = c_up_k[phase & 1][t & 1];
+          stf(wp + phase * per + (long long)y * K + (long long)t * Cs + x, v[kh * 4 + kw]);
+        }
+    } break;
+    case 2: {
+      const int Cs = J.a;
+      const long long K = 9ll * Cs;
+#pragma unroll
+      for (int phase = 0; phase < 4; ++phase)
+#pragma unroll
+        for (int t9 = 0; t9 < 9; ++t9) {
+          const int dy = t9 / 3 - 1, dx = t9 % 3 - 1, ph = phase >> 1, pw = phase & 1;
+          const int kh = ph == 0 ? (dy == 0 ? 1 : (dy == -1 ? 3 : -1)) : (dy == 1 ? 0 : (dy == 0 ? 2 : -1));
+          const int kw = pw == 0 ? (dx == 0 ? 1 : (dx == -1 ? 3 : -1)) : (dx == 1 ? 0 : (dx == 0 ? 2 : -1));
+          if (kh >= 0 && kw >= 0) stf(wp + (long long)(phase * 4 + y) * K + (long long)t9 * Cs + x, v[kh * 4 + kw]);
+        }
+    } break;
+    case 3: {
+#pragma unroll
+      for (int t = 0; t < 16; ++t) stf(wp + ((long long)t * J.b + y) * J.c + x, v[t]);
+    } break;
+    default: {
+#pragma unroll
+      for (int t = 0; t < 16; ++t) reinterpret_cast<float*>(J.wp)[(long long)t * J.a + x] = v[t];
+    } break;
+  }
+}
+template <typename W>
 __device__ __forceinline__ void pack_multi_block(const PackJobs& jobs, int bx) {
   int ji = 0;
   while (ji + 1 < jobs.n && bx >= jobs.first_chunk[ji + 1]) ++ji;
   const PackJob& J = jobs.j[ji];
   const long long u = (long long)(bx - jobs.first_chunk[ji]) * PACK_CHUNK + threadIdx.x;
   if (u >= J.total) return;
-  W* wp = reinterpret_cast<W*>(J.wp);
+  int x, y, Bc = J.b;
+  if (J.kind == 0) { x = (int)(u / J.b); y = (int)(u % J.b); }
+  else if (J.kind == 4) { x = (int)u; y = 0; Bc = 1; }
+  else { y = (int)(u / J.a); x = (int)(u % J.a); }
+  const float* src = J.w + ((long long)x * Bc + y) * 16;
   float v[16];
-  auto load16 = [&](const float* src) {
-#pragma unroll
-    for (int q = 0; q < 4; ++q) {
-      const f32x4 t = *reinterpret_cast<const f32x4*>(src + 4 * q);
-      v[4 * q] = t[0]; v[4 * q + 1] = t[1]; v[4 * q + 2] = t[2]; v[4 * q + 3] = t[3];
-    }
-  };
-  switch (J.kind) {
-    case 0: {
-      const int Cb = J.b, cs = (int)(u / Cb), cb = (int)(u % Cb);
-      load16(J.w + ((long long)cs * Cb + cb) * 16);
-      W* d = wp + (((long long)cs * 16) << J.c) + cb;
-#pragma unroll
-      for (int t = 0; t < 16; ++t) stf(d + ((long long)t << J.c), v[t]);
-    } break;
-    case 1: {
-      const int Cs = J.a, Cb = J.b, cb = (int)(u / Cs), cs = (int)(u % Cs);
-      load16(J.w + ((long long)cs * Cb + cb) * 16);
-      const long long K = 4ll * Cs, per = (long long)J.c * K;
-#pragma unroll
-      for (int phase = 0; phase < 4; ++phase)
-#pragma unroll
-        for (int t = 0; t < 4; ++t) {
-          const int kh = c_up_k[phase >> 1][t >> 1], kw = c_up_k[phase & 1][t & 1];
-          stf(wp + phase * per + (long long)cb * K + (long long)t * Cs + cs, v[kh * 4 + kw]);
-        }
-    } break;
-    case 2: {
-      const int Cs = J.a, Cb = J.b, c = (int)(u / Cs), cs = (int)(u % Cs);
-      load16(J.w + ((long long)cs * Cb + c) * 16);
-      const long long K = 9ll * Cs;
-#pragma unroll
-      for (int phase = 0; phase < 4; ++phase)
-#pragma unroll
-        for (int t9 = 0; t9 < 9; ++t9) {
-          const int dy = t9 / 3 - 1, dx = t9 % 3 - 1, ph = phase >> 1, pw = phase & 1;
-          const int kh = ph == 0 ? (dy == 0 ? 1 : (dy == -1 ? 3 : -1)) : (dy == 1 ? 0 : (dy == 0 ? 2 : -1));
-          const int kw = pw == 0 ? (dx == 0 ? 1 : (dx == -1 ? 3 : -1)) : (dx == 1 ? 0 : (dx == 0 ? 2 : -1));
-          if (kh >= 0 && kw >= 0) stf(wp + (long long)(phase * 4 + c) * K + (long long)t9 * Cs + cs, v[kh * 4 + kw]);
-        }
-    } break;
-    case 3: {
-      const int Ci = J.a, Co = J.b, co = (int)(u / Ci), ci = (int)(u % Ci);
-      load16(J.w + ((long long)ci * Co + co) * 16);
-#pragma unroll
-      for (int t = 0; t < 16; ++t) stf(wp + ((long long)t * Co + co) * J.c + ci, v[t]);
-    } break;
-    default: {
-      const int c = (int)u;
-      load16(J.w + (long long)c * 16);
-#pragma unroll
-      for (int t = 0; t < 16; ++t) reinterpret_cast<float*>(J.wp)[(long long)t * J.a + c] = v[t];
-    } break;
-  }
+#pragma unroll
+  for (int q = 0; q < 4; ++q) {
+    const f32x4 t = *reinterpret_cast<const f32x4*>(src + 4 * q);
+    v[4 * q] = t[0]; v[4 * q + 1] = t[1]; v[4 * q + 2] = t[2]; v[4 * q + 3] = t[3];
+  }
+  pack_store_pair<W>(J, x, y, v);
 }
 template <typename W>
 __global__ __launch_bounds__(256) void pack_multi_kernel(const PackJobs jobs) { pack_multi_block<W>(jobs, (int)blockIdx.x); }
@@ -300,3 +310,66 @@
   const int q = (int)blockIdx.x - pack_chunks;
   step_tail_block(t, q % tail_x, q / tail_x);
 }
+
+#define ADAM_MAX_FLAT 8
+struct AdamGroup { long long off; int A, Bc, j0, nj; };
+struct AdamPlan {
+  AdamGroup g[PACK_MAX_JOBS]; int first_blk[PACK_MAX_JOBS + 1]; int ng;
+  long long fa[ADAM_MAX_FLAT], fb[ADAM_MAX_FLAT]; int first_fblk[ADAM_MAX_FLAT + 1]; int nf;
+};
+struct AdamArenas { float* p; const float* g; float *m, *v, *ema; const float* hp; float* zero; long long nzero4; const unsigned* skip_if; };
+template <typename W, bool EMA>
+__device__ __forceinline__ void adam_pair_block(const PackJobs& jobs, const AdamGroup& G, int tile, const AdamArenas& a, const AdamScal& s) {
+  __shared__ __attribute__((aligned(16))) float sm[16 * 17 * 20];
+  const int tid = threadIdx.x, lane = tid & 63, wv = tid >> 6;
+  const int ty = (G.Bc + 15) >> 4, x0 = tile / ty * 16, y0 = tile % ty * 16;
+  const int nq = min(64, (G.Bc - y0) * 4);
+#pragma unroll
+  for (int k = 0; k < 4; ++k) {
+    const int xr = 4 * k + wv;
+    if (x0 + xr < G.A && lane < nq) {
+      float pn[4];
+      adam_quad<EMA>(a.p, a.g, a.m, a.v, a.ema, (G.off >> 2) + ((long long)(x0 + xr) * G.Bc + y0) * 4 + lane, s, pn);
+      *reinterpret_cast<f32x4*>(sm + (xr * 17 + (lane >> 2)) * 20 + (lane & 3) * 4) = f32x4{pn[0], pn[1], pn[2], pn[3]};
+    }
+  }
+  __syncthreads();
+  for (int f = G.j0; f < G.j0 + G.nj; ++f) {
+    const PackJob& J = jobs.j[f];
+    const int xl = J.kind == 0 ? tid >> 4 : tid & 15, yl = J.kind == 0 ? tid & 15 : tid >> 4;
+    if (x0 + xl >= G.A || y0 + yl >= G.Bc) continue;
+    float r[16];
+#pragma unroll
+    for (int q = 0; q < 4; ++q) {
+      const f32x4 t = *reinterpret_cast<const f32x4*>(sm + (xl * 17 + yl) * 20 + 4 * q);
+      r[4 * q] = t[0]; r[4 * q + 1] = t[1]; r[4 * q + 2] = t[2]; r[4 * q + 3] = t[3];
+    }
+    pack_store_pair<W>(J, x0 + xl, y0 + yl, r);
+  }
+}
+template <typename W, bool EMA>
+__global__ __launch_bounds__(256) void adam_pack_kernel(const PackJobs jobs, const AdamPlan plan, const AdamArenas a, AdamScal s, int pair_blks,
+                                                        int flat_blks, const TailJobs t, int tail_x) {
+  const int bx = (int)blockIdx.x, nb = pair_blks + flat_blks;
+  if (bx >= nb) { step_tail_block(t, (bx - nb) % tail_x, (bx - nb) / tail_x); return; }
+  for (long long i = bx * 256ll + threadIdx.x; i < a.nzero4; i += nb * 256ll) reinterpret_cast<f32x4*>(a.zero)[i] = f32x4{0.f, 0.f, 0.f, 0.f};
+  if (a.skip_if && *a.skip_if != 0u) return;
+  if (a.hp) { s.step_size = a.hp[0]; s.bc2_sqrt = a.hp[1]; if (EMA) s.ema_w = a.hp[2]; }
+  if (bx < pair_blks) {
+    int gi = 0;
+    while (gi + 1 < plan.ng && bx >= plan.first_blk[gi + 1]) ++gi;
+    adam_pair_block<W, EMA>(jobs, plan.g[gi], bx - plan.first_blk[gi], a, s);
+    return;
+  }
+  const int fx = bx - pair_blks;
+  int fi = 0;
+  while (fi + 1 < plan.nf && fx >= plan.first_fblk[fi + 1]) ++fi;
+  const long long fa = plan.fa[fi], fb = plan.fb[fi], a4 = min((fa + 3) & ~3ll, fb), b4 = max(fb & ~3ll, a4);
+  const int k = fx - plan.first_fblk[fi];
+  const long long i = (a4 >> 2) + k * 256ll + threadIdx.x;
+  if (i < (b4 >> 2)) adam_quad<EMA>(a.p, a.g, a.m, a.v, a.ema, i, s);
+  if (k == 0) {
+    const int nh = (int)(a4 - fa), nt = (int)(fb - b4);
+    if ((int)threadIdx.x < nh + nt) adam_single<EMA>(a.p, a.g, a.m, a.v, a.ema, (int)threadIdx.x < nh ? fa + threadIdx.x : b4 + (threadIdx.x - nh), s);
+  }
+}
diff --git a/jck-generation_amd/csrc/ops.hip b/jck-generation_amd/csrc/ops.hip
--- a/jck-generation_amd/csrc/ops.hip
+++ b/jck-generation_amd/csrc/ops.hip
@@ -573,6 +573,88 @@
   return JCK_OK;
 }
 
+int jck_adam_pack_hp(int prec, float* p, const float* g, float* m, float* v, float* ema, long long first, long long count, const PackJobs& jobs,
+                     double beta1, double beta2, double eps, float grad_scale, const float* hp, float step_size, float bc2_sqrt, float ema_w,
+                     hipStream_t st, float* zero, long long nzero, const unsigned* skip_if, const TailJobs* tail, int tail_x) {
+  if (((uintptr_t)p | (uintptr_t)g | (uintptr_t)m | (uintptr_t)v | (uintptr_t)ema) & 15) JCK_FAIL(JCK_E_ARG, "adam_pack: the arenas must be 16-byte aligned");
+  if (zero && (((uintptr_t)zero & 15) || (nzero & 3))) JCK_FAIL(JCK_E_ARG, "adam: the zero range must be 16-byte aligned, count % 4 == 0");
+  if (first < 0 || count < 0) JCK_FAIL(JCK_E_ARG, "adam_pack: bad range");
+  PackJobs sel = {};
+  AdamPlan plan = {};
+  int blk = 0;
+  for (int i = 0; i < jobs.n; ++i) {
+    const PackJob& J = jobs.j[i];
+    const int A = J.a, Bc = J.kind == 4 ? 1 : J.b;
+    const long long off = J.w - p, numel = 16ll * A * Bc;
+    if (off + numel <= first || off >= first + count) continue;
+    if (off < first || off + numel > first + count || (off & 3)) JCK_FAIL(JCK_E_ARG, "adam_pack: a conv weight straddles the range or is not 16-byte aligned");
+    if (plan.ng && plan.g[plan.ng - 1].off == off) ++plan.g[plan.ng - 1].nj;
+    else {
+      if (plan.ng && off < plan.g[plan.ng - 1].off + 16ll * plan.g[plan.ng - 1].A * plan.g[plan.ng - 1].Bc) JCK_FAIL(JCK_E_ARG, "adam_pack: conv weights must come in arena order, without overlap");
+      plan.g[plan.ng] = AdamGroup{off, A, Bc, sel.n, 1};
+      plan.first_blk[plan.ng++] = blk;
+      blk += cdiv(A, 16) * cdiv(Bc, 16);
+    }
+    sel.j[sel.n++] = J;
+  }
+  plan.first_blk[plan.ng] = blk;
+  const int pair_blks = blk;
+  int fblk = 0;
+  auto flat = [&](long long a, long long b) {
+    if (a >= b) return true;
+    if (plan.nf == ADAM_MAX_FLAT) return false;
+    plan.fa[plan.nf] = a; plan.fb[plan.nf] = b;
+    plan.first_fblk[plan.nf++] = fblk;
+    const long long a4 = std::min((a + 3) & ~3ll, b), b4 = std::max(b & ~3ll, a4);
+    fblk += (int)std::max<long long>(1, ((b4 - a4) / 4 + 255) / 256);
+    return true;
+  };
+  long long at = first;
+  bool fits = true;
+  for (int i = 0; i < plan.ng; ++i) {
+    fits = fits && flat(at, plan.g[i].off);
+    at = plan.g[i].off + 16ll * plan.g[i].A * plan.g[i].Bc;
+  }
+  fits = fits && flat(at, first + count);
+  if (!fits) JCK_FAIL(JCK_E_ARG, "adam_pack: more than ADAM_MAX_FLAT ranges between the conv weights");
+  plan.first_fblk[plan.nf] = fblk;
+  const int nb = pair_blks + fblk;
+  const TailJobs no_tail = {};
+  const int tail_blks = tail ? tail_x * (tail->nl + 1) : 0;
+  if (nb + tail_blks == 0) return JCK_OK;
+  const AdamArenas a = {p, g, m, v, ema, hp, zero, zero ? nzero / 4 : 0, skip_if};
+  const AdamScal s = {(float)(1.0 - beta1), (float)beta2, (float)(1.0 - beta2), (float)eps, step_size, bc2_sqrt, grad_scale, ema_w};
+#define ADAM_PACK_LAUNCH(W, EMA) \
+  hipLaunchKernelGGL((adam_pack_kernel<W, EMA>), dim3(nb + tail_blks), dim3(256), 0, st, sel, plan, a, s, pair_blks, fblk, tail ? *tail : no_tail, tail ? tail_x : 1)
+  if (prec == JCK_PREC_BF16) { if (ema) ADAM_PACK_LAUNCH(bf16_t, true); else ADAM_PACK_LAUNCH(bf16_t, false); }
+  else if (ema) ADAM_PACK_LAUNCH(float, true);
+  else ADAM_PACK_LAUNCH(float, false);
+#undef ADAM_PACK_LAUNCH
+  HIPCHK(hipGetLastError());
+  return JCK_OK;
+}
+extern "C" int jck_adam_pack(int prec, float* p, const float* g, float* m, float* v, float* ema, long long n, int njobs, const int* kind,
+                             const long long* w_off, void* const* wp, const int* a, const int* b, double lr, double beta1, double beta2, double eps,
+                             int step, float grad_scale, float ema_weight, const unsigned* skip_if, void* stream) {
+  if (step < 1) JCK_FAIL(JCK_E_ARG, "adam: step is 1-based");
+  if (njobs < 0 || njobs > PACK_MAX_JOBS || (njobs && (!kind || !w_off || !wp || !a || !b))) JCK_FAIL(JCK_E_ARG, "adam_pack: 0..12 jobs, every table given");
+  if (prec != JCK_PREC_BF16 && !prec_f32_storage(prec)) JCK_FAIL(JCK_E_ARG, "bad prec");
+  PackJobs jobs = {};
+  for (int i = 0; i < njobs; ++i) {
+    PackJob& J = jobs.j[i];
+    if (kind[i] < 0 || kind[i] > 4 || a[i] < 1 || (kind[i] != 4 && b[i] < 1) || !wp[i]) JCK_FAIL(JCK_E_ARG, "adam_pack: bad job");
+    J.w = p + w_off[i]; J.wp = wp[i]; J.kind = kind[i]; J.a = a[i]; J.b = kind[i] == 4 ? 0 : b[i];
+    J.total = (long long)a[i] * (kind[i] == 4 ? 1 : b[i]);
+    J.c = kind[i] == 0 ? ilog2(jck_pad_chan(b[i])) : kind[i] == 1 ? jck_pad_rows(b[i]) : kind[i] == 3 ? (a[i] + 127) / 128 * 128 : 0;
+    if (kind[i] == 0 && (1 << J.c) != jck_pad_chan(b[i])) JCK_FAIL(JCK_E_ARG, "adam_pack: down needs a power-of-two (padded) Cb");
+    if (kind[i] == 2 && b[i] > 4) JCK_FAIL(JCK_E_ARG, "adam_pack: up16 packs at most 4 channels");
+  }
+  jobs.n = njobs;
+  const double bc1 = 1.0 - std::pow(beta1, step), bc2 = 1.0 - std::pow(beta2, step);
+  return jck_adam_pack_hp(prec, p, g, m, v, ema, 0, n, jobs, beta1, beta2, eps, grad_scale, nullptr, (float)(lr / bc1), (float)std::sqrt(bc2),
+                          ema_weight, (hipStream_t)stream, nullptr, 0, skip_if, nullptr, 0);
+}
+
 static int launch_latent_loss(KernelId id, double bytes, int prec, const void* x, const float* target, const float* weight, const void* g_x,
                               void* g_raw, float* loss, int N, int HW, hipStream_t st) {
   ProfScope prof(id, 0.0, st, bytes);
diff --git a/jck-generation_amd/csrc/ops_internal.hpp b/jck-generation_amd/csrc/ops_internal.hpp
--- a/jck-generation_amd/csrc/ops_internal.hpp
+++ b/jck-generation_amd/csrc/ops_internal.hpp
@@ -100,6 +100,11 @@
                 float grad_scale, const float* hp, hipStream_t st, float* zero = nullptr, long long nzero = 0,
                 const unsigned* skip_if = nullptr,
                 float* ema = nullptr);
+struct PackJobs;
+struct TailJobs;
+int jck_adam_pack_hp(int prec, float* p, const float* g, float* m, float* v, float* ema, long long first, long long count, const PackJobs& jobs,
+                     double beta1, double beta2, double eps, float grad_scale, const float* hp, float step_size, float bc2_sqrt, float ema_w,
+                     hipStream_t st, float* zero, long long nzero, const unsigned* skip_if, const TailJobs* tail, int tail_x);
 const unsigned* jck_grid_sync_error_word(const void* sync_ws);
 int bn_fwd_fused(int prec, const void* y, const float* stats, int slots_per_group, float count, const float* gamma, const float* beta,
                  float eps, float slope, void* a, float* aux, float* stat_out, float* running_mean, float* running_var, int64_t* nbt,
diff --git a/jck-generation_amd/hipgan/_lib.py b/jck-generation_amd/hipgan/_lib.py
--- a/jck-generation_amd/hipgan/_lib.py
+++ b/jck-generation_amd/hipgan/_lib.py
@@ -112,6 +112,8 @@
     "jck_head_bwd_conv2": (i32, [i32, vp, vp, vp, i32, i32, i32, vp, vp, vp, vp]),
     "jck_adam": (i32, [vp, vp, vp, vp, i64, f64, f64, f64, f64, i32, f32, vp]),
     "jck_adam_ema": (i32, [vp, vp, vp, vp, vp, i64, f64, f64, f64, f64, i32, f32, f32, vp, vp]),
+    "jck_adam_pack": (i32, [i32, vp, vp, vp, vp, vp, i64, i32, C.POINTER(i32), C.POINTER(i64), C.POINTER(vp), C.POINTER(i32), C.POINTER(i32),
+                            f64, f64, f64, f64, i32, f32, f32, vp, vp]),
     "jck_engine_create": (i32, [C.POINTER(vp), i32, i32, i32]),
     "jck_engine_create_sized": (i32, [C.POINTER(vp), i32, i32, i32, i32]),
     "jck_engine_create_ex": (i32, [C.POINTER(vp), i32, i32, i32, i32, C.c_uint]),
```

Measured after the change: 166,000 images/sec (median of 6 runs). 1.0% higher.
